# hirofumi0810/tensorflow_end2end_speech_recognition

Hardware: AMD Instinct MI355X
Metric: acoustic frames/sec (train), TIMIT-shaped BLSTM-CTC (higher is better)
Workload: dtype bf16; 1 GPU; TIMIT 61-phone 5x256 BLSTM-CTC, B=16/GPU, D=120, C=62, seq_len~U{100..778}, dropout 0.2, rmsprop, train step; global_batch=16, parallelism=dp1, padded_to=own Tmax per rank

## Files before the change

include/asr_hip.h:

```cpp
#ifndef ASR_HIP_H_
#define ASR_HIP_H_

#include <stddef.h>
#include <stdint.h>

#ifdef __cplusplus
extern "C" {
#endif

typedef struct asr_handle asr_handle;
typedef void* asr_stream;

typedef enum {
  ASR_OK = 0,
  ASR_ERR_INVALID_ARG = -1,
  ASR_ERR_UNSUPPORTED = -2,
  ASR_ERR_HIP = -3,
  ASR_ERR_WORKSPACE = -4
} asr_status;

typedef enum { ASR_F32 = 0, ASR_BF16 = 1 } asr_dtype;

typedef enum {
  ASR_OPT_SGD = 0, ASR_OPT_MOMENTUM = 1, ASR_OPT_NESTEROV = 2, ASR_OPT_ADAGRAD = 3,
  ASR_OPT_ADADELTA = 4, ASR_OPT_RMSPROP = 5, ASR_OPT_ADAM = 6
} asr_optimizer;

int asr_abi_version(void);
int asr_create(asr_handle** out, int device);
int asr_create_ex(asr_handle** out, int device, size_t scratch_bytes);
size_t asr_scratch_bytes(asr_handle* h);
int asr_destroy(asr_handle* h);
const char* asr_last_error_string(asr_handle* h);
int asr_set_xcd_skip(asr_handle* h, int n);
int asr_set_gemm_tn_workgroups(asr_handle* h, int n);
int asr_device_info(asr_handle* h, int* num_cu, char* name, int name_len);

int asr_bt_to_tb(asr_handle* h, int dtype, const float* in_btd, void* out_tbd,
                 int B, int T, int D, asr_stream s);
int asr_bt_to_tb_ld(asr_handle* h, int dtype, const float* in_btd, void* out_tbd,
                    int B, int T, int D, int ld_out, asr_stream s);
int asr_stack_frames(asr_handle* h, const float* x, const int32_t* seq_len, int B, int T, int F,
                     int num_stack, int num_skip, float* out, int32_t* out_len, asr_stream s);
int asr_splice(asr_handle* h, const float* x, const int32_t* seq_len, int B, int T, int D, int splice,
               int num_stack, float* out, asr_stream s);
int asr_transpose2d(asr_handle* h, int dtype, const void* in, int rows, int cols, int ld_in,
                    void* out, int ld_out, asr_stream s);
int asr_cast_from_f32(asr_handle* h, int dtype, const float* in, void* out, size_t n, asr_stream s);
int asr_cast_to_f32(asr_handle* h, int dtype, const void* in, float* out, size_t n, asr_stream s);
int asr_apply_mask(asr_handle* h, int dtype, const void* in, const float* mask, void* out,
                   size_t n, asr_stream s);
int asr_touch(asr_handle* h, const void* p, size_t bytes, asr_stream s);
int asr_dropout_mask(asr_handle* h, float* mask, size_t n, float keep_prob,
                     uint64_t seed, uint64_t offset, asr_stream s);
int asr_dropout_apply(asr_handle* h, int dtype, const void* in, void* out, size_t n, float keep_prob, uint64_t seed,
                      uint64_t offset, asr_stream s);
int asr_relu_bwd_drop(asr_handle* h, int dtype, const float* dout, const void* out, size_t n, float keep_prob,
                      uint64_t seed, uint64_t offset, void* dpre, asr_stream s);
int asr_colsum(asr_handle* h, int dtype, const void* a, int M, int N, int lda,
               float* out, asr_stream s);

int asr_gemm(asr_handle* h, int dtype, int out_dtype, int transA, int transB,
             int M, int N, int K, const void* A, int lda, const void* B, int ldb,
             void* C, int ldc, const float* bias, int accumulate, asr_stream s);

int asr_gemm_act(asr_handle* h, int dtype, int out_dtype, int transA, int transB,
                 int M, int N, int K, const void* A, int lda, const void* B, int ldb,
                 void* C, int ldc, const float* bias, int accumulate, int act, asr_stream s);
int asr_gemm_mul(asr_handle* h, int dtype, int transA, int transB, int M, int N, int K,
                 const void* A, int lda, const void* B, int ldb, float* C, int ldc,
                 const float* bias, int accumulate, int act, const float* mul, int ldmul, asr_stream s);
int asr_gemm_drop(asr_handle* h, int dtype, int transA, int transB, int M, int N, int K, const void* A, int lda,
                  const void* B, int ldb, float* C, int ldc, const float* bias, int accumulate, int act, float keep_prob,
                  uint64_t seed, uint64_t offset, asr_stream s);

int asr_im2col3x3(asr_handle* h, int dtype, const void* in, int N, int H, int W, int Cin, int ldp,
                  void* patches, asr_stream s);
int asr_col2im3x3(asr_handle* h, const float* dpatches, int N, int H, int W, int Cin, int ldp,
                  float* din, asr_stream s);
int asr_im2col(asr_handle* h, int dtype, const void* in_nhwc, int N, int H, int W, int Cin, int kh, int kw,
               int sh, int sw, int ldp, void* patches, asr_stream s);
int asr_col2im(asr_handle* h, const float* dpatches, int N, int H, int W, int Cin, int kh, int kw,
               int sh, int sw, int ldp, float* din_nhwc, asr_stream s);
int asr_conv3x3_prep_weights(asr_handle* h, const float* w_hwio, int Cin, int Cout, void* wt_fwd,
                             void* wt_bwd, asr_stream s);
int asr_conv3x3_fwd(asr_handle* h, const void* x, int N, int H, int W, int Cin, const void* wt_fwd,
                    const float* bias, int Cout, int relu, void* out, asr_stream s);
int asr_conv3x3_fwd_drop(asr_handle* h, const void* x, int N, int H, int W, int Cin, const void* wt_fwd,
                         const float* bias, int Cout, float keep_prob, uint64_t seed, uint64_t offset, void* out,
                         asr_stream s);
int asr_conv3x3_bwd_data(asr_handle* h, const void* dy, int N, int H, int W, int Cout,
                         const void* wt_bwd, int Cin, float* dx, asr_stream s);
int asr_conv3x3_bwd_data_relu(asr_handle* h, const void* dy, int N, int H, int W, int Cout, const void* wt_bwd, int Cin,
                              const void* act_below, float keep_prob, uint64_t seed, uint64_t offset, int use_drop,
                              void* dpre_below, asr_stream s);
int asr_conv3x3_bwd_weight(asr_handle* h, const void* x, const void* dy, int N, int H, int W,
                           int Cin, int Cout, float* dw, int accumulate, asr_stream s);
int asr_conv3x3_bwd_weight_bias(asr_handle* h, const void* x, const void* dy, int N, int H, int W,
                                int Cin, int Cout, float* dw, float* dbias, asr_stream s);
int asr_maxpool2x2_fwd(asr_handle* h, int dtype, const void* in, int N, int H, int W, int C,
                       void* out, uint8_t* argmax, asr_stream s);
int asr_maxpool2x2_fwd_drop(asr_handle* h, int dtype, const void* in, int N, int H, int W, int C, void* out,
                            uint8_t* argmax, float keep_prob, uint64_t seed, uint64_t offset, asr_stream s);
int asr_maxpool2x2_bwd(asr_handle* h, const float* dout, const uint8_t* argmax, int N, int H, int W,
                       int C, float* din, asr_stream s);
int asr_conv3x3_smallc_fwd(asr_handle* h, const void* x, int N, int H, int W, int Cin, const void* w2d,
                           const float* bias, int Cout, int relu, void* out, asr_stream s);
int asr_conv3x3_smallc_fwd_drop(asr_handle* h, const void* x, int N, int H, int W, int Cin, const void* w2d,
                                const float* bias, int Cout, float keep_prob, uint64_t seed, uint64_t offset, void* out,
                                asr_stream s);
int asr_conv3x3_smallc_bwd_weight(asr_handle* h, const void* x, const void* dpre, int N, int H, int W, int Cin,
                                  int Cout, float* dw, asr_stream s);
int asr_conv3x3_smallc_bwd_weight_bias(asr_handle* h, const void* x, const void* dpre, int N, int H, int W, int Cin,
                                       int Cout, float* dw, float* dbias, asr_stream s);
int asr_maxpool2x2_relu_bwd(asr_handle* h, int dtype, const float* dout, const uint8_t* argmax, const void* act, int N,
                            int H, int W, int C, void* dpre, float keep_prob, uint64_t seed, uint64_t offset,
                            int use_drop, asr_stream s);
int asr_relu_bwd(asr_handle* h, int dtype, const float* dout, const void* out, const float* mask,
                 size_t n, void* dpre, asr_stream s);
int asr_relu_bwd_scaled(asr_handle* h, int dtype, const float* dout, const void* out, size_t n, float keep, void* dpre,
                        asr_stream s);

int asr_conv3x5_prep_weights(asr_handle* h, const float* w_hwio, int Cin, int Cout, void* wt_fwd, void* wt_bwd,
                             asr_stream s);
int asr_conv3x5_fwd(asr_handle* h, const void* x, int N, int H, int W, int Cin, const void* wt_fwd, const float* bias,
                    int Cout, int relu, void* out, asr_stream s);
int asr_conv3x5_fwd_drop(asr_handle* h, const void* x, int N, int H, int W, int Cin, const void* wt_fwd,
                         const float* bias, int Cout, float keep_prob, uint64_t seed, uint64_t offset, void* out,
                         asr_stream s);
int asr_conv3x5_bwd_data(asr_handle* h, const void* dy, int N, int H, int W, int Cout, const void* wt_bwd, int Cin,
                         float* dx, asr_stream s);
int asr_conv3x5_bwd_data_relu(asr_handle* h, const void* dy, int N, int H, int W, int Cout, const void* wt_bwd, int Cin,
                              const void* act_below, float keep_prob, uint64_t seed, uint64_t offset, int use_drop,
                              void* dpre_below, asr_stream s);
int asr_conv3x5_bwd_weight_bias(asr_handle* h, const void* x, const void* dy, int N, int H, int W, int Cin, int Cout,
                                float* dw, float* dbias, asr_stream s);
int asr_maxpool3x1_fwd(asr_handle* h, int dtype, const void* in, int N, int H, int W, int C, void* out, uint8_t* argmax,
                       float keep_prob, uint64_t seed, uint64_t offset, int use_drop, asr_stream s);
int asr_maxpool3x1_bwd(asr_handle* h, int dtype, const void* dout, const uint8_t* argmax, int N, int H, int W, int C,
                       void* din, asr_stream s);

int asr_conv3x4_prep_weights(asr_handle* h, const float* w_hwio, int Cin, int Cout, void* wt_fwd, void* wt_bwd,
                             asr_stream s);
int asr_conv3x4_fwd(asr_handle* h, const void* x, int N, int H, int W, int Cin, const void* wt_fwd, const float* bias,
                    int Cout, int relu, int out_f32, void* out, asr_stream s);
int asr_conv3x4_bwd_data(asr_handle* h, const void* dy, int N, int H, int W, int Cout, const void* wt_bwd, int Cin,
                         float* dx, asr_stream s);
int asr_conv3x4_bwd_weight_bias(asr_handle* h, const void* x, const void* dy, int N, int H, int W, int Cin, int Cout,
                                float* dw, float* dbias, asr_stream s);
size_t asr_bn_workspace_bytes(long long M, int C);
int asr_bn_stats(asr_handle* h, const float* x, long long M, int C, float eps, float momentum, const float* avg_mean,
                 const float* avg_var, float* stats, void* ws, asr_stream s);
int asr_bn_apply(asr_handle* h, int out_dtype, const float* x, int N, int H, int W, int C, const float* mean,
                 const float* var, const float* gamma, const float* beta, float eps, int pool, void* out,
                 uint8_t* argmax, asr_stream s);
int asr_bn_bwd(asr_handle* h, int out_dtype, const float* dz, const uint8_t* argmax, int pool, const float* x, int N,
               int H, int W, int C, const float* stats, const float* gamma, int relu_gate, float* dgamma, float* dbeta,
               void* dx, void* ws, asr_stream s);
int asr_softmax_xent_soft(asr_handle* h, const float* logits, const float* targets, int rows, int C, float grad_scale,
                          float* row_loss, float* dlogits, asr_stream s);

int asr_lstm_prep_weights(asr_handle* h, int dtype, const float* kernel, const float* bias,
                          int Din, int H, void* wx_il, float* bias_il,
                          void* packed_fwd, void* packed_bwd, asr_stream s);
int asr_lstm_prep_layer(asr_handle* h, int dtype, int ndir, const float* const* vars, int Din, int ldk, int H,
                        void* wxT, void* wx_cat, float* bias_cat, void* packed_fwd, void* packed_bwd,
                        float* peep_out, asr_stream s);
int asr_lstm_grad_finish(asr_handle* h, int ndir, float* const* grads, int rows, int H, const float* dw_il,
                         const float* dpeep_dbias, int has_peep, asr_stream s);
int asr_gate_deinterleave(asr_handle* h, const float* in, int ld_in, float* out, int ld_out,
                          int rows, int H, asr_stream s);

int asr_lstm_fwd(asr_handle* h, int dtype, int T, int B, int H, int ndir,
                 const float* xproj, const void* wh_packed, const float* peep,
                 const int32_t* seq_len, float forget_bias, float cell_clip,
                 void* gates, void* hout, float* cs, float* c_final, float* h_final,
                 asr_stream s);

int asr_lstm_bwd(asr_handle* h, int dtype, int T, int B, int H, int ndir,
                 const float* dhout, const void* gates, const float* cs,
                 const void* wh_packed_bwd, const float* peep, const int32_t* seq_len,
                 const float* d_c_final, const float* d_h_final,
                 void* dgates, float* dpeep_dbias, float* dpeep_workspace, asr_stream s);
int asr_lstm_bwd_ex(asr_handle* h, int dtype, int T, int B, int H, int ndir,
                    const float* dhout, const void* gates, const float* cs,
                    const void* wh_packed_bwd, const float* peep, const int32_t* seq_len,
                    const float* d_c_final, const float* d_h_final, float clip_no_grad,
                    void* dgates, float* dpeep_dbias, float* dpeep_workspace, asr_stream s);

int asr_check_async_errors(asr_handle* h, unsigned* flags_out);
int asr_peek_async_errors(asr_handle* h, unsigned* host_flags, asr_stream s);
int asr_clear_async_errors(asr_handle* h, asr_stream s);
int asr_debug_set_lstm_flags(int flags);
int asr_debug_set_gru_persistent(int on);

int asr_debug_tear_probe(asr_handle* h, unsigned* buf, unsigned iters, int peer, int write_through,
                         unsigned long long* out, asr_stream s);

int asr_debug_placement(asr_handle* h, unsigned* out, int nblocks, int spin_cycles, asr_stream s);
int asr_debug_poison_lds(asr_handle* h, asr_stream s);

int asr_gru_fwd(asr_handle* h, int T, int B, int H, int ndir, const float* xg, const float* xc,
                const float* wgh, const float* wch, const int32_t* seq_len, int tmax, float* r, float* u,
                float* c, float* rh, float* hout, float* hstate2, asr_stream s);
int asr_gru_bwd(asr_handle* h, int T, int B, int H, int ndir, const float* dout, const float* d_h_final,
                const float* hout, const float* r, const float* u, const float* c, const float* wghT,
                const float* wchT, const int32_t* seq_len, int tmax, float* dgate, float* dcand,
                float* work2, asr_stream s);

size_t asr_ctc_workspace_bytes(int T, int B, int max_label_len);
int asr_ctc_loss(asr_handle* h, const float* logits, int T, int B, int C,
                 const int32_t* labels_flat, const int32_t* label_offsets,
                 const int32_t* seq_len, int max_label_len, float grad_scale,
                 float* loss, float* grad, int32_t* num_infeasible,
                 void* workspace, size_t workspace_bytes, asr_stream s);

int asr_ctc_greedy_decode(asr_handle* h, const float* logits, int T, int B, int C,
                          const int32_t* seq_len, int blank,
                          int32_t* out_labels, int32_t* out_len, asr_stream s);

size_t asr_ctc_beam_workspace_bytes(int T, int B, int C, int beam_width);
int asr_ctc_beam_decode(asr_handle* h, const float* logits, int T, int B, int C,
                        const int32_t* seq_len, int blank, int beam_width,
                        int32_t* out_labels, int32_t* out_len, double* out_score,
                        void* workspace, size_t workspace_bytes, asr_stream s);

int asr_softmax_rows(asr_handle* h, const float* in, float* out, int rows, int C, asr_stream s);
// ... 135 lines not shown
```

tensorflow_end2end_speech_recognition_amd/_lib.py:

```python
import ctypes as C
import os

_PKG = os.path.dirname(os.path.abspath(__file__))
LIB_PATH = os.path.join(_PKG, 'libasr_hip.so')

ASR_F32, ASR_BF16 = 0, 1
OPTIMIZER_IDS = {'sgd': 0, 'momentum': 1, 'nestrov': 2, 'adagrad': 3, 'adadelta': 4,
                 'rmsprop': 5, 'adam': 6}

_vp, _i, _f, _sz = C.c_void_p, C.c_int, C.c_float, C.c_size_t
_i64, _u64 = C.c_int64, C.c_uint64

SIGNATURES = {
    'asr_abi_version': (_i, []),
    'asr_create': (_i, [C.POINTER(_vp), _i]),
    'asr_create_ex': (_i, [C.POINTER(_vp), _i, _sz]),
    'asr_scratch_bytes': (_sz, [_vp]),
    'asr_destroy': (_i, [_vp]),
    'asr_set_xcd_skip': (_i, [_vp, _i]),
    'asr_set_gemm_tn_workgroups': (_i, [_vp, _i]),
    'asr_last_error_string': (C.c_char_p, [_vp]),
    'asr_device_info': (_i, [_vp, C.POINTER(_i), C.c_char_p, _i]),
    'asr_bt_to_tb': (_i, [_vp, _i, _vp, _vp, _i, _i, _i, _vp]),
    'asr_bt_to_tb_ld': (_i, [_vp, _i, _vp, _vp, _i, _i, _i, _i, _vp]),
    'asr_transpose2d': (_i, [_vp, _i, _vp, _i, _i, _i, _vp, _i, _vp]),
    'asr_cast_from_f32': (_i, [_vp, _i, _vp, _vp, _sz, _vp]),
    'asr_cast_to_f32': (_i, [_vp, _i, _vp, _vp, _sz, _vp]),
    'asr_apply_mask': (_i, [_vp, _i, _vp, _vp, _vp, _sz, _vp]),
    'asr_dropout_mask': (_i, [_vp, _vp, _sz, _f, _u64, _u64, _vp]),
    'asr_touch': (_i, [_vp, _vp, _sz, _vp]),
    'asr_dropout_apply': (_i, [_vp, _i, _vp, _vp, _sz, _f, _u64, _u64, _vp]),
    'asr_relu_bwd_drop': (_i, [_vp, _i, _vp, _vp, _sz, _f, _u64, _u64, _vp, _vp]),
    'asr_colsum': (_i, [_vp, _i, _vp, _i, _i, _i, _vp, _vp]),
    'asr_gemm': (_i, [_vp, _i, _i, _i, _i, _i, _i, _i, _vp, _i, _vp, _i, _vp, _i, _vp, _i, _vp]),
    'asr_gemm_act': (_i, [_vp, _i, _i, _i, _i, _i, _i, _i, _vp, _i, _vp, _i, _vp, _i, _vp, _i, _i, _vp]),
    'asr_gemm_drop': (_i, [_vp, _i, _i, _i, _i, _i, _i, _vp, _i, _vp, _i, _vp, _i, _vp, _i, _i, _f, _u64, _u64, _vp]),
    'asr_gemm_mul': (_i, [_vp, _i, _i, _i, _i, _i, _i, _vp, _i, _vp, _i, _vp, _i, _vp, _i, _i, _vp, _i, _vp]),
    'asr_conv3x3_prep_weights': (_i, [_vp, _vp, _i, _i, _vp, _vp, _vp]),
    'asr_conv3x3_fwd': (_i, [_vp, _vp, _i, _i, _i, _i, _vp, _vp, _i, _i, _vp, _vp]),
    'asr_conv3x3_fwd_drop': (_i, [_vp, _vp, _i, _i, _i, _i, _vp, _vp, _i, _f, _u64, _u64, _vp, _vp]),
    'asr_conv3x3_bwd_data': (_i, [_vp, _vp, _i, _i, _i, _i, _vp, _i, _vp, _vp]),
    'asr_conv3x3_smallc_fwd': (_i, [_vp, _vp, _i, _i, _i, _i, _vp, _vp, _i, _i, _vp, _vp]),
    'asr_conv3x3_smallc_fwd_drop': (_i, [_vp, _vp, _i, _i, _i, _i, _vp, _vp, _i, _f, _u64, _u64, _vp, _vp]),
    'asr_conv3x3_smallc_bwd_weight': (_i, [_vp, _vp, _vp, _i, _i, _i, _i, _i, _vp, _vp]),
    'asr_conv3x3_smallc_bwd_weight_bias': (_i, [_vp, _vp, _vp, _i, _i, _i, _i, _i, _vp, _vp, _vp]),
    'asr_conv3x3_bwd_data_relu': (_i, [_vp, _vp, _i, _i, _i, _i, _vp, _i, _vp, _f, _u64, _u64, _i, _vp, _vp]),
    'asr_conv3x3_bwd_weight': (_i, [_vp, _vp, _vp, _i, _i, _i, _i, _i, _vp, _i, _vp]),
    'asr_conv3x3_bwd_weight_bias': (_i, [_vp, _vp, _vp, _i, _i, _i, _i, _i, _vp, _vp, _vp]),
    'asr_im2col3x3': (_i, [_vp, _i, _vp, _i, _i, _i, _i, _i, _vp, _vp]),
    'asr_col2im3x3': (_i, [_vp, _vp, _i, _i, _i, _i, _i, _vp, _vp]),
    'asr_im2col': (_i, [_vp, _i, _vp, _i, _i, _i, _i, _i, _i, _i, _i, _i, _vp, _vp]),
    'asr_col2im': (_i, [_vp, _vp, _i, _i, _i, _i, _i, _i, _i, _i, _i, _vp, _vp]),
    'asr_maxpool2x2_fwd': (_i, [_vp, _i, _vp, _i, _i, _i, _i, _vp, _vp, _vp]),
    'asr_maxpool2x2_fwd_drop': (_i, [_vp, _i, _vp, _i, _i, _i, _i, _vp, _vp, _f, _u64, _u64, _vp]),
    'asr_relu_bwd_scaled': (_i, [_vp, _i, _vp, _vp, _sz, _f, _vp, _vp]),
    'asr_maxpool2x2_bwd': (_i, [_vp, _vp, _vp, _i, _i, _i, _i, _vp, _vp]),
    'asr_relu_bwd': (_i, [_vp, _i, _vp, _vp, _vp, _sz, _vp, _vp]),
    'asr_maxpool2x2_relu_bwd': (_i, [_vp, _i, _vp, _vp, _vp, _i, _i, _i, _i, _vp, _f, _u64, _u64, _i, _vp]),
    'asr_conv3x5_prep_weights': (_i, [_vp, _vp, _i, _i, _vp, _vp, _vp]),
    'asr_conv3x5_fwd': (_i, [_vp, _vp, _i, _i, _i, _i, _vp, _vp, _i, _i, _vp, _vp]),
    'asr_conv3x5_fwd_drop': (_i, [_vp, _vp, _i, _i, _i, _i, _vp, _vp, _i, _f, _u64, _u64, _vp, _vp]),
    'asr_conv3x5_bwd_data': (_i, [_vp, _vp, _i, _i, _i, _i, _vp, _i, _vp, _vp]),
    'asr_conv3x5_bwd_data_relu': (_i, [_vp, _vp, _i, _i, _i, _i, _vp, _i, _vp, _f, _u64, _u64, _i, _vp, _vp]),
    'asr_conv3x5_bwd_weight_bias': (_i, [_vp, _vp, _vp, _i, _i, _i, _i, _i, _vp, _vp, _vp]),
    'asr_maxpool3x1_fwd': (_i, [_vp, _i, _vp, _i, _i, _i, _i, _vp, _vp, _f, _u64, _u64, _i, _vp]),
    'asr_maxpool3x1_bwd': (_i, [_vp, _i, _vp, _vp, _i, _i, _i, _i, _vp, _vp]),
    'asr_conv3x4_prep_weights': (_i, [_vp, _vp, _i, _i, _vp, _vp, _vp]),
    'asr_conv3x4_fwd': (_i, [_vp, _vp, _i, _i, _i, _i, _vp, _vp, _i, _i, _i, _vp, _vp]),
    'asr_conv3x4_bwd_data': (_i, [_vp, _vp, _i, _i, _i, _i, _vp, _i, _vp, _vp]),
    'asr_conv3x4_bwd_weight_bias': (_i, [_vp, _vp, _vp, _i, _i, _i, _i, _i, _vp, _vp, _vp]),
    'asr_bn_workspace_bytes': (_sz, [_i64, _i]),
    'asr_bn_stats': (_i, [_vp, _vp, _i64, _i, _f, _f, _vp, _vp, _vp, _vp, _vp]),
    'asr_bn_apply': (_i, [_vp, _i, _vp, _i, _i, _i, _i, _vp, _vp, _vp, _vp, _f, _i, _vp, _vp, _vp]),
    'asr_bn_bwd': (_i, [_vp, _i, _vp, _vp, _i, _vp, _i, _i, _i, _i, _vp, _vp, _i, _vp, _vp, _vp, _vp, _vp]),
    'asr_softmax_xent_soft': (_i, [_vp, _vp, _vp, _i, _i, _f, _vp, _vp, _vp]),
    'asr_lstm_prep_weights': (_i, [_vp, _i, _vp, _vp, _i, _i, _vp, _vp, _vp, _vp, _vp]),
    'asr_lstm_prep_layer': (_i, [_vp, _i, _i, _vp, _i, _i, _i, _vp, _vp, _vp, _vp, _vp, _vp, _vp]),
    'asr_lstm_grad_finish': (_i, [_vp, _i, _vp, _i, _i, _vp, _vp, _i, _vp]),
    'asr_gate_deinterleave': (_i, [_vp, _vp, _i, _vp, _i, _i, _i, _vp]),
    'asr_lstm_fwd': (_i, [_vp, _i, _i, _i, _i, _i, _vp, _vp, _vp, _vp, _f, _f, _vp, _vp, _vp, _vp, _vp, _vp]),
    'asr_lstm_bwd': (_i, [_vp, _i, _i, _i, _i, _i, _vp, _vp, _vp, _vp, _vp, _vp, _vp, _vp, _vp, _vp,
                          _vp, _vp]),
    'asr_lstm_bwd_ex': (_i, [_vp, _i, _i, _i, _i, _i, _vp, _vp, _vp, _vp, _vp, _vp, _vp, _vp, _f, _vp, _vp,
                             _vp, _vp]),
    'asr_gru_fwd': (_i, [_vp, _i, _i, _i, _i, _vp, _vp, _vp, _vp, _vp, _i, _vp, _vp, _vp, _vp, _vp, _vp, _vp]),
    'asr_gru_bwd': (_i, [_vp, _i, _i, _i, _i, _vp, _vp, _vp, _vp, _vp, _vp, _vp, _vp, _vp, _i, _vp, _vp, _vp, _vp]),
    'asr_check_async_errors': (_i, [_vp, C.POINTER(C.c_uint)]),
    'asr_peek_async_errors': (_i, [_vp, _vp, _vp]),
    'asr_clear_async_errors': (_i, [_vp, _vp]),
    'asr_debug_set_lstm_flags': (_i, [_i]),
    'asr_debug_set_gru_persistent': (_i, [_i]),
    'asr_debug_placement': (_i, [_vp, _vp, _i, _i, _vp]),
    'asr_debug_poison_lds': (_i, [_vp, _vp]),
    'asr_debug_tear_probe': (_i, [_vp, _vp, C.c_uint, _i, _i, _vp, _vp]),
    'asr_ctc_workspace_bytes': (_sz, [_i, _i, _i]),
    'asr_ctc_loss': (_i, [_vp, _vp, _i, _i, _i, _vp, _vp, _vp, _i, _f, _vp, _vp, _vp, _vp, _sz, _vp]),
    'asr_ctc_greedy_decode': (_i, [_vp, _vp, _i, _i, _i, _vp, _i, _vp, _vp, _vp]),
    'asr_ctc_beam_workspace_bytes': (_sz, [_i, _i, _i, _i]),
    'asr_ctc_beam_decode': (_i, [_vp, _vp, _i, _i, _i, _vp, _i, _i, _vp, _vp, _vp, _vp, _sz, _vp]),
    'asr_softmax_rows': (_i, [_vp, _vp, _vp, _i, _i, _vp]),
    'asr_lstm_cell_fwd': (_i, [_vp] * 6 + [_i, _i, _f, _f] + [_vp] * 6),
    'asr_lstm_cell_fwd_ex': (_i, [_vp] * 6 + [_i, _i, _f, _f] + [_vp] * 5 + [_vp, _vp, _vp, _i, _vp, _i, _vp]),
    'asr_lstm_cell_gemm_ok': (_i, [_i, _i, _i, _i]),
    'asr_lstm_cell_gemm_prep': (_i, [_vp, _vp, _vp, _i, _i, _vp, _vp]),
    'asr_lstm_cell_gemm_fwd': (_i, [_vp, _vp, _i, _i, _vp, _i] + [_vp] * 4 + [_i, _i, _f, _f] + [_vp] * 5 +
                               [_vp, _vp, _vp, _i, _vp, _i, _vp]),
    'asr_lstm_cell_gemm_h_bytes': (_sz, [_i, _i]),
    'asr_lstm_cell_gemm_prep_h': (_i, [_vp, _vp, _vp, _i, _i, _vp, _vp]),
    'asr_lstm_cell_gemm_fwd_h': (_i, [_vp, _vp, _i, _i, _vp] + [_vp] * 4 + [_i, _i, _f, _f] + [_vp] * 5 +
                                 [_vp, _vp, _vp, _i, _vp, _i, _vp]),
    'asr_lstm_cell_gemm_bwd_h': (_i, [_vp, _vp, _i, _i, _i, _vp, _vp, _i, _vp]),
    'asr_lstm_cell_bwd': (_i, [_vp] * 9 + [_i, _i] + [_vp] * 5),
    'asr_lstm_cell_bwd_ex': (_i, [_vp] * 9 + [_i, _i, _f] + [_vp] * 5),
    'asr_stack_frames': (_i, [_vp, _vp, _vp, _i, _i, _i, _i, _i, _vp, _vp, _vp]),
    'asr_splice': (_i, [_vp, _vp, _vp, _i, _i, _i, _i, _i, _vp, _vp]),
    'asr_att_energy_fwd': (_i, [_vp, _vp, _vp, _vp, _i, _i, _i, _i, _vp, _vp]),
    'asr_att_energy_bwd': (_i, [_vp, _vp, _vp, _vp, _vp, _i, _i, _i, _i, _vp, _vp, _vp, _vp]),
    'asr_att_softmax_ctx_fwd': (_i, [_vp, _vp, _vp, _f, _vp, _i, _i, _i, _i, _vp, _vp, _vp, _vp]),
    'asr_att_softmax_ctx_fwd_ex': (_i, [_vp, _vp, _vp, _f, _vp, _i, _i, _i, _i, _vp, _vp, _vp, _vp, _i, _vp, _i, _vp]),
    'asr_att_softmax_ctx_bwd': (_i, [_vp, _vp, _vp, _vp, _f, _vp, _i, _i, _i, _i, _vp, _vp, _vp, _vp, _vp]),
    'asr_att_loc_energy_fwd': (_i, [_vp] * 7 + [_i, _i, _i, _i, _vp, _vp]),
    'asr_att_loc_energy_bwd': (_i, [_vp] * 8 + [_i, _i, _i, _i] + [_vp] * 6 + [_i, _vp]),
    'asr_att_decoder_fwd': (_i, [_vp, _vp, _vp]),
    'asr_att_decoder_bwd': (_i, [_vp, _vp, _vp]),
    'asr_att_decoder_infer': (_i, [_vp, _vp, _vp, _vp, _vp]),
    'asr_add_cols': (_i, [_vp, _vp, _i, _vp, _i, _vp, _i, _i, _i, _vp]),
    'asr_tanh_fwd': (_i, [_vp, _vp, _vp, _sz, _vp]),
    'asr_tanh_bwd': (_i, [_vp, _vp, _vp, _vp, _sz, _vp]),
    'asr_embedding_gather': (_i, [_vp, _vp, _vp, _i, _i, _vp, _vp]),
    'asr_embedding_scatter': (_i, [_vp, _vp, _vp, _i, _i, _i, _vp, _vp]),
    'asr_seq_xent': (_i, [_vp, _vp, _vp, _vp, _i, _i, _f, _f, _vp, _vp, _vp]),
    'asr_argmax_rows': (_i, [_vp, _vp, _i, _i, _vp, _vp]),
    'asr_clip_plan': (_i, [_vp, _vp, _i, _vp]),
    'asr_clip_by_norm_multi': (_i, [_vp, _vp, _vp, _vp, _i, _i64, _f, _vp, _vp]),
    'asr_weight_decay': (_i, [_vp, _vp, _vp, _vp, _vp, _i, _f, _vp, _vp]),
    'asr_optimizer_step': (_i, [_vp, _i, _vp, _vp, _vp, _vp, _sz, _f, _i64, _vp]),
    'asr_scale': (_i, [_vp, _vp, _sz, _f, _vp]),
    'asr_comm_set_library': (_i, [C.c_char_p]),
    'asr_comm_unique_id': (_i, [_vp]),
    'asr_comm_init': (_i, [C.POINTER(_vp), _vp, _i, _i, _vp]),
    'asr_comm_destroy': (_i, [_vp]),
    'asr_comm_info': (_i, [_vp, C.POINTER(_i), C.POINTER(_i)]),
    'asr_allreduce_mean': (_i, [_vp, _vp, _sz, _vp]),
}

_lib = None


ABI_VERSION = 5


def load():
    global _lib
    if _lib is not None:
        return _lib
    if not os.path.exists(LIB_PATH):
        raise RuntimeError(
            'libasr_hip.so not found at %s -- build it with '
            '`python -m tensorflow_end2end_speech_recognition_amd.build` '
            '(there is no CPU fallback for the HIP path)' % LIB_PATH)
    lib = C.CDLL(LIB_PATH, mode=C.RTLD_GLOBAL)
    ver = getattr(lib, 'asr_abi_version', None)
    got = int(ver()) if ver is not None else 0
    if got < ABI_VERSION:
        raise RuntimeError('%s reports asr_abi_version() = %d but this package binds version %d entry points: the '
                           'library is stale -- rebuild it with `python -m tensorflow_end2end_speech_recognition_amd.build`'
                           % (LIB_PATH, got, ABI_VERSION))
    for name, (res, args) in SIGNATURES.items():
        fn = getattr(lib, name, None)
        if fn is None:
            raise RuntimeError('%s (abi %d) does not export %s: rebuild it with '
                               '`python -m tensorflow_end2end_speech_recognition_amd.build`' % (LIB_PATH, got, name))
        fn.restype = res
        fn.argtypes = args
    _lib = lib
    return lib


class AsrError(RuntimeError):
    pass


class Handle(object):

    def __init__(self, device=0):
        self.lib = load()
        h = _vp()
        rc = self.lib.asr_create(C.byref(h), int(device))
        if rc != 0:
            raise AsrError('asr_create(device=%d) failed with %d: no usable MI355X/HIP device -- '
# ... 36 lines not shown
```

tensorflow_end2end_speech_recognition_amd/csrc/elementwise.hip:

```cpp
#include "common.h"
#include <math.h>

extern "C" int asr_abi_version(void) { return 5; }

extern "C" int asr_create(asr_handle** out, int device) { return asr_create_ex(out, device, (size_t)192 << 20); }
extern "C" size_t asr_scratch_bytes(asr_handle* h) { return h ? h->scratch_bytes : 0; }

extern "C" int asr_create_ex(asr_handle** out, int device, size_t scratch_bytes) {
  if (!out || scratch_bytes < ((size_t)96 << 20)) return ASR_ERR_INVALID_ARG;
  int n = 0;
  if (hipGetDeviceCount(&n) != hipSuccess || device < 0 || device >= n) return ASR_ERR_HIP;
  if (hipSetDevice(device) != hipSuccess) return ASR_ERR_HIP;
  hipDeviceProp_t p;
  if (hipGetDeviceProperties(&p, device) != hipSuccess) return ASR_ERR_HIP;
  asr_handle* h = new asr_handle();
  h->device = device;
  h->num_cu = p.multiProcessorCount;
  snprintf(h->name, sizeof(h->name), "%s (%s)", p.name, p.gcnArchName);
  h->err[0] = 0;
  h->scratch = nullptr;
  h->scratch_bytes = scratch_bytes;
  h->xch_dirty[0] = h->xch_dirty[1] = 0;
  h->xch_next = 0;
  h->xcd_skip = 0;
// ... 31 lines not shown
  return ASR_OK;
}

namespace {
__global__ void placement_kernel(unsigned* out, int spin) {
  if (threadIdx.x == 0) {
    out[2 * blockIdx.x] = __builtin_amdgcn_s_getreg((3 << 11) | 20) & 0xFu;
    out[2 * blockIdx.x + 1] = __builtin_amdgcn_s_getreg((31 << 11) | 4);
  }
  const unsigned long long t0 = __builtin_amdgcn_s_memtime();
  while ((long long)(__builtin_amdgcn_s_memtime() - t0) < spin) __builtin_amdgcn_s_sleep(8);
}
}
extern "C" int asr_debug_placement(asr_handle* h, unsigned* out, int nblocks, int spin_cycles, asr_stream s) {
  if (!h || !out || nblocks < 1) return ASR_ERR_INVALID_ARG;
  hipLaunchKernelGGL(placement_kernel, dim3(nblocks), dim3(64), 0, (hipStream_t)s, out, spin_cycles);
  ASR_CHECK_LAUNCH(h, "placement_kernel");
  return ASR_OK;
}

namespace {

inline int grid_for(size_t n, int per_thread = 1) {
  size_t blocks = (n + 256 * (size_t)per_thread - 1) / (256 * (size_t)per_thread);
  if (blocks < 1) blocks = 1;
  if (blocks > 2048) blocks = 2048;
  return (int)blocks;
}

template <typename T>
__global__ void bt_to_tb_kernel(const float* __restrict__ in, T* __restrict__ out, int B, int T_, int D, int ld) {
  const size_t total = (size_t)B * T_ * ld;
  for (size_t i = blockIdx.x * (size_t)blockDim.x + threadIdx.x; i < total;
       i += (size_t)gridDim.x * blockDim.x) {
    const int dd = i % ld;
    const size_t r = i / ld;
    const int b = r % B;
    const size_t t = r / B;
    out[i] = dd < D ? Elem<T>::from_f32(in[((size_t)b * T_ + t) * D + dd]) : Elem<T>::from_f32(0.f);
  }
}

template <typename T>
__global__ void cast_from_f32_kernel(const float* __restrict__ in, T* __restrict__ out, size_t n) {
  for (size_t i = blockIdx.x * (size_t)blockDim.x + threadIdx.x; i < n; i += (size_t)gridDim.x * blockDim.x)
    out[i] = Elem<T>::from_f32(in[i]);
}
template <typename T>
__global__ void cast_to_f32_kernel(const T* __restrict__ in, float* __restrict__ out, size_t n) {
  for (size_t i = blockIdx.x * (size_t)blockDim.x + threadIdx.x; i < n; i += (size_t)gridDim.x * blockDim.x)
    out[i] = Elem<T>::to_f32(in[i]);
}
template <typename T>
__global__ void apply_mask_kernel(const T* __restrict__ in, const float* __restrict__ mask,
                                  T* __restrict__ out, size_t n) {
  for (size_t i = blockIdx.x * (size_t)blockDim.x + threadIdx.x; i < n; i += (size_t)gridDim.x * blockDim.x)
    out[i] = Elem<T>::from_f32(Elem<T>::to_f32(in[i]) * mask[i]);
}

__device__ __forceinline__ void philox4x32(uint32_t c[4], uint32_t k0, uint32_t k1) {
#pragma unroll
  for (int r = 0; r < 10; ++r) {
    const uint64_t p0 = (uint64_t)0xD2511F53u * c[0];
    const uint64_t p1 = (uint64_t)0xCD9E8D57u * c[2];
    const uint32_t n0 = (uint32_t)(p1 >> 32) ^ c[1] ^ k0;
    const uint32_t n1 = (uint32_t)p1;
    const uint32_t n2 = (uint32_t)(p0 >> 32) ^ c[3] ^ k1;
    const uint32_t n3 = (uint32_t)p0;
    c[0] = n0; c[1] = n1; c[2] = n2; c[3] = n3;
    k0 += 0x9E3779B9u; k1 += 0xBB67AE85u;
  }
}
__global__ void dropout_mask_kernel(float* __restrict__ mask, size_t n, float keep, uint64_t seed,
                                    uint64_t offset) {
  const float inv = 1.f / keep;
  const size_t n4 = (n + 3) / 4;
  for (size_t i = blockIdx.x * (size_t)blockDim.x + threadIdx.x; i < n4; i += (size_t)gridDim.x * blockDim.x) {
    const uint64_t ctr = offset + i;
    uint32_t c[4] = {(uint32_t)ctr, (uint32_t)(ctr >> 32), 0u, 0u};
    philox4x32(c, (uint32_t)seed, (uint32_t)(seed >> 32));
#pragma unroll
    for (int j = 0; j < 4; ++j) {
      const size_t e = i * 4 + j;
      if (e < n) {
        const float u = (c[j] >> 8) * (1.0f / 16777216.0f);
        mask[e] = (u < keep) ? inv : 0.f;
      }
    }
  }
}

__device__ __forceinline__ void dropout_words(uint64_t ctr, uint64_t seed, float keep, float inv, float m[4]) {
  uint32_t c[4] = {(uint32_t)ctr, (uint32_t)(ctr >> 32), 0u, 0u};
  philox4x32(c, (uint32_t)seed, (uint32_t)(seed >> 32));
#pragma unroll
  for (int j = 0; j < 4; ++j) m[j] = ((c[j] >> 8) * (1.0f / 16777216.0f) < keep) ? inv : 0.f;
}
template <typename T> struct Vec4;
template <> struct Vec4<float> {
  typedef f32x4_t raw_t;
  static __device__ __forceinline__ void load(const float* p, float v[4]) {
    const f32x4_t r = *reinterpret_cast<const f32x4_t*>(p);
    v[0] = r[0]; v[1] = r[1]; v[2] = r[2]; v[3] = r[3];
  }
  static __device__ __forceinline__ void store(float* p, const float v[4]) {
    *reinterpret_cast<f32x4_t*>(p) = (f32x4_t){v[0], v[1], v[2], v[3]};
  }
};
template <> struct Vec4<bf16_t> {
  typedef __attribute__((ext_vector_type(4))) unsigned short us4_t;
  static __device__ __forceinline__ void load(const bf16_t* p, float v[4]) {
    const us4_t r = *reinterpret_cast<const us4_t*>(p);
#pragma unroll
    for (int j = 0; j < 4; ++j) v[j] = bf16_to_f32(r[j]);
  }
  static __device__ __forceinline__ void store(bf16_t* p, const float v[4]) {
    us4_t r;
#pragma unroll
    for (int j = 0; j < 4; ++j) r[j] = f32_to_bf16(v[j]);
    *reinterpret_cast<us4_t*>(p) = r;
  }
};
template <typename TI, typename TO>
__global__ void dropout_apply_kernel(const TI* __restrict__ in, const TO* __restrict__ relu_out, TO* __restrict__ out,
                                     size_t n, float keep, uint64_t seed, uint64_t offset, int vec_ok) {
  const float inv = 1.f / keep;
  const size_t n4 = (n + 3) / 4;
  for (size_t i = blockIdx.x * (size_t)blockDim.x + threadIdx.x; i < n4; i += (size_t)gridDim.x * blockDim.x) {
    float m[4];
    dropout_words(offset + i, seed, keep, inv, m);
    const size_t e0 = i * 4;
    if (vec_ok && e0 + 4 <= n) {
      float x[4], r[4];
      Vec4<TI>::load(in + e0, x);
      if (relu_out) Vec4<TO>::load(relu_out + e0, r);
#pragma unroll
      for (int j = 0; j < 4; ++j) {
        x[j] *= m[j];
        if (relu_out) x[j] = r[j] > 0.f ? x[j] : 0.f;
      }
      Vec4<TO>::store(out + e0, x);
      continue;
    }
#pragma unroll
    for (int j = 0; j < 4; ++j) {
      const size_t e = e0 + j;
      if (e < n) {
        float g = Elem<TI>::to_f32(in[e]) * m[j];
        if (relu_out) g = Elem<TO>::to_f32(relu_out[e]) > 0.f ? g : 0.f;
        out[e] = Elem<TO>::from_f32(g);
      }
    }
  }
}

__global__ void touch_kernel(const f32x4_t* __restrict__ p, size_t n16, unsigned* __restrict__ sink) {
  f32x4_t acc = {0.f, 0.f, 0.f, 0.f};
  for (size_t i = blockIdx.x * (size_t)blockDim.x + threadIdx.x; i < n16; i += (size_t)gridDim.x * blockDim.x) {
    const f32x4_t v = p[i];
    acc[0] += v[0]; acc[1] += v[1]; acc[2] += v[2]; acc[3] += v[3];
  }
  if (acc[0] + acc[1] + acc[2] + acc[3] == 1.2345e-33f) *sink = 1u;
}

constexpr int COLSUM_ROWS = 512;
template <typename T>
__global__ __launch_bounds__(256) void colsum_kernel(const T* __restrict__ a, int M, int N, int lda,
                                                     float* __restrict__ partial) {
  __shared__ float part[4][64];
  const int col = blockIdx.x * 64 + (threadIdx.x & 63);
  const int rgp = threadIdx.x >> 6;
  const int r0 = blockIdx.y * COLSUM_ROWS, r1 = min(M, r0 + COLSUM_ROWS);
  float s = 0.f;
  if (col < N) {
#pragma unroll 8
    for (int m = r0 + rgp; m < r1; m += 4) s += Elem<T>::to_f32(a[(size_t)m * lda + col]);
  }
  part[rgp][threadIdx.x & 63] = s;
  __syncthreads();
  if (rgp == 0 && col < N)
    partial[(size_t)blockIdx.y * N + col] =
        part[0][threadIdx.x] + part[1][threadIdx.x] + part[2][threadIdx.x] + part[3][threadIdx.x];
}
__global__ __launch_bounds__(256) void colsum_bf16_vec_kernel(const bf16_t* __restrict__ a, long long M, int N,
                                                              long long rows_per_block, float* __restrict__ partial) {
  extern __shared__ float cred[];
  const int NV = N / 8, RT = 256 / NV;
  const int cg = threadIdx.x % NV, rt = threadIdx.x / NV;
  const long long r0 = (long long)blockIdx.x * rows_per_block;
  const long long r1 = r0 + rows_per_block < M ? r0 + rows_per_block : M;
  float s[8] = {0.f, 0.f, 0.f, 0.f, 0.f, 0.f, 0.f, 0.f};
  if (rt < RT) {
    for (long long m = r0 + rt; m < r1; m += RT) {
      const bf16x8_t v = *reinterpret_cast<const bf16x8_t*>(a + (size_t)m * N + cg * 8);
#pragma unroll
      for (int i = 0; i < 8; ++i) s[i] += bf16_to_f32((bf16_t)v[i]);
    }
#pragma unroll
    for (int i = 0; i < 8; ++i) cred[rt * N + cg * 8 + i] = s[i];
  }
  __syncthreads();
  for (int col = threadIdx.x; col < N; col += 256) {
    float t = 0.f;
    for (int r = 0; r < RT; ++r) t += cred[r * N + col];
    partial[(size_t)blockIdx.x * N + col] = t;
  }
}
__global__ void colsum_final_kernel(const float* __restrict__ partial, int RB, int N, float* __restrict__ out) {
  const int col = blockIdx.x * blockDim.x + threadIdx.x;
  if (col >= N) return;
  float s = 0.f;
#pragma unroll 8
  for (int r = 0; r < RB; ++r) s += partial[(size_t)r * N + col];
  out[col] = s;
}

__global__ __launch_bounds__(256) void colsum_final_wide_kernel(const float* __restrict__ partial, int RB, int N,
                                                                float* __restrict__ out) {
  __shared__ float red[16][17];
  const int c = threadIdx.x & 15, grp = threadIdx.x >> 4;
  const int col = blockIdx.x * 16 + c;
  float s = 0.f;
  if (col < N)
    for (int r = grp; r < RB; r += 16) s += partial[(size_t)r * N + col];
  red[grp][c] = s;
  __syncthreads();
  if (grp == 0 && col < N) {
    float t = 0.f;
#pragma unroll
    for (int k = 0; k < 16; ++k) t += red[k][c];
    out[col] = t;
  }
}

constexpr int NORM_CHUNK = 4096;
__global__ __launch_bounds__(256) void sqsum_partial_kernel(const float* __restrict__ g,
                                                            const int64_t* __restrict__ offsets,
                                                            const int64_t* __restrict__ chunk_start,
                                                            int num_tensors, float* __restrict__ partial) {
  __shared__ float red[4];
  const int64_t cid = blockIdx.x;
  int lo = 0, hi = num_tensors - 1;
  while (lo < hi) {
    const int mid = (lo + hi + 1) >> 1;
    if (chunk_start[mid] <= cid) lo = mid; else hi = mid - 1;
  }
  const int64_t beg = offsets[lo] + (cid - chunk_start[lo]) * NORM_CHUNK;
  const int64_t end = min(beg + (int64_t)NORM_CHUNK, offsets[lo + 1]);
  float s = 0.f;
#pragma unroll 8
  for (int64_t i = beg + threadIdx.x; i < end; i += 256) { const float v = g[i]; s += v * v; }
  s = wave_reduce_sum(s);
  if ((threadIdx.x & 63) == 0) red[threadIdx.x >> 6] = s;
  __syncthreads();
  if (threadIdx.x == 0) partial[cid] = red[0] + red[1] + red[2] + red[3];
}
__global__ void clip_scale_kernel(float* __restrict__ g, const int64_t* __restrict__ offsets,
                                  const int64_t* __restrict__ chunk_start, int num_tensors,
                                  const float* __restrict__ partial, float clip) {
  const int64_t cid = blockIdx.x;
  int lo = 0, hi = num_tensors - 1;
  while (lo < hi) {
    const int mid = (lo + hi + 1) >> 1;
    if (chunk_start[mid] <= cid) lo = mid; else hi = mid - 1;
  }
  __shared__ float sp[1024];
  float ss = 0.f;
  const int64_t cend = chunk_start[lo + 1];
  for (int64_t c0 = chunk_start[lo]; c0 < cend; c0 += 1024) {
    const int n = (int)min((int64_t)1024, cend - c0);
    for (int i = threadIdx.x; i < n; i += blockDim.x) sp[i] = partial[c0 + i];
    __syncthreads();
    for (int i = 0; i < n; ++i) ss += sp[i];
    __syncthreads();
  }
  const float norm = sqrtf(ss);
  const float scale = clip / fmaxf(norm, clip);
  if (scale == 1.f) return;
  const int64_t beg = offsets[lo] + (cid - chunk_start[lo]) * NORM_CHUNK;
  const int64_t end = min(beg + (int64_t)NORM_CHUNK, offsets[lo + 1]);
  const int64_t a0 = min(end, (beg + 3) & ~(int64_t)3), a1 = a0 + ((end - a0) & ~(int64_t)3);
  for (int64_t i = beg + threadIdx.x; i < a0; i += blockDim.x) g[i] *= scale;
  for (int64_t i = a0 + 4 * (int64_t)threadIdx.x; i < a1; i += 4 * (int64_t)blockDim.x) {
    f32x4_t v = *reinterpret_cast<f32x4_t*>(g + i);
    v[0] *= scale; v[1] *= scale; v[2] *= scale; v[3] *= scale;
    *reinterpret_cast<f32x4_t*>(g + i) = v;
  }
  for (int64_t i = a1 + threadIdx.x; i < end; i += blockDim.x) g[i] *= scale;
}

__global__ void weight_decay_kernel(float* __restrict__ g, const float* __restrict__ p,
                                    const int64_t* __restrict__ offsets,
                                    const uint8_t* __restrict__ decay_mask, int num_tensors, float wd) {
  const int t = blockIdx.y;
  if (!decay_mask[t]) return;
  const int64_t beg = offsets[t], end = offsets[t + 1];
  for (int64_t i = beg + blockIdx.x * (int64_t)blockDim.x + threadIdx.x; i < end;
       i += (int64_t)gridDim.x * blockDim.x)
    g[i] += wd * p[i];
}
__global__ __launch_bounds__(256) void l2_loss_kernel(const float* __restrict__ p,
                                                      const int64_t* __restrict__ offsets,
                                                      const uint8_t* __restrict__ decay_mask,
                                                      int num_tensors, float wd, float* __restrict__ out) {
  __shared__ float red[4];
  float s = 0.f;
// ... 163 lines not shown
    float* o = out + f * row;
    const bool live = t < len;
    for (int c4 = threadIdx.x * 4; c4 < row; c4 += 1024) {
      const uint4 u = *reinterpret_cast<const uint4*>(tab + c4);
      const uint32_t uu[4] = {u.x, u.y, u.z, u.w};
      float v[4];
#pragma unroll
      for (int e = 0; e < 4; ++e) {
        v[e] = 0.f;
        if (live && uu[e] != 0xffffffffu) {
          const int is = (int)(uu[e] >> 24);
          int src = t + is - splice;
          if (t <= splice - 1 && is < splice - t) src = 0;
          else if (len - splice <= t && src > len - 1) src = len - 1;
          v[e] = xb[(size_t)src * D + (uu[e] & 0xffffffu)];
        }
      }
      *reinterpret_cast<float4*>(o + c4) = make_float4(v[0], v[1], v[2], v[3]);
    }
  }
}
}

extern "C" int asr_stack_frames(asr_handle* h, const float* x, const int32_t* seq_len, int B, int T, int F,
                                int num_stack, int num_skip, float* out, int32_t* out_len, asr_stream s) {
  if (!h) return ASR_ERR_INVALID_ARG;
  ASR_NEED(x && seq_len && out && B >= 0 && T >= 0 && F > 0 && num_stack >= 1 && num_skip >= 1,
           "asr_stack_frames: bad args");
  ASR_NEED(num_stack >= num_skip, "asr_stack_frames: num_skip must not exceed num_stack");
  const int Tn = (T + num_skip - 1) / num_skip;
  const size_t n = (size_t)B * Tn * F * num_stack;
  if (!n) return ASR_OK;
  hipLaunchKernelGGL(stack_frames_kernel, dim3(grid_for(n)), dim3(256), 0, (hipStream_t)s, x, seq_len, B, T, F,
                     num_stack, num_skip, Tn, out, out_len);
  ASR_CHECK_LAUNCH(h, "asr_stack_frames");
  return ASR_OK;
}

extern "C" int asr_splice(asr_handle* h, const float* x, const int32_t* seq_len, int B, int T, int D, int splice,
                          int num_stack, float* out, asr_stream s) {
  if (!h) return ASR_ERR_INVALID_ARG;
  ASR_NEED(x && seq_len && out && B >= 0 && T >= 0 && D > 0 && splice >= 1 && num_stack >= 1,
           "asr_splice: bad args");
  ASR_NEED(D % (3 * num_stack) == 0, "asr_splice: frame width %d is not channels*3*num_stack", D);
  const size_t n = (size_t)B * T * D * splice;
  if (!n) return ASR_OK;
  const size_t row = (size_t)D * splice;
  if (row % 4 == 0 && row * sizeof(uint32_t) <= 48 * 1024 && splice < 256 && D < (1 << 24) &&
      (reinterpret_cast<uintptr_t>(out) & 15) == 0) {
    const size_t nblk = ((size_t)B * T + SPLICE_FPB - 1) / SPLICE_FPB;
    hipLaunchKernelGGL(splice_rows_kernel, dim3((unsigned)nblk), dim3(256), row * sizeof(uint32_t), (hipStream_t)s, x,
                       seq_len, B, T, D, splice, num_stack, out);
  } else {
    hipLaunchKernelGGL(splice_kernel, dim3(grid_for(n)), dim3(256), 0, (hipStream_t)s, x, seq_len, B, T, D, splice,
                       num_stack, out);
  }
  ASR_CHECK_LAUNCH(h, "asr_splice");
  return ASR_OK;
}

extern "C" int asr_bt_to_tb_ld(asr_handle* h, int dtype, const float* in, void* out, int B, int T, int D, int ld_out,
                               asr_stream s) {
  if (!h) return ASR_ERR_INVALID_ARG;
  ASR_NEED(asr_dtype_ok(dtype) && in && out && B >= 0 && T >= 0 && D >= 0 && ld_out >= D, "asr_bt_to_tb: bad args");
  const size_t n = (size_t)B * T * ld_out;
  if (!n) return ASR_OK;
  if (dtype == ASR_F32) hipLaunchKernelGGL(bt_to_tb_kernel<float>, dim3(grid_for(n)), dim3(256), 0, (hipStream_t)s, in, (float*)out, B, T, D, ld_out);
  else hipLaunchKernelGGL(bt_to_tb_kernel<bf16_t>, dim3(grid_for(n)), dim3(256), 0, (hipStream_t)s, in, (bf16_t*)out, B, T, D, ld_out);
  ASR_CHECK_LAUNCH(h, "asr_bt_to_tb");
  return ASR_OK;
}
extern "C" int asr_bt_to_tb(asr_handle* h, int dtype, const float* in, void* out, int B, int T, int D, asr_stream s) {
  return asr_bt_to_tb_ld(h, dtype, in, out, B, T, D, D, s);
}
extern "C" int asr_cast_from_f32(asr_handle* h, int dtype, const float* in, void* out, size_t n, asr_stream s) {
  if (!h) return ASR_ERR_INVALID_ARG;
  ASR_NEED(asr_dtype_ok(dtype) && in && out, "asr_cast_from_f32: bad args");
  if (!n) return ASR_OK;
  if (dtype == ASR_F32) hipLaunchKernelGGL(cast_from_f32_kernel<float>, dim3(grid_for(n)), dim3(256), 0, (hipStream_t)s, in, (float*)out, n);
  else hipLaunchKernelGGL(cast_from_f32_kernel<bf16_t>, dim3(grid_for(n)), dim3(256), 0, (hipStream_t)s, in, (bf16_t*)out, n);
  ASR_CHECK_LAUNCH(h, "asr_cast_from_f32");
  return ASR_OK;
}
extern "C" int asr_cast_to_f32(asr_handle* h, int dtype, const void* in, float* out, size_t n, asr_stream s) {
  if (!h) return ASR_ERR_INVALID_ARG;
  ASR_NEED(asr_dtype_ok(dtype) && in && out, "asr_cast_to_f32: bad args");
  if (!n) return ASR_OK;
  if (dtype == ASR_F32) hipLaunchKernelGGL(cast_to_f32_kernel<float>, dim3(grid_for(n)), dim3(256), 0, (hipStream_t)s, (const float*)in, out, n);
  else hipLaunchKernelGGL(cast_to_f32_kernel<bf16_t>, dim3(grid_for(n)), dim3(256), 0, (hipStream_t)s, (const bf16_t*)in, out, n);
  ASR_CHECK_LAUNCH(h, "asr_cast_to_f32");
  return ASR_OK;
}
extern "C" int asr_apply_mask(asr_handle* h, int dtype, const void* in, const float* mask, void* out, size_t n, asr_stream s) {
  if (!h) return ASR_ERR_INVALID_ARG;
  ASR_NEED(asr_dtype_ok(dtype) && in && mask && out, "asr_apply_mask: bad args");
  if (!n) return ASR_OK;
  if (dtype == ASR_F32) hipLaunchKernelGGL(apply_mask_kernel<float>, dim3(grid_for(n)), dim3(256), 0, (hipStream_t)s, (const float*)in, mask, (float*)out, n);
  else hipLaunchKernelGGL(apply_mask_kernel<bf16_t>, dim3(grid_for(n)), dim3(256), 0, (hipStream_t)s, (const bf16_t*)in, mask, (bf16_t*)out, n);
  ASR_CHECK_LAUNCH(h, "asr_apply_mask");
  return ASR_OK;
}
extern "C" int asr_dropout_mask(asr_handle* h, float* mask, size_t n, float keep_prob, uint64_t seed, uint64_t offset, asr_stream s) {
  if (!h) return ASR_ERR_INVALID_ARG;
  ASR_NEED(mask && keep_prob > 0.f && keep_prob <= 1.f, "asr_dropout_mask: keep_prob must be in (0,1]");
  if (!n) return ASR_OK;
  hipLaunchKernelGGL(dropout_mask_kernel, dim3(grid_for((n + 3) / 4)), dim3(256), 0, (hipStream_t)s, mask, n, keep_prob, seed, offset);
  ASR_CHECK_LAUNCH(h, "asr_dropout_mask");
  return ASR_OK;
}
extern "C" int asr_dropout_apply(asr_handle* h, int dtype, const void* in, void* out, size_t n, float keep_prob,
                                 uint64_t seed, uint64_t offset, asr_stream s) {
  if (!h) return ASR_ERR_INVALID_ARG;
  ASR_NEED(asr_dtype_ok(dtype) && in && out && keep_prob > 0.f && keep_prob <= 1.f, "asr_dropout_apply: bad args");
  if (!n) return ASR_OK;
  const dim3 grid(grid_for((n + 3) / 4));
  const int vec_ok = (((uintptr_t)in | (uintptr_t)out) % 16) == 0;
  if (dtype == ASR_F32)
    hipLaunchKernelGGL((dropout_apply_kernel<float, float>), grid, dim3(256), 0, (hipStream_t)s, (const float*)in,
                       (const float*)nullptr, (float*)out, n, keep_prob, seed, offset, vec_ok);
  else
    hipLaunchKernelGGL((dropout_apply_kernel<bf16_t, bf16_t>), grid, dim3(256), 0, (hipStream_t)s, (const bf16_t*)in,
                       (const bf16_t*)nullptr, (bf16_t*)out, n, keep_prob, seed, offset, vec_ok);
  ASR_CHECK_LAUNCH(h, "asr_dropout_apply");
  return ASR_OK;
}
extern "C" int asr_relu_bwd_drop(asr_handle* h, int dtype, const float* dout, const void* out, size_t n, float keep_prob,
                                 uint64_t seed, uint64_t offset, void* dpre, asr_stream s) {
  if (!h) return ASR_ERR_INVALID_ARG;
  ASR_NEED(asr_dtype_ok(dtype) && dout && out && dpre && keep_prob > 0.f && keep_prob <= 1.f, "asr_relu_bwd_drop: bad args");
  if (!n) return ASR_OK;
  const dim3 grid(grid_for((n + 3) / 4));
  const int vec_ok = (((uintptr_t)dout | (uintptr_t)out | (uintptr_t)dpre) % 16) == 0;
  if (dtype == ASR_F32)
    hipLaunchKernelGGL((dropout_apply_kernel<float, float>), grid, dim3(256), 0, (hipStream_t)s, dout, (const float*)out,
                       (float*)dpre, n, keep_prob, seed, offset, vec_ok);
  else
    hipLaunchKernelGGL((dropout_apply_kernel<float, bf16_t>), grid, dim3(256), 0, (hipStream_t)s, dout,
                       (const bf16_t*)out, (bf16_t*)dpre, n, keep_prob, seed, offset, vec_ok);
  ASR_CHECK_LAUNCH(h, "asr_relu_bwd_drop");
  return ASR_OK;
}
extern "C" int asr_touch(asr_handle* h, const void* p, size_t bytes, asr_stream s) {
  if (!h) return ASR_ERR_INVALID_ARG;
  ASR_NEED(p && ((uintptr_t)p) % 16 == 0, "asr_touch: 16-byte aligned buffer");
  const size_t n16 = bytes / 16;
  if (!n16) return ASR_OK;
  int blocks = (int)((n16 + 255) / 256);
  if (blocks > 1024) blocks = 1024;
  hipLaunchKernelGGL(touch_kernel, dim3(blocks), dim3(256), 0, (hipStream_t)s, (const f32x4_t*)p, n16,
                     (unsigned*)h->scratch);
  ASR_CHECK_LAUNCH(h, "asr_touch");
  return ASR_OK;
}
extern "C" int asr_colsum(asr_handle* h, int dtype, const void* a, int M, int N, int lda, float* out, asr_stream s) {
  if (!h) return ASR_ERR_INVALID_ARG;
  ASR_NEED(asr_dtype_ok(dtype) && a && out && M >= 0 && N > 0 && lda >= N, "asr_colsum: bad args");
  if (dtype == ASR_BF16 && lda == N && N % 8 == 0 && 256 % (N / 8) == 0 && N <= 512 && M >= 4096 &&
      ((uintptr_t)a & 15) == 0) {
    long long rpb = ((long long)M + 2047) / 2048;
    if (rpb < 256) rpb = 256;
    const int nb = (int)(((long long)M + rpb - 1) / rpb);
    float* pv = (float*)h->scratch;
    hipLaunchKernelGGL(colsum_bf16_vec_kernel, dim3(nb), dim3(256), (size_t)(256 / (N / 8)) * N * sizeof(float),
                       (hipStream_t)s, (const bf16_t*)a, (long long)M, N, rpb, pv);
    if (nb > 64)
      hipLaunchKernelGGL(colsum_final_wide_kernel, dim3((N + 15) / 16), dim3(256), 0, (hipStream_t)s, pv, nb, N, out);
    else
      hipLaunchKernelGGL(colsum_final_kernel, dim3((N + 255) / 256), dim3(256), 0, (hipStream_t)s, pv, nb, N, out);
    ASR_CHECK_LAUNCH(h, "asr_colsum");
    return ASR_OK;
  }
  int RB = (M + COLSUM_ROWS - 1) / COLSUM_ROWS > 0 ? (M + COLSUM_ROWS - 1) / COLSUM_ROWS : 1;
  const size_t need = ((size_t)RB + (size_t)(RB + COLSUM_ROWS - 1) / COLSUM_ROWS + 1) * N * sizeof(float);
  if (need > h->scratch_bytes - ASR_XCH_BYTES) ASR_FAIL(h, ASR_ERR_WORKSPACE, "asr_colsum: scratch too small");
  float* partial = (float*)h->scratch;
  {
    const dim3 grid((N + 63) / 64, RB);
    if (dtype == ASR_F32) hipLaunchKernelGGL(colsum_kernel<float>, grid, dim3(256), 0, (hipStream_t)s, (const float*)a, M, N, lda, partial);
    else hipLaunchKernelGGL(colsum_kernel<bf16_t>, grid, dim3(256), 0, (hipStream_t)s, (const bf16_t*)a, M, N, lda, partial);
  }
  float* other = partial + (size_t)RB * N;
  while (RB > 64) {
    const int RB2 = (RB + COLSUM_ROWS - 1) / COLSUM_ROWS;
    hipLaunchKernelGGL(colsum_kernel<float>, dim3((N + 63) / 64, RB2), dim3(256), 0, (hipStream_t)s, partial, RB, N, N, other);
    float* t = partial; partial = other; other = t;
    RB = RB2;
  }
  hipLaunchKernelGGL(colsum_final_kernel, dim3((N + 255) / 256), dim3(256), 0, (hipStream_t)s, partial, RB, N, out);
  ASR_CHECK_LAUNCH(h, "asr_colsum");
  return ASR_OK;
}

extern "C" int asr_clip_plan(asr_handle* h, const int64_t* offsets_host, int num_tensors,
                             int64_t* chunk_start_host) {
  if (!h) return ASR_ERR_INVALID_ARG;
  ASR_NEED(offsets_host && chunk_start_host && num_tensors >= 0, "asr_clip_plan: bad args");
  int64_t c = 0;
  for (int t = 0; t < num_tensors; ++t) {
    chunk_start_host[t] = c;
    c += (offsets_host[t + 1] - offsets_host[t] + NORM_CHUNK - 1) / NORM_CHUNK;
  }
  chunk_start_host[num_tensors] = c;
  return ASR_OK;
}
extern "C" int asr_clip_by_norm_multi(asr_handle* h, float* grads, const int64_t* offsets,
                                      const int64_t* chunk_start, int num_tensors, int64_t total_chunks,
                                      float clip_norm, float* partial_ws, asr_stream s) {
  if (!h) return ASR_ERR_INVALID_ARG;
  ASR_NEED(grads && offsets && chunk_start && partial_ws && num_tensors >= 0 && clip_norm > 0.f,
           "asr_clip_by_norm_multi: bad args (clip_norm must be > 0)");
  if (num_tensors == 0 || total_chunks == 0) return ASR_OK;
  hipLaunchKernelGGL(sqsum_partial_kernel, dim3((unsigned)total_chunks), dim3(256), 0, (hipStream_t)s, grads,
                     offsets, chunk_start, num_tensors, partial_ws);
  ASR_CHECK_LAUNCH(h, "asr_clip_by_norm_multi(sqsum)");
  hipLaunchKernelGGL(clip_scale_kernel, dim3((unsigned)total_chunks), dim3(256), 0, (hipStream_t)s, grads,
                     offsets, chunk_start, num_tensors, partial_ws, clip_norm);
  ASR_CHECK_LAUNCH(h, "asr_clip_by_norm_multi(scale)");
  return ASR_OK;
}
extern "C" int asr_weight_decay(asr_handle* h, float* grads, const float* params, const int64_t* offsets,
                                const uint8_t* decay_mask, int num_tensors, float wd, float* l2_out,
                                asr_stream s) {
  if (!h) return ASR_ERR_INVALID_ARG;
  ASR_NEED(params && offsets && decay_mask && num_tensors >= 0 && wd >= 0.f, "asr_weight_decay: bad args");
  if (num_tensors == 0) return ASR_OK;
  if (grads) {
    hipLaunchKernelGGL(weight_decay_kernel, dim3(64, num_tensors), dim3(256), 0, (hipStream_t)s, grads, params,
                       offsets, decay_mask, num_tensors, wd);
    ASR_CHECK_LAUNCH(h, "asr_weight_decay");
  }
  if (l2_out) {
    hipLaunchKernelGGL(l2_loss_kernel, dim3(1), dim3(256), 0, (hipStream_t)s, params, offsets, decay_mask,
                       num_tensors, wd, l2_out);
    ASR_CHECK_LAUNCH(h, "asr_weight_decay(l2)");
  }
  return ASR_OK;
}
extern "C" int asr_optimizer_step(asr_handle* h, int optimizer, float* params, const float* grads,
                                  float* slot0, float* slot1, size_t n, float lr, int64_t step,
                                  asr_stream s) {
  if (!h) return ASR_ERR_INVALID_ARG;
  ASR_NEED(params && grads, "asr_optimizer_step: null params/grads");
  if (!n) return ASR_OK;
  const int needs0 = optimizer != ASR_OPT_SGD;
  const int needs1 = optimizer == ASR_OPT_ADADELTA || optimizer == ASR_OPT_RMSPROP || optimizer == ASR_OPT_ADAM;
  ASR_NEED(!needs0 || slot0, "asr_optimizer_step: optimizer %d needs slot0", optimizer);
  ASR_NEED(!needs1 || slot1, "asr_optimizer_step: optimizer %d needs slot1", optimizer);
  float adam_lr_t = lr;
  if (optimizer == ASR_OPT_ADAM) {
    ASR_NEED(step >= 1, "asr_optimizer_step: adam needs step >= 1");
    adam_lr_t = (float)(lr * sqrt(1.0 - pow(0.999, (double)step)) / (1.0 - pow(0.9, (double)step)));
  }
  const dim3 g(grid_for(n)), b(256);
  hipStream_t st = (hipStream_t)s;
  switch (optimizer) {
#define ASR_OPT_CASE(O) case O: hipLaunchKernelGGL(optimizer_kernel<O>, g, b, 0, st, params, grads, slot0, slot1, n, lr, adam_lr_t); break
    ASR_OPT_CASE(ASR_OPT_SGD);
    ASR_OPT_CASE(ASR_OPT_MOMENTUM);
    ASR_OPT_CASE(ASR_OPT_NESTEROV);
    ASR_OPT_CASE(ASR_OPT_ADAGRAD);
    ASR_OPT_CASE(ASR_OPT_ADADELTA);
    ASR_OPT_CASE(ASR_OPT_RMSPROP);
    ASR_OPT_CASE(ASR_OPT_ADAM);
#undef ASR_OPT_CASE
    default: ASR_FAIL(h, ASR_ERR_INVALID_ARG, "asr_optimizer_step: unknown optimizer %d", optimizer);
  }
  ASR_CHECK_LAUNCH(h, "asr_optimizer_step");
  return ASR_OK;
}
extern "C" int asr_scale(asr_handle* h, float* x, size_t n, float scale, asr_stream s) {
  if (!h) return ASR_ERR_INVALID_ARG;
  ASR_NEED(x, "asr_scale: null");
  if (!n) return ASR_OK;
  hipLaunchKernelGGL(scale_kernel, dim3(grid_for(n)), dim3(256), 0, (hipStream_t)s, x, n, scale);
  ASR_CHECK_LAUNCH(h, "asr_scale");
  return ASR_OK;
}

namespace {
__global__ __launch_bounds__(256) void poison_lds_kernel(unsigned pattern, unsigned words, unsigned* sink) {
  extern __shared__ unsigned lds_words[];
  for (unsigned i = threadIdx.x; i < words; i += 256) lds_words[i] = pattern;
  __syncthreads();
  if (sink && lds_words[(threadIdx.x * 97u) % words] != pattern) *sink = 1u;
  __builtin_amdgcn_s_sleep(64);
}
}
extern "C" int asr_debug_poison_lds(asr_handle* h, asr_stream s) {
  if (!h) return ASR_ERR_INVALID_ARG;
  const size_t bytes = (size_t)160 << 10;
  (void)hipFuncSetAttribute((const void*)poison_lds_kernel, hipFuncAttributeMaxDynamicSharedMemorySize, (int)bytes);
  hipLaunchKernelGGL(poison_lds_kernel, dim3((unsigned)(2 * h->num_cu)), dim3(256), bytes, (hipStream_t)s, 0xFFFFFFFFu,
                     (unsigned)(bytes / 4), (unsigned*)nullptr);
  ASR_CHECK_LAUNCH(h, "asr_debug_poison_lds");
  return ASR_OK;
}
```

tensorflow_end2end_speech_recognition_amd/csrc/gemm.hip:

```cpp
#include "common.h"
#include <stdlib.h>

namespace {

static inline bool first_on_device(unsigned long long& mask) {
  int d = 0;
  (void)hipGetDevice(&d);
  const unsigned long long bit = 1ull << (d & 63);
  if (mask & bit) return false;
  mask |= bit;
  return true;
}

template <typename T> struct GT;
template <> struct GT<float> {
  static constexpr int BK = 32;
  static constexpr int VEC = 4;
};
template <> struct GT<bf16_t> {
  static constexpr int BK = 64;
  static constexpr int VEC = 8;
};

template <typename T> struct Vec16 { T v[GT<T>::VEC]; } __attribute__((aligned(16)));
// ... 58 lines not shown
#pragma unroll
        for (int j = 0; j < VEC; ++j) s[(r + j) * lds_ld + k] = reg[i].v[j];
      }
    }
  }
};

template <typename T, typename TO, int BM, int BN, bool TA, bool TB>
__global__ __launch_bounds__(256) void gemm_kernel(int M, int N, int K, const T* __restrict__ A,
                                                   int lda, const T* __restrict__ B, int ldb,
                                                   TO* __restrict__ C, int ldc,
                                                   const float* __restrict__ bias, int accumulate,
                                                   int a_aligned, int b_aligned, int kchunk,
                                                   float* __restrict__ partial, int act, int c_vec) {
  constexpr int BK = GT<T>::BK, VEC = GT<T>::VEC;
  constexpr int LDS_LD = BK + VEC;
  constexpr int WM = BM / 2, WN = BN / 2, TM = WM / 16, TN = WN / 16;
  extern __shared__ __attribute__((aligned(16))) char smem[];
  T* As = reinterpret_cast<T*>(smem);
  T* Bs = As + BM * LDS_LD;

  const int lane = threadIdx.x & 63, wave = threadIdx.x >> 6;
  const int wm = wave >> 1, wn = wave & 1;
  const int m0 = blockIdx.y * BM, n0 = blockIdx.x * BN;

  TileLoader<T, BM, !TA> la;
  TileLoader<T, BN, TB> lb;

  f32x4_t acc[TM][TN];
#pragma unroll
  for (int i = 0; i < TM; ++i)
#pragma unroll
    for (int j = 0; j < TN; ++j) acc[i][j] = (f32x4_t){0.f, 0.f, 0.f, 0.f};

  const int kbeg = blockIdx.z * kchunk;
  const int kend = min(K, kbeg + kchunk);
  const int nkt = (kend - kbeg + BK - 1) / BK;
  constexpr int STAGE = (BM + BN) * LDS_LD;
  la.load(A, lda, m0, kbeg, M, kend, a_aligned);
  lb.load(B, ldb, n0, kbeg, N, kend, b_aligned);
  la.store(As, LDS_LD);
  lb.store(Bs, LDS_LD);
  __syncthreads();

  for (int kt = 0; kt < nkt; ++kt) {
    const T* Ac = As + (kt & 1) * STAGE;
    const T* Bc = Bs + (kt & 1) * STAGE;
    if (kt + 1 < nkt) {
      la.load(A, lda, m0, kbeg + (kt + 1) * BK, M, kend, a_aligned);
      lb.load(B, ldb, n0, kbeg + (kt + 1) * BK, N, kend, b_aligned);
    }
    const int fr = lane & 15, fq = lane >> 4;
    if constexpr (sizeof(T) == 2) {
#pragma unroll
      for (int ks = 0; ks < BK / 32; ++ks) {
        bf16x8_t a[TM], b[TN];
#pragma unroll
        for (int i = 0; i < TM; ++i)
          a[i] = *reinterpret_cast<const bf16x8_t*>(Ac + (wm * WM + i * 16 + fr) * LDS_LD + ks * 32 + fq * 8);
#pragma unroll
        for (int j = 0; j < TN; ++j)
          b[j] = *reinterpret_cast<const bf16x8_t*>(Bc + (wn * WN + j * 16 + fr) * LDS_LD + ks * 32 + fq * 8);
#pragma unroll
        for (int i = 0; i < TM; ++i)
#pragma unroll
          for (int j = 0; j < TN; ++j)
            acc[i][j] = __builtin_amdgcn_mfma_f32_16x16x32_bf16(b[j], a[i], acc[i][j], 0, 0, 0);
      }
    } else {
#pragma unroll
      for (int ks = 0; ks < BK / 4; ++ks) {
        float a[TM], b[TN];
#pragma unroll
        for (int i = 0; i < TM; ++i) a[i] = Ac[(wm * WM + i * 16 + fr) * LDS_LD + ks * 4 + fq];
#pragma unroll
        for (int j = 0; j < TN; ++j) b[j] = Bc[(wn * WN + j * 16 + fr) * LDS_LD + ks * 4 + fq];
#pragma unroll
        for (int i = 0; i < TM; ++i)
#pragma unroll
          for (int j = 0; j < TN; ++j)
            acc[i][j] = __builtin_amdgcn_mfma_f32_16x16x4f32(b[j], a[i], acc[i][j], 0, 0, 0);
      }
    }
    if (kt + 1 < nkt) {
      la.store(As + ((kt + 1) & 1) * STAGE, LDS_LD);
      lb.store(Bs + ((kt + 1) & 1) * STAGE, LDS_LD);
    }
    __syncthreads();
  }

#pragma unroll
  for (int i = 0; i < TM; ++i)
#pragma unroll
    for (int j = 0; j < TN; ++j) {
      const int m = m0 + wm * WM + i * 16 + (lane & 15);
      const int nb = n0 + wn * WN + j * 16 + (lane >> 4) * 4;
      if (m >= M || nb >= N) continue;
      const bool full = nb + 3 < N;
      if (partial) {
        float* pp = partial + ((size_t)blockIdx.z * M + m) * N + nb;
        if (full && (N & 3) == 0) *reinterpret_cast<f32x4_t*>(pp) = acc[i][j];
        else
          for (int r = 0; r < 4 && nb + r < N; ++r) pp[r] = acc[i][j][r];
        continue;
      }
      TO* cp = C + (size_t)m * ldc + nb;
      float v[4];
#pragma unroll
      for (int r = 0; r < 4; ++r) v[r] = acc[i][j][r] + ((bias && nb + r < N) ? bias[nb + r] : 0.f);
      if (full && c_vec) {
        if constexpr (sizeof(TO) == 4) {
          if (accumulate) {
            const f32x4_t o = *reinterpret_cast<const f32x4_t*>(cp);
#pragma unroll
            for (int r = 0; r < 4; ++r) v[r] += o[r];
          }
          if (act == 1) {
#pragma unroll
            for (int r = 0; r < 4; ++r) v[r] = fmaxf(v[r], 0.f);
          }
          *reinterpret_cast<f32x4_t*>(cp) = (f32x4_t){v[0], v[1], v[2], v[3]};
        } else {
          typedef __attribute__((ext_vector_type(4))) unsigned short us4_t;
          if (accumulate) {
            const us4_t o = *reinterpret_cast<const us4_t*>(cp);
#pragma unroll
            for (int r = 0; r < 4; ++r) v[r] += bf16_to_f32(o[r]);
          }
          if (act == 1) {
#pragma unroll
            for (int r = 0; r < 4; ++r) v[r] = fmaxf(v[r], 0.f);
          }
          *reinterpret_cast<us4_t*>(cp) = (us4_t){f32_to_bf16(v[0]), f32_to_bf16(v[1]), f32_to_bf16(v[2]), f32_to_bf16(v[3])};
        }
      } else {
        for (int r = 0; r < 4 && nb + r < N; ++r) {
          float w = v[r];
          if (accumulate) w += load_out<TO>(cp + r);
          if (act == 1) w = fmaxf(w, 0.f);
          store_out<TO>(cp + r, w);
        }
      }
    }
}

__device__ __forceinline__ unsigned nt_swz(int row) { return (((row + 4) >> 3) & 1) ? 8u : 0u; }

struct GemmDrop {
  float keep;
  uint64_t seed, offset;
  int use;
};

template <typename TO>
__global__ __launch_bounds__(256) void gemm_nt_bf16_kernel(int M, int N, int K, const bf16_t* __restrict__ A,
                                                           int lda, const bf16_t* __restrict__ Bt, int ldb,
                                                           TO* __restrict__ C, int ldc,
                                                           const float* __restrict__ bias, int accumulate,
                                                           int act, const float* __restrict__ mul, int ldm,
                                                           GemmDrop drop) {
  constexpr int BM = 128, BN = 128, BK = 64, LD = BK + 8;
  constexpr int STAGE = (BM + BN) * LD;
  extern __shared__ __attribute__((aligned(16))) char smem[];
  bf16_t* S = reinterpret_cast<bf16_t*>(smem);

  const int tid = threadIdx.x, lane = tid & 63, wave = tid >> 6;
  const int wm = wave >> 1, wn = wave & 1;
  const int ntn = N / BN, ntm = (M + BM - 1) / BM, total = ntn * ntm;
  int t = blockIdx.x;
  if ((total & 7) == 0) t = (t & 7) * (total >> 3) + (t >> 3);
  const int m0 = (t / ntn) * BM, n0 = (t % ntn) * BN;

  const bf16_t* pa[4];
  const bf16_t* pb[4];
  unsigned so[4];
#pragma unroll
  for (int i = 0; i < 4; ++i) {
    const int v = tid + i * 256, r = v >> 3, kv = (v & 7) * 8;
    pa[i] = A + (size_t)min(m0 + r, M - 1) * lda + kv;
    pb[i] = Bt + (size_t)(n0 + r) * ldb + kv;
    so[i] = (unsigned)(r * LD) + ((unsigned)kv ^ nt_swz(r));
  }
  bf16x8_t ra[4], rb[4];
  auto gload = [&]() {
#pragma unroll
    for (int i = 0; i < 4; ++i) {
      ra[i] = *reinterpret_cast<const bf16x8_t*>(pa[i]);
      rb[i] = *reinterpret_cast<const bf16x8_t*>(pb[i]);
      pa[i] += BK;
      pb[i] += BK;
    }
  };
  auto sstore = [&](bf16_t* st) {
#pragma unroll
    for (int i = 0; i < 4; ++i) {
      *reinterpret_cast<bf16x8_t*>(st + so[i]) = ra[i];
      *reinterpret_cast<bf16x8_t*>(st + BM * LD + so[i]) = rb[i];
    }
  };

  f32x4_t acc[4][4];
#pragma unroll
  for (int i = 0; i < 4; ++i)
#pragma unroll
    for (int j = 0; j < 4; ++j) acc[i][j] = (f32x4_t){0.f, 0.f, 0.f, 0.f};

  const int nkt = K / BK;
  gload();
  sstore(S);
  __syncthreads();
  const int fr = lane & 15, fq = lane >> 4;
  const unsigned aoff = (unsigned)((wm * 64 + fr) * LD) + ((unsigned)(fq * 8) ^ nt_swz(fr));
  const unsigned boff = (unsigned)(BM * LD + (wn * 64 + fr) * LD) + ((unsigned)(fq * 8) ^ nt_swz(fr));
  for (int kt = 0; kt < nkt; ++kt) {
    const bf16_t* cur = S + (kt & 1) * STAGE;
    if (kt + 1 < nkt) gload();
#pragma unroll
    for (int ks = 0; ks < 2; ++ks) {
      bf16x8_t a[4], b[4];
#pragma unroll
      for (int i = 0; i < 4; ++i) a[i] = *reinterpret_cast<const bf16x8_t*>(cur + aoff + i * 16 * LD + ks * 32);
#pragma unroll
      for (int j = 0; j < 4; ++j) b[j] = *reinterpret_cast<const bf16x8_t*>(cur + boff + j * 16 * LD + ks * 32);
#pragma unroll
      for (int i = 0; i < 4; ++i)
#pragma unroll
        for (int j = 0; j < 4; ++j)
          acc[i][j] = __builtin_amdgcn_mfma_f32_16x16x32_bf16(b[j], a[i], acc[i][j], 0, 0, 0);
    }
    if (kt + 1 < nkt) sstore(S + ((kt + 1) & 1) * STAGE);
    __syncthreads();
  }
#pragma unroll
  for (int i = 0; i < 4; ++i) {
    const int m = m0 + wm * 64 + i * 16 + fr;
    if (m >= M) continue;
#pragma unroll
    for (int j = 0; j < 4; ++j) {
      const int nb = n0 + wn * 64 + j * 16 + fq * 4;
      TO* cp = C + (size_t)m * ldc + nb;
      float v[4];
#pragma unroll
      for (int r = 0; r < 4; ++r) v[r] = acc[i][j][r];
      if (bias) {
        const f32x4_t bv = *reinterpret_cast<const f32x4_t*>(bias + nb);
#pragma unroll
        for (int r = 0; r < 4; ++r) v[r] += bv[r];
      }
      if constexpr (sizeof(TO) == 4) {
        if (accumulate) {
          const f32x4_t o = *reinterpret_cast<const f32x4_t*>(cp);
#pragma unroll
          for (int r = 0; r < 4; ++r) v[r] += o[r];
        }
        if (act == 1) {
#pragma unroll
          for (int r = 0; r < 4; ++r) v[r] = fmaxf(v[r], 0.f);
        }
        if (mul) {
          const f32x4_t mv = *reinterpret_cast<const f32x4_t*>(mul + (size_t)m * ldm + nb);
#pragma unroll
          for (int r = 0; r < 4; ++r) v[r] *= mv[r];
        }
        if (drop.use) {
          float mk[4];
          asr_dropout_words(drop.offset + ((size_t)m * N + nb) / 4, drop.seed, drop.keep, 1.f / drop.keep, mk);
#pragma unroll
          for (int r = 0; r < 4; ++r) v[r] *= mk[r];
        }
        *reinterpret_cast<f32x4_t*>(cp) = (f32x4_t){v[0], v[1], v[2], v[3]};
      } else {
        typedef __attribute__((ext_vector_type(4))) unsigned short us4_t;
        if (accumulate) {
          const us4_t o = *reinterpret_cast<const us4_t*>(cp);
#pragma unroll
          for (int r = 0; r < 4; ++r) v[r] += bf16_to_f32(o[r]);
        }
        if (act == 1) {
#pragma unroll
          for (int r = 0; r < 4; ++r) v[r] = fmaxf(v[r], 0.f);
        }
        *reinterpret_cast<us4_t*>(cp) = (us4_t){f32_to_bf16(v[0]), f32_to_bf16(v[1]), f32_to_bf16(v[2]), f32_to_bf16(v[3])};
      }
    }
  }
}

template <typename TO, int BM, int BN, int WM, int WN>
__global__ __launch_bounds__(WM * WN * 64, 1) void gemm_nt_bf16_big_kernel(int M, int N, int K, const bf16_t* __restrict__ A,
                                                                           int lda, const bf16_t* __restrict__ Bt, int ldb,
                                                                           TO* __restrict__ C, int ldc,
                                                                           const float* __restrict__ bias, int accumulate,
                                                                           int act, const float* __restrict__ mul, int ldm,
                                                                           GemmDrop drop) {
  constexpr int BK = 64, LD = BK + 8, NT = WM * WN * 64;
  constexpr int STAGE = (BM + BN) * LD;
  constexpr int TM = BM / WM, TN = BN / WN, TI = TM / 16, TJ = TN / 16;
  constexpr int VA = BM * 8 / NT, VB = BN * 8 / NT, RSTEP = NT / 8;
  extern __shared__ __attribute__((aligned(16))) char smem[];
  bf16_t* S = reinterpret_cast<bf16_t*>(smem);

  const int tid = threadIdx.x, lane = tid & 63, wave = tid >> 6;
  const int wm = wave / WN, wn = wave % WN;
  const int ntn = N / BN, ntm = (M + BM - 1) / BM, total = ntn * ntm;
  int t = blockIdx.x;
  if ((total & 7) == 0) t = (t & 7) * (total >> 3) + (t >> 3);
  const int m0 = (t / ntn) * BM, n0 = (t % ntn) * BN;

  const int r0 = tid >> 3, kv = (tid & 7) * 8;
  unsigned oa[VA], ob[VB];
#pragma unroll
  for (int i = 0; i < VA; ++i) oa[i] = (unsigned)(((size_t)min(m0 + r0 + RSTEP * i, M - 1) * lda + kv) * sizeof(bf16_t));
#pragma unroll
  for (int i = 0; i < VB; ++i) ob[i] = (unsigned)(((size_t)(n0 + r0 + RSTEP * i) * ldb + kv) * sizeof(bf16_t));
  const unsigned so0 = (unsigned)(r0 * LD) + ((unsigned)kv ^ nt_swz(r0));
  const __amdgpu_buffer_rsrc_t rsA = __builtin_amdgcn_make_buffer_rsrc(
      const_cast<bf16_t*>(A), 0, (int)min((size_t)0xFFFFFFFFu, ((size_t)(M - 1) * lda + K) * sizeof(bf16_t)), 0x00020000);
  const __amdgpu_buffer_rsrc_t rsB = __builtin_amdgcn_make_buffer_rsrc(
      const_cast<bf16_t*>(Bt), 0, (int)min((size_t)0xFFFFFFFFu, ((size_t)(N - 1) * ldb + K) * sizeof(bf16_t)), 0x00020000);
  typedef __attribute__((ext_vector_type(4))) unsigned u32x4_t;
  u32x4_t ra[VA], rb[VB];
  unsigned koff = 0;
  auto gload = [&]() {
#pragma unroll
    for (int i = 0; i < VA; ++i) ra[i] = __builtin_amdgcn_raw_buffer_load_b128(rsA, oa[i], koff, 0);
#pragma unroll
    for (int i = 0; i < VB; ++i) rb[i] = __builtin_amdgcn_raw_buffer_load_b128(rsB, ob[i], koff, 0);
    koff += BK * sizeof(bf16_t);
  };
  auto sstore = [&](bf16_t* st) {
#pragma unroll
    for (int i = 0; i < VA; ++i) *reinterpret_cast<u32x4_t*>(st + so0 + i * RSTEP * LD) = ra[i];
#pragma unroll
    for (int i = 0; i < VB; ++i) *reinterpret_cast<u32x4_t*>(st + BM * LD + so0 + i * RSTEP * LD) = rb[i];
  };

  f32x4_t acc[TI][TJ];
#pragma unroll
  for (int i = 0; i < TI; ++i)
#pragma unroll
    for (int j = 0; j < TJ; ++j) acc[i][j] = (f32x4_t){0.f, 0.f, 0.f, 0.f};

  const int nkt = K / BK;
  gload();
  sstore(S);
  __syncthreads();
  const int fr = lane & 15, fq = lane >> 4;
  const unsigned aoff = (unsigned)((wm * TM + fr) * LD) + ((unsigned)(fq * 8) ^ nt_swz(fr));
  const unsigned boff = (unsigned)(BM * LD + (wn * TN + fr) * LD) + ((unsigned)(fq * 8) ^ nt_swz(fr));
  for (int kt = 0; kt < nkt; ++kt) {
    const bf16_t* cur = S + (kt & 1) * STAGE;
    if (kt + 1 < nkt) gload();
#pragma unroll
    for (int ks = 0; ks < 2; ++ks) {
      bf16x8_t a[TI];
#pragma unroll
      for (int i = 0; i < TI; ++i) a[i] = *reinterpret_cast<const bf16x8_t*>(cur + aoff + i * 16 * LD + ks * 32);
#pragma unroll
      for (int jh = 0; jh < TJ; jh += 4) {
        bf16x8_t b[4];
#pragma unroll
        for (int j = 0; j < 4; ++j) b[j] = *reinterpret_cast<const bf16x8_t*>(cur + boff + (jh + j) * 16 * LD + ks * 32);
#pragma unroll
        for (int i = 0; i < TI; ++i)
#pragma unroll
          for (int j = 0; j < 4; ++j)
            acc[i][jh + j] = __builtin_amdgcn_mfma_f32_16x16x32_bf16(b[j], a[i], acc[i][jh + j], 0, 0, 0);
      }
    }
    if (kt + 1 < nkt) sstore(S + ((kt + 1) & 1) * STAGE);
    __syncthreads();
  }
#pragma unroll
  for (int i = 0; i < TI; ++i) {
    const int m = m0 + wm * TM + i * 16 + fr;
    if (m >= M) continue;
#pragma unroll
    for (int j = 0; j < TJ; ++j) {
      const int nb = n0 + wn * TN + j * 16 + fq * 4;
      TO* cp = C + (size_t)m * ldc + nb;
      float v[4];
#pragma unroll
      for (int r = 0; r < 4; ++r) v[r] = acc[i][j][r];
      if (bias) {
        const f32x4_t bv = *reinterpret_cast<const f32x4_t*>(bias + nb);
#pragma unroll
        for (int r = 0; r < 4; ++r) v[r] += bv[r];
      }
      if constexpr (sizeof(TO) == 4) {
        if (accumulate) {
          const f32x4_t o = *reinterpret_cast<const f32x4_t*>(cp);
#pragma unroll
          for (int r = 0; r < 4; ++r) v[r] += o[r];
        }
        if (act == 1) {
#pragma unroll
          for (int r = 0; r < 4; ++r) v[r] = fmaxf(v[r], 0.f);
        }
        if (mul) {
          const f32x4_t mv = *reinterpret_cast<const f32x4_t*>(mul + (size_t)m * ldm + nb);
#pragma unroll
          for (int r = 0; r < 4; ++r) v[r] *= mv[r];
        }
        if (drop.use) {
          float mk[4];
          asr_dropout_words(drop.offset + ((size_t)m * N + nb) / 4, drop.seed, drop.keep, 1.f / drop.keep, mk);
#pragma unroll
          for (int r = 0; r < 4; ++r) v[r] *= mk[r];
        }
        *reinterpret_cast<f32x4_t*>(cp) = (f32x4_t){v[0], v[1], v[2], v[3]};
      } else {
        typedef __attribute__((ext_vector_type(4))) unsigned short us4_t;
        if (accumulate) {
          const us4_t o = *reinterpret_cast<const us4_t*>(cp);
#pragma unroll
          for (int r = 0; r < 4; ++r) v[r] += bf16_to_f32(o[r]);
        }
        if (act == 1) {
#pragma unroll
          for (int r = 0; r < 4; ++r) v[r] = fmaxf(v[r], 0.f);
        }
        *reinterpret_cast<us4_t*>(cp) = (us4_t){f32_to_bf16(v[0]), f32_to_bf16(v[1]), f32_to_bf16(v[2]), f32_to_bf16(v[3])};
      }
    }
  }
}

template <typename TO, int BM, int BN, int WM, int WN>
static void launch_gemm_nt_big(int M, int N, int K, const void* A, int lda, const void* B, int ldb, void* C, int ldc,
                               const float* bias, int accumulate, hipStream_t st, int act, const float* mul, int ldm,
                               GemmDrop drop) {
  const size_t lds = (size_t)2 * (BM + BN) * (64 + 8) * sizeof(bf16_t);
  static unsigned long long attr_done = 0;
  auto k = gemm_nt_bf16_big_kernel<TO, BM, BN, WM, WN>;
  if (first_on_device(attr_done)) {
    (void)hipFuncSetAttribute((const void*)k, hipFuncAttributeMaxDynamicSharedMemorySize, (int)lds);
  }
  const long tiles = (long)(N / BN) * ((M + BM - 1) / BM);
  hipLaunchKernelGGL(k, dim3((unsigned)tiles), dim3(WM * WN * 64), lds, st, M, N, K, (const bf16_t*)A, lda,
                     (const bf16_t*)B, ldb, (TO*)C, ldc, bias, accumulate, act, mul, ldm, drop);
}

template <typename TO>
bool try_gemm_nt_bf16(int transA, int transB, int M, int N, int K, const void* A, int lda, const void* B,
                      int ldb, void* C, int ldc, const float* bias, int accumulate, hipStream_t st, int act,
                      const float* mul, int ldm, GemmDrop drop = GemmDrop{1.f, 0, 0, 0}) {
  if (transA || !transB || K % 64 != 0 || N % 128 != 0 || M < 1024) return false;
  if (drop.use && sizeof(TO) != 4) return false;
  if (mul && (sizeof(TO) != 4 || ldm % 4 != 0 || ((uintptr_t)mul) % 16 != 0)) return false;
  if (lda % 8 != 0 || ldb % 8 != 0 || ((uintptr_t)A) % 16 != 0 || ((uintptr_t)B) % 16 != 0) return false;
  if (ldc % 4 != 0 || ((uintptr_t)C) % (4 * sizeof(TO)) != 0 || (bias && ((uintptr_t)bias) % 16 != 0)) return false;
  static const int big = [] { const char* e = getenv("ASR_GEMM_NT_BIG"); return e ? atoi(e) : 1; }();
  const bool fits32 = ((size_t)(M - 1) * lda + K) * sizeof(bf16_t) < 0xFFFFFFFFull && ((size_t)(N - 1) * ldb + K) * sizeof(bf16_t) < 0xFFFFFFFFull;
  const long tiles256 = (long)(N / 256) * ((M + 255) / 256);
  if (big && fits32 && N % 256 == 0 && (big == 2 ? M >= 2048 : tiles256 >= 512)) {
    launch_gemm_nt_big<TO, 256, 256, 2, 4>(M, N, K, A, lda, B, ldb, C, ldc, bias, accumulate, st, act, mul, ldm, drop);
    return true;
  }
  const size_t lds = (size_t)2 * (128 + 128) * (64 + 8) * sizeof(bf16_t);
  static unsigned long long attr_done = 0;
  if (first_on_device(attr_done)) {
    (void)hipFuncSetAttribute((const void*)gemm_nt_bf16_kernel<TO>, hipFuncAttributeMaxDynamicSharedMemorySize, (int)lds);
  }
  const int total = (N / 128) * ((M + 127) / 128);
  hipLaunchKernelGGL(gemm_nt_bf16_kernel<TO>, dim3(total), dim3(256), lds, st, M, N, K, (const bf16_t*)A, lda,
                     (const bf16_t*)B, ldb, (TO*)C, ldc, bias, accumulate, act, mul, ldm, drop);
  return true;
}

__device__ __forceinline__ int xcd_work_index(int skip) {
  const int b = blockIdx.x, x = b & 7;
  if (x < skip) return -1;
  return (b >> 3) * (8 - skip) + (x - skip);
}
static inline unsigned xcd_grid(long work, int skip) {
  const long per = 8 - skip;
  return (unsigned)((work + per - 1) / per * 8);
}

constexpr int SK_WAVES = 8;
struct SkinnyCell {
  const float *c_prev, *h_prev, *peep, *live, *out_mask;
  float *gates, *c_raw, *c_out, *h_out, *h_raw, *cell_out, *h_out2, *cell_out2;
  int U, ld_h2, ld_c2;
  float fb, clip;
};
__device__ __forceinline__ float sk_sigf(float x) { return 1.0f / (1.0f + expf(-x)); }
template <bool TRANSB, int NT, bool CELL = false, bool BH = false>
__global__ __launch_bounds__(64 * SK_WAVES) void gemm_skinny_f32_kernel(int M, int N, int K, const float* __restrict__ A,
                                                                        int lda, const float* __restrict__ Bm, int ldb,
                                                                        float* __restrict__ C, int ldc,
                                                                        const float* __restrict__ bias, int accumulate,
                                                                        int act, SkinnyCell cell) {
  constexpr int TN = 16 * NT;
  __shared__ float red[SK_WAVES][16][TN + 1];
  const int lane = threadIdx.x & 63, wave = threadIdx.x >> 6;
  const int col = lane & 15, rg = lane >> 4;
  const int n0 = blockIdx.x * TN, m0 = blockIdx.y * 16;
  float cl_cp = 0.f, cl_hp = 0.f, cl_lv = 0.f, cl_wci = 0.f, cl_wcf = 0.f, cl_wco = 0.f, cl_om = 1.f;
  const int cl_m = m0 + (int)threadIdx.x / (TN / 4), cl_u = n0 / 4 + (int)threadIdx.x % (TN / 4);
  const bool cl_on = CELL && (int)threadIdx.x < 16 * (TN / 4) && cl_m < M;
  if (CELL && cl_on) {
    const size_t ci = (size_t)cl_m * cell.U + cl_u;
    cl_cp = cell.c_prev[ci];
    cl_hp = cell.h_prev[ci];
    cl_lv = cell.live[cl_m];
    if (cell.peep) { cl_wci = cell.peep[cl_u]; cl_wcf = cell.peep[cell.U + cl_u]; cl_wco = cell.peep[2 * cell.U + cl_u]; }
    if (cell.out_mask) cl_om = cell.out_mask[ci];
  }
  typedef __attribute__((ext_vector_type(4))) unsigned skw4_t;
  static_assert(!BH || (TRANSB ? NT == 1 : NT == 2), "bf16 weights: NT = 2 fragment image / NT = 1 transposed rows");
  struct Frag {
    f32x4_t a[4], b[BH ? 1 : NT][BH ? 1 : 4];
    skw4_t w[BH ? (TRANSB ? 2 : 4) : 1];
    float keep;
  };
  f32x4_t acc[NT];
#pragma unroll
  for (int j = 0; j < NT; ++j) acc[j] = (f32x4_t){0.f, 0.f, 0.f, 0.f};
  const float* ap = A + (size_t)min(m0 + col, M - 1) * lda + ((BH && TRANSB) ? rg * 16 : rg * 4);
  const int units = K / 64;
  const bf16_t* Bh = reinterpret_cast<const bf16_t*>(Bm);
  auto load = [&](int round, Frag& f) {
    const int unit = wave + round * SK_WAVES;
    const bool valid = unit < units;
    const int kb = (valid ? unit : units - 1) * 64;
    f.keep = valid ? 1.f : 0.f;
    if constexpr (BH) {
      if constexpr (TRANSB) {
#pragma unroll
        for (int j = 0; j < 4; ++j) f.a[j] = *reinterpret_cast<const f32x4_t*>(ap + kb + j * 4);
        const bf16_t* bp = Bh + (size_t)(n0 + col) * ldb + kb + rg * 16;
        f.w[0] = *reinterpret_cast<const skw4_t*>(bp);
        f.w[1] = *reinterpret_cast<const skw4_t*>(bp + 8);
      } else {
#pragma unroll
        for (int j = 0; j < 4; ++j) f.a[j] = *reinterpret_cast<const f32x4_t*>(ap + kb + j * 16);
        const skw4_t* bp = reinterpret_cast<const skw4_t*>(Bh + (((size_t)blockIdx.x * units + (kb >> 6)) * 64 + lane) * 32);
#pragma unroll
        for (int j = 0; j < 4; ++j) f.w[j] = bp[j];
      }
      return;
    }
#pragma unroll
    for (int j = 0; j < 4; ++j) {
      f.a[j] = *reinterpret_cast<const f32x4_t*>(ap + kb + j * 16);
#pragma unroll
      for (int n = 0; n < NT; ++n) {
        if (TRANSB) {
          f.b[n][j] = *reinterpret_cast<const f32x4_t*>(Bm + (size_t)(n0 + n * 16 + col) * ldb + kb + j * 16 + rg * 4);
        } else {
          const float* bp = Bm + (size_t)(kb + j * 16 + rg * 4) * ldb + n0 + n * 16 + col;
#pragma unroll
          for (int e = 0; e < 4; ++e) f.b[n][j][e] = bp[(size_t)e * ldb];
        }
      }
    }
  };
  auto mma = [&](const Frag& f) {
    if constexpr (BH) {
#pragma unroll
      for (int j = 0; j < 4; ++j)
#pragma unroll
        for (int e = 0; e < 4; ++e) {
          if constexpr (TRANSB) {
            const int t = 4 * j + e;
            const unsigned wd = f.w[t >> 3][(t & 7) >> 1];
            const float bv = __uint_as_float((t & 1) ? (wd & 0xffff0000u) : (wd << 16));
            acc[0] = __builtin_amdgcn_mfma_f32_16x16x4f32(f.a[j][e] * f.keep, bv, acc[0], 0, 0, 0);
          } else {
            const unsigned wd = f.w[j][e];
            acc[0] = __builtin_amdgcn_mfma_f32_16x16x4f32(f.a[j][e] * f.keep, __uint_as_float(wd << 16), acc[0], 0, 0, 0);
            acc[NT - 1] = __builtin_amdgcn_mfma_f32_16x16x4f32(f.a[j][e] * f.keep, __uint_as_float(wd & 0xffff0000u), acc[NT - 1], 0, 0, 0);
          }
        }
      return;
    }
#pragma unroll
    for (int j = 0; j < 4; ++j)
#pragma unroll
      for (int e = 0; e < 4; ++e)
#pragma unroll
        for (int n = 0; n < NT; ++n)
          acc[n] = __builtin_amdgcn_mfma_f32_16x16x4f32(f.a[j][e] * f.keep, f.b[n][j][e], acc[n], 0, 0, 0);
  };
  Frag f0, f1;
  load(0, f0);
  if (units <= SK_WAVES) {
    mma(f0);
  } else {
    const int rounds = ((units + SK_WAVES - 1) / SK_WAVES + 1) & ~1;
    for (int r = 0; r < rounds; r += 2) {
      load(r + 1, f1);
      __builtin_amdgcn_sched_barrier(0);
      mma(f0);
      __builtin_amdgcn_sched_barrier(0);
      load(r + 2, f0);
      __builtin_amdgcn_sched_barrier(0);
      mma(f1);
      __builtin_amdgcn_sched_barrier(0);
    }
  }
#pragma unroll
  for (int n = 0; n < NT; ++n)
#pragma unroll
    for (int r = 0; r < 4; ++r) red[wave][rg * 4 + r][n * 16 + col] = acc[n][r];
  __syncthreads();
  if constexpr (CELL) {
    if (!cl_on) return;
    const int m = (int)threadIdx.x / (TN / 4), ul = (int)threadIdx.x % (TN / 4), U = cell.U;
    float p[4];
#pragma unroll
    for (int g = 0; g < 4; ++g) {
      float v = 0.f;
#pragma unroll
      for (int w = 0; w < SK_WAVES; ++w) v += red[w][m][ul * 4 + g];
      if (bias) v += bias[n0 + ul * 4 + g];
      p[g] = v;
    }
// ... 908 lines not shown
    return launch_layout<T, TO, 128, 128>(transA, transB, grid, lds, st, M, N, K, (const T*)A, lda,
                                          (const T*)B, ldb, (TO*)C, ldc, bias, accumulate, aa, ba, K, nullptr, act);
  }
  const long tiles64 = (long)((M + 63) / 64) * ((N + 63) / 64);
  int S = 1;
  if (tiles64 < 256 && K >= 16 * BK) {
    S = (int)((512 + tiles64 - 1) / tiles64);
    const int maxS = K / (4 * BK);
    if (S > maxS) S = maxS;
    if (S > 64) S = 64;
    while (S > 1 && (size_t)S * M * N * sizeof(float) > h->scratch_bytes - ASR_XCH_BYTES) --S;
  }
  size_t lds = (size_t)2 * (64 + 64) * (BK + VEC) * sizeof(T);
  if (S <= 1) {
    dim3 grid((N + 63) / 64, (M + 63) / 64);
    return launch_layout<T, TO, 64, 64>(transA, transB, grid, lds, st, M, N, K, (const T*)A, lda,
                                        (const T*)B, ldb, (TO*)C, ldc, bias, accumulate, aa, ba, K, nullptr, act);
  }
  int kchunk = (K + S - 1) / S;
  kchunk = (kchunk + BK - 1) / BK * BK;
  S = (K + kchunk - 1) / kchunk;
  dim3 grid((N + 63) / 64, (M + 63) / 64, S);
  float* partial = (float*)h->scratch;
  launch_layout<T, TO, 64, 64>(transA, transB, grid, lds, st, M, N, K, (const T*)A, lda, (const T*)B, ldb,
                               (TO*)C, ldc, nullptr, 0, aa, ba, kchunk, partial, 0);
  const size_t total = (size_t)M * N;
  int blocks = (int)((total + 255) / 256);
  if (blocks > 2048) blocks = 2048;
  hipLaunchKernelGGL(splitk_reduce_kernel<TO>, dim3(blocks), dim3(256), 0, st, partial, S, M, N, (TO*)C, ldc,
                     bias, accumulate, act, 0);
  return 0;
}

__global__ void interleave_gates_kernel(const float* __restrict__ W, const float* __restrict__ bias, int K, int U,
                                        float* __restrict__ out) {
  const size_t n = (size_t)(K + (bias ? 1 : 0)) * U;
  for (size_t i = blockIdx.x * (size_t)blockDim.x + threadIdx.x; i < n; i += (size_t)gridDim.x * blockDim.x) {
    const size_t k = i / U;
    const int u = (int)(i % U);
    const float* src = k < (size_t)K ? W + k * 4 * U : bias;
    *reinterpret_cast<f32x4_t*>(out + k * 4 * U + (size_t)u * 4) = (f32x4_t){src[u], src[U + u], src[2 * U + u], src[3 * U + u]};
  }
}

__global__ void cell_images_h_kernel(const float* __restrict__ W, const float* __restrict__ bias, int K, int U,
                                     bf16_t* __restrict__ frag, float* __restrict__ bias_il, bf16_t* __restrict__ plain) {
  const size_t n = (size_t)K * 4 * U;
  const int units = K / 64;
  for (size_t i = blockIdx.x * (size_t)blockDim.x + threadIdx.x; i < n; i += (size_t)gridDim.x * blockDim.x) {
    plain[i] = f32_to_bf16(W[i]);
    const int idx = (int)(i & 31), lane = (int)((i >> 5) & 63);
    const size_t bu = i >> 11;
    const int unit = (int)(bu % units), nb = (int)(bu / units);
    const int nn = idx & 1, je = idx >> 1, j = je >> 2, e = je & 3, rg = lane >> 4, col = lane & 15;
    const int k = unit * 64 + 16 * j + 4 * rg + e, c = nb * 32 + 16 * nn + col;
    frag[i] = f32_to_bf16(W[(size_t)k * 4 * U + (size_t)(c & 3) * U + (c >> 2)]);
    if (i < (size_t)4 * U) bias_il[i] = bias ? bias[(i & 3) * U + (i >> 2)] : 0.f;
  }
}

}

extern "C" int asr_gemm_act(asr_handle* h, int dtype, int out_dtype, int transA, int transB, int M,
                            int N, int K, const void* A, int lda, const void* B, int ldb, void* C,
                            int ldc, const float* bias, int accumulate, int act, asr_stream s);
extern "C" int asr_gemm(asr_handle* h, int dtype, int out_dtype, int transA, int transB, int M,
                        int N, int K, const void* A, int lda, const void* B, int ldb, void* C,
                        int ldc, const float* bias, int accumulate, asr_stream s) {
  return asr_gemm_act(h, dtype, out_dtype, transA, transB, M, N, K, A, lda, B, ldb, C, ldc, bias, accumulate, 0, s);
}
extern "C" int asr_gemm_act(asr_handle* h, int dtype, int out_dtype, int transA, int transB, int M,
                            int N, int K, const void* A, int lda, const void* B, int ldb, void* C,
                            int ldc, const float* bias, int accumulate, int act, asr_stream s) {
  if (!h) return ASR_ERR_INVALID_ARG;
  if (!asr_dtype_ok(dtype) || !asr_dtype_ok(out_dtype))
    ASR_FAIL(h, ASR_ERR_INVALID_ARG, "asr_gemm: bad dtype %d/%d", dtype, out_dtype);
  if (act != 0 && act != 1) ASR_FAIL(h, ASR_ERR_INVALID_ARG, "asr_gemm_act: act must be 0 (none) or 1 (relu)");
  if (M < 0 || N < 0 || K < 0 || !A || !B || !C)
    ASR_FAIL(h, ASR_ERR_INVALID_ARG, "asr_gemm: bad shape/pointer M=%d N=%d K=%d", M, N, K);
  if (lda < (transA ? M : K) || ldb < (transB ? K : N) || ldc < N)
    ASR_FAIL(h, ASR_ERR_INVALID_ARG, "asr_gemm: leading dimension too small (lda=%d ldb=%d ldc=%d)",
             lda, ldb, ldc);
  if (M == 0 || N == 0) return ASR_OK;
  hipStream_t st = (hipStream_t)s;
  if (dtype == ASR_F32 && out_dtype == ASR_F32)
    launch_gemm<float, float>(h, transA, transB, M, N, K, A, lda, B, ldb, C, ldc, bias, accumulate, st, act);
  else if (dtype == ASR_F32 && out_dtype == ASR_BF16)
    launch_gemm<float, bf16_t>(h, transA, transB, M, N, K, A, lda, B, ldb, C, ldc, bias, accumulate, st, act);
  else if (dtype == ASR_BF16 && out_dtype == ASR_F32)
    launch_gemm<bf16_t, float>(h, transA, transB, M, N, K, A, lda, B, ldb, C, ldc, bias, accumulate, st, act);
  else
    launch_gemm<bf16_t, bf16_t>(h, transA, transB, M, N, K, A, lda, B, ldb, C, ldc, bias, accumulate, st, act);
  ASR_CHECK_LAUNCH(h, "asr_gemm");
  return ASR_OK;
}

namespace {
__global__ void mul_rows_kernel(float* __restrict__ C, int ldc, const float* __restrict__ mul, int ldm, int M, int N) {
  const size_t total = (size_t)M * N;
  for (size_t i = blockIdx.x * (size_t)blockDim.x + threadIdx.x; i < total; i += (size_t)gridDim.x * blockDim.x) {
    const size_t m = i / N, n = i % N;
    C[m * ldc + n] *= mul[m * ldm + n];
  }
}
}

extern "C" int asr_gemm_mul(asr_handle* h, int dtype, int transA, int transB, int M, int N, int K, const void* A,
                            int lda, const void* B, int ldb, float* C, int ldc, const float* bias, int accumulate,
                            int act, const float* mul, int ldmul, asr_stream s) {
  if (!h) return ASR_ERR_INVALID_ARG;
  if (!mul) return asr_gemm_act(h, dtype, ASR_F32, transA, transB, M, N, K, A, lda, B, ldb, C, ldc, bias, accumulate, act, s);
  if (!asr_dtype_ok(dtype) || (act != 0 && act != 1) || M < 0 || N < 0 || K < 0 || !A || !B || !C ||
      lda < (transA ? M : K) || ldb < (transB ? K : N) || ldc < N || ldmul < N)
    ASR_FAIL(h, ASR_ERR_INVALID_ARG, "asr_gemm_mul: bad args M=%d N=%d K=%d lda=%d ldb=%d ldc=%d ldmul=%d", M, N, K, lda,
             ldb, ldc, ldmul);
  if (M == 0 || N == 0) return ASR_OK;
  hipStream_t st = (hipStream_t)s;
  bool fused = false;
  if (dtype == ASR_F32)
    launch_gemm<float, float>(h, transA, transB, M, N, K, A, lda, B, ldb, C, ldc, bias, accumulate, st, act, mul, ldmul, &fused);
  else
    launch_gemm<bf16_t, float>(h, transA, transB, M, N, K, A, lda, B, ldb, C, ldc, bias, accumulate, st, act, mul, ldmul, &fused);
  ASR_CHECK_LAUNCH(h, "asr_gemm_mul");
  if (!fused) {
    const size_t total = (size_t)M * N;
    int blocks = (int)((total + 255) / 256);
    if (blocks > 2048) blocks = 2048;
    hipLaunchKernelGGL(mul_rows_kernel, dim3(blocks), dim3(256), 0, st, C, ldc, mul, ldmul, M, N);
    ASR_CHECK_LAUNCH(h, "asr_gemm_mul(multiply)");
  }
  return ASR_OK;
}

extern "C" int asr_dropout_apply(asr_handle* h, int dtype, const void* in, void* out, size_t n, float keep_prob,
                                 uint64_t seed, uint64_t offset, asr_stream s);
extern "C" int asr_gemm_drop(asr_handle* h, int dtype, int transA, int transB, int M, int N, int K, const void* A,
                             int lda, const void* B, int ldb, float* C, int ldc, const float* bias, int accumulate,
                             int act, float keep_prob, uint64_t seed, uint64_t offset, asr_stream s) {
  if (!h) return ASR_ERR_INVALID_ARG;
  if (!asr_dtype_ok(dtype) || (act != 0 && act != 1) || M < 0 || N < 0 || K < 0 || !A || !B || !C ||
      lda < (transA ? M : K) || ldb < (transB ? K : N) || ldc != N || N % 4 != 0 || !(keep_prob > 0.f && keep_prob <= 1.f))
    ASR_FAIL(h, ASR_ERR_INVALID_ARG, "asr_gemm_drop: bad args M=%d N=%d K=%d ldc=%d (ldc == N, N %% 4 == 0)", M, N, K, ldc);
  if (M == 0 || N == 0) return ASR_OK;
  hipStream_t st = (hipStream_t)s;
  bool fused = false;
  const GemmDrop drop = {keep_prob, seed, offset, 1};
  if (dtype == ASR_F32)
    launch_gemm<float, float>(h, transA, transB, M, N, K, A, lda, B, ldb, C, ldc, bias, accumulate, st, act, nullptr, 0, &fused, drop);
  else
    launch_gemm<bf16_t, float>(h, transA, transB, M, N, K, A, lda, B, ldb, C, ldc, bias, accumulate, st, act, nullptr, 0, &fused, drop);
  ASR_CHECK_LAUNCH(h, "asr_gemm_drop");
  if (!fused) return asr_dropout_apply(h, ASR_F32, C, C, (size_t)M * N, keep_prob, seed, offset, s);
  return ASR_OK;
}

extern "C" int asr_conv3x3_prep_weights(asr_handle* h, const float* w_hwio, int Cin, int Cout, void* wt_fwd,
                                        void* wt_bwd, asr_stream s) {
  if (!h) return ASR_ERR_INVALID_ARG;
  if (!w_hwio || !wt_fwd || !wt_bwd || Cin < 1 || Cout < 1)
    ASR_FAIL(h, ASR_ERR_INVALID_ARG, "asr_conv3x3_prep_weights: bad args");
  const size_t total = (size_t)9 * Cin * Cout;
  int blocks = (int)((total + 255) / 256);
  if (blocks > 1024) blocks = 1024;
  hipLaunchKernelGGL(conv3x3_prep_kernel, dim3(blocks), dim3(256), 0, (hipStream_t)s, w_hwio, Cin, Cout,
                     (bf16_t*)wt_fwd, (bf16_t*)wt_bwd);
  ASR_CHECK_LAUNCH(h, "asr_conv3x3_prep_weights");
  return ASR_OK;
}

static unsigned long long* g_convdbg_host = nullptr;
extern "C" int asr_debug_conv_cycles(unsigned long long* out, int n) {
  if (!g_convdbg_host || n > 64 * 4 * 8) return -1;
  return hipMemcpy(out, g_convdbg_host, n * sizeof(unsigned long long), hipMemcpyDeviceToHost) == hipSuccess ? 0 : -3;
}
template <typename TO>
static int conv3x3_launch(asr_handle* h, const void* x, int Nimg, int H, int W, int Cin, const void* wt,
                          const float* bias, int Cout, int act, void* out, hipStream_t st,
                          ConvGate gate = ConvGate{nullptr, 1.f, 0, 0, 0}) {
  const long long mp = (long long)Nimg * H * W;
  if (mp <= 0 || mp >= (1ll << 31)) ASR_FAIL(h, ASR_ERR_UNSUPPORTED, "asr_conv3x3: %lld pixels", mp);
  const int Mpix = (int)mp;
  {
    static const bool img_on = [] { const char* e = getenv("ASR_CONV_IMG"); return !(e && e[0] == '0'); }();
    const size_t img_bytes = (size_t)(H + 2) * (W + 2) * (Cin * 2 + 16);
    const int nvec = H * W * Cin / 8;
    const bool shape = (Cin == 64 || Cin == 128) && (Cout == 64 || Cout == 128);
    if (img_on && shape && nvec <= 16 * 256 && img_bytes <= (size_t)156 * 1024 && Nimg >= 64) {
      const int nbuf = 2 * img_bytes <= (size_t)158 * 1024 ? 2 : 1;
      const size_t lds = nbuf * img_bytes + 128 * sizeof(float);
      const int mv = (nvec + 255) / 256;
      const unsigned grid = (unsigned)(Nimg < h->num_cu ? Nimg : h->num_cu);
      static unsigned long long* dbg_host = nullptr;
      static const bool dbg_on = [] { const char* e = getenv("ASR_CONV_DBG"); return e && e[0] == '1'; }();
      if (dbg_on && !dbg_host) {
        (void)hipMalloc(&dbg_host, 64 * 4 * 8 * sizeof(unsigned long long));
        (void)hipMemcpyToSymbol(HIP_SYMBOL(g_convdbg), &dbg_host, sizeof(dbg_host));
        g_convdbg_host = dbg_host;
      }
      const int actc = act == 2 ? (gate.use_drop == 1 ? 4 : 2) : act;
      static const bool stream_on = [] { const char* e = getenv("ASR_CONV_STREAM"); return !(e && e[0] == '0'); }();
      const bool strm = stream_on && nbuf == 2;
#define ASR_CONV_IMG_A(CI, CO, MV, AC)                                                                               \
  do {                                                                                                               \
     \
    constexpr bool SOK = CI == 64 && CO == 64 && (AC == 1 || AC == 3);                                               \
    auto k = conv3x3_img_kernel<TO, CI, CO, MV, AC, false>;                                                          \
    if constexpr (SOK) { if (strm) k = conv3x3_img_kernel<TO, CI, CO, MV, AC, false, 4, true>; }                     \
    if constexpr (AC == 1) { if (dbg_on) k = conv3x3_img_kernel<TO, CI, CO, MV, AC, true>; }                         \
    (void)hipFuncSetAttribute((const void*)k, hipFuncAttributeMaxDynamicSharedMemorySize, (int)lds);                 \
    hipLaunchKernelGGL(k, dim3(grid), dim3(256), lds, st, Nimg, H, W, (const bf16_t*)x, (const bf16_t*)wt, (TO*)out, \
                       bias, gate, nbuf);                                                                            \
  } while (0)
#define ASR_CONV_IMG8_A(CI, CO, MV, AC)                                                                              \
  do {                                                                                                               \
    auto k = conv3x3_img_kernel<TO, CI, CO, MV, AC, false, 8>;                                                       \
    (void)hipFuncSetAttribute((const void*)k, hipFuncAttributeMaxDynamicSharedMemorySize, (int)lds);                 \
    hipLaunchKernelGGL(k, dim3(grid), dim3(512), lds, st, Nimg, H, W, (const bf16_t*)x, (const bf16_t*)wt, (TO*)out, \
                       bias, gate, nbuf);                                                                            \
  } while (0)
#define ASR_CONV_IMG(CI, CO, MV)                                                                                     \
  do {                                                                                                               \
    if constexpr (sizeof(TO) == 4) { ASR_CONV_IMG_A(CI, CO, MV, 0); }                                                \
    else {                                                                                                           \
      if (actc == 1) ASR_CONV_IMG_A(CI, CO, MV, 1);                                                                  \
      else if (actc == 2) ASR_CONV_IMG_A(CI, CO, MV, 2);                                                             \
      else if (actc == 3) ASR_CONV_IMG_A(CI, CO, MV, 3);                                                             \
      else if (actc == 4) ASR_CONV_IMG_A(CI, CO, MV, 4);                                                             \
      else ASR_CONV_IMG_A(CI, CO, MV, 0);                                                                            \
    }                                                                                                                \
  } while (0)
      static const bool w8_on = [] { const char* e = getenv("ASR_CONV_IMG_W8"); return !(e && e[0] == '0'); }();
      bool done8 = false;
      if constexpr (sizeof(TO) == 2) {
        if (Cin == 64 && w8_on && mv <= 4 && actc == 3) {
          if (Cout == 64) ASR_CONV_IMG8_A(64, 64, 2, 3); else ASR_CONV_IMG8_A(64, 128, 2, 3);
          done8 = true;
        }
      }
      if (done8) {}
      else if (Cin == 64 && Cout == 64) { if (mv <= 14) ASR_CONV_IMG(64, 64, 14); else ASR_CONV_IMG(64, 64, 16); }
      else if (Cin == 64 && Cout == 128) { if (mv <= 4) ASR_CONV_IMG(64, 128, 4); else ASR_CONV_IMG(64, 128, 16); }
      else if (Cin == 128 && Cout == 128) { if (mv <= 8) ASR_CONV_IMG(128, 128, 8); else ASR_CONV_IMG(128, 128, 16); }
      else { if (mv <= 8) ASR_CONV_IMG(128, 64, 8); else ASR_CONV_IMG(128, 64, 16); }
#undef ASR_CONV_IMG
#undef ASR_CONV_IMG_A
#undef ASR_CONV_IMG8_A
      ASR_CHECK_LAUNCH(h, "asr_conv3x3(image-resident)");
      return ASR_OK;
    }
  }
  const int tm = (Mpix + 127) / 128;
  if (Cout % 128 == 0) {
    const size_t lds = (size_t)2 * (128 + 128) * 72 * sizeof(bf16_t);
    auto k = conv3x3_nt_bf16_kernel<TO, 128>;
    (void)hipFuncSetAttribute((const void*)k, hipFuncAttributeMaxDynamicSharedMemorySize, (int)lds);
    hipLaunchKernelGGL(k, dim3((unsigned)tm * (Cout / 128)), dim3(256), lds, st, Mpix, H, W, Cin, Cout,
                       (const bf16_t*)x, (const bf16_t*)wt, (TO*)out, bias, act, gate);
  } else {
    const size_t lds = (size_t)2 * (128 + 64) * 72 * sizeof(bf16_t);
    auto k = conv3x3_nt_bf16_kernel<TO, 64>;
    hipLaunchKernelGGL(k, dim3((unsigned)tm * (Cout / 64)), dim3(256), lds, st, Mpix, H, W, Cin, Cout,
                       (const bf16_t*)x, (const bf16_t*)wt, (TO*)out, bias, act, gate);
  }
  ASR_CHECK_LAUNCH(h, "asr_conv3x3");
  return ASR_OK;
}

extern "C" int asr_conv3x3_fwd(asr_handle* h, const void* x, int Nimg, int H, int W, int Cin, const void* wt_fwd,
                               const float* bias, int Cout, int relu, void* out, asr_stream s) {
  if (!h) return ASR_ERR_INVALID_ARG;
  if (!x || !wt_fwd || !out || Nimg < 1 || H < 1 || W < 1)
    ASR_FAIL(h, ASR_ERR_INVALID_ARG, "asr_conv3x3_fwd: bad args");
  if (Cin % 64 != 0 || Cout % 64 != 0)
    ASR_FAIL(h, ASR_ERR_UNSUPPORTED, "asr_conv3x3_fwd: Cin=%d, Cout=%d must be multiples of 64", Cin, Cout);
  return conv3x3_launch<bf16_t>(h, x, Nimg, H, W, Cin, wt_fwd, bias, Cout, relu ? 1 : 0, out, (hipStream_t)s);
}

extern "C" int asr_conv3x3_fwd_drop(asr_handle* h, const void* x, int Nimg, int H, int W, int Cin, const void* wt_fwd,
                                    const float* bias, int Cout, float keep_prob, uint64_t seed, uint64_t offset,
                                    void* out, asr_stream s) {
  if (!h) return ASR_ERR_INVALID_ARG;
  if (!x || !wt_fwd || !out || Nimg < 1 || H < 1 || W < 1 || !(keep_prob > 0.f && keep_prob <= 1.f))
    ASR_FAIL(h, ASR_ERR_INVALID_ARG, "asr_conv3x3_fwd_drop: bad args");
  if (Cin % 64 != 0 || Cout % 64 != 0)
    ASR_FAIL(h, ASR_ERR_UNSUPPORTED, "asr_conv3x3_fwd_drop: Cin=%d, Cout=%d must be multiples of 64", Cin, Cout);
  const ConvGate gate = {nullptr, keep_prob, seed, offset, 1};
  return conv3x3_launch<bf16_t>(h, x, Nimg, H, W, Cin, wt_fwd, bias, Cout, 3, out, (hipStream_t)s, gate);
}

extern "C" int asr_conv3x3_bwd_data(asr_handle* h, const void* dy, int Nimg, int H, int W, int Cout,
                                    const void* wt_bwd, int Cin, float* dx, asr_stream s) {
  if (!h) return ASR_ERR_INVALID_ARG;
  if (!dy || !wt_bwd || !dx || Nimg < 1 || H < 1 || W < 1)
    ASR_FAIL(h, ASR_ERR_INVALID_ARG, "asr_conv3x3_bwd_data: bad args");
  if (Cin % 64 != 0 || Cout % 64 != 0)
    ASR_FAIL(h, ASR_ERR_UNSUPPORTED, "asr_conv3x3_bwd_data: Cin=%d, Cout=%d must be multiples of 64", Cin, Cout);
  return conv3x3_launch<float>(h, dy, Nimg, H, W, Cout, wt_bwd, nullptr, Cin, 0, dx, (hipStream_t)s);
}

extern "C" int asr_conv3x3_bwd_data_relu(asr_handle* h, const void* dy, int Nimg, int H, int W, int Cout,
                                         const void* wt_bwd, int Cin, const void* act_below, float keep_prob,
                                         uint64_t seed, uint64_t offset, int use_drop, void* dpre_below, asr_stream s) {
  if (!h) return ASR_ERR_INVALID_ARG;
  if (!dy || !wt_bwd || !act_below || !dpre_below || Nimg < 1 || H < 1 || W < 1 ||
      (use_drop && !(keep_prob > 0.f && keep_prob <= 1.f)) || use_drop < 0 || use_drop > 2)
    ASR_FAIL(h, ASR_ERR_INVALID_ARG, "asr_conv3x3_bwd_data_relu: bad args");
// ... 385 lines not shown
```

tensorflow_end2end_speech_recognition_amd/models/encoders/core/blstm.py:

```python
import collections
import os as _os

import numpy as np
import torch

from .... import ops
from ...._lib import ASR_F32
from ....utils.parameter import ParamStore
from . import rnn_util
from .rnn_util import LSTMLayer, LSTMPLayer, declare_lstm_vars, declare_lstmp_vars

WARM_BPTT = _os.environ.get('ASR_WARM_BPTT', '1') != '0'
ENC_HALVES = _os.environ.get('ASR_ENC_HALVES', '0') == '1'
PIPE_LANE = 6

LSTMStateTuple = collections.namedtuple('LSTMStateTuple', ('c', 'h'))

LSTM_IMPLS = ('BasicLSTMCell', 'LSTMCell', 'LSTMBlockCell', 'LSTMBlockFusedCell', 'CudnnLSTM')


class _RecurrentEncoderBase(object):
    ndir = 2
    scope_fmt = 'blstm_hidden%d'

    def __init__(self, num_units, num_proj, num_layers, lstm_impl, use_peephole, parameter_init,
                 clip_activation, time_major=True, name='lstm_encoder', dtype=ASR_F32, seed=0):
        assert num_proj != 0
        if lstm_impl not in LSTM_IMPLS:
            raise IndexError('lstm_impl is "BasicLSTMCell" or "LSTMCell" or "LSTMBlockCell" or '
                             '"LSTMBlockFusedCell" or "CudnnLSTM".')
        self.num_units = num_units
        self.num_proj = num_proj if lstm_impl == 'LSTMCell' else None
        if self.num_proj is not None and type(self).__name__ not in ('BLSTMEncoder', 'LSTMEncoder', 'VGGBLSTMEncoder',
                                                                     'VGGLSTMEncoder', 'MultitaskBLSTMEncoder',
                                                                     'MultitaskLSTMEncoder', 'CLDNNEncoder'):
            raise ValueError('LSTMCell projection layers (num_proj) are implemented for the blstm / lstm / vgg_* / '
                             'multitask_* / cldnn_wang encoders, not for %s' % type(self).__name__)
        self.num_layers = num_layers
        self.lstm_impl = lstm_impl
        self.use_peephole = bool(use_peephole) and lstm_impl != 'BasicLSTMCell'
        self.parameter_init = parameter_init
        self.clip_activation = None if lstm_impl == 'BasicLSTMCell' else clip_activation
        self.time_major = time_major
        self.name = name
        self.dtype = ops.dtype_id(dtype)
        self.layer_dtype = self.dtype
        if self.num_proj is not None:
            self.dtype = ASR_F32
        self.seed = seed
        self.layers = None
        self.store = None
        self.scope_prefix = ''
        self.num_layers_sub = None
        self.grad_ready_hook = None
        self.side_extra = None
        self.side_extra_event = None
        self.want_f32_outputs = True
        self.halves = ENC_HALVES
        self.layers_b = None
        self._split = 0

    def build(self, store, input_dim, rng, scope_prefix=''):
        self.store = store
        self.scope_prefix = scope_prefix
        self.layers = []
        din = input_dim
        H = self.num_units
        if self.num_proj is not None:
            P = int(self.num_proj)
            for i in range(1, self.num_layers + 1):
                bases = self._declare_projected(store, i, din, P, rng)
                self.layers.append(LSTMPLayer(store, bases, din, H, P, self.use_peephole, 1.0, self.clip_activation,
                                              dtype=self.layer_dtype))
                din = self.ndir * P
            self.output_dim = self.ndir * P
            return self.output_dim
        for i in range(1, self.num_layers + 1):
            bases = self._declare(store, i, din, rng)
            self.layers.append(LSTMLayer(store, bases, din, H, self.use_peephole, 1.0,
                                         self.clip_activation))
            din = self.ndir * H
        self.output_dim = self.ndir * H
        return self.output_dim

    def _declare_projected(self, store, i, din, P, rng):
        scope = self.scope_prefix + (self.scope_fmt % i)
        return declare_lstmp_vars(store, scope, din, self.num_units, P, self.ndir, self.use_peephole,
                                  self.parameter_init, rng)

    def _declare(self, store, i, din, rng):
        scope = self.scope_prefix + (self.scope_fmt % i)
        return declare_lstm_vars(store, scope, din, self.num_units, self.ndir, self.use_peephole,
                                 self.parameter_init, rng)

    def _ensure_built(self, inputs):
        if self.layers is None:
            store = ParamStore(inputs.device)
            self.build(store, inputs.shape[-1], np.random.RandomState(self.seed))
            store.finalize()

    def __call__(self, inputs, inputs_seq_len, keep_prob, is_training, drop_masks=None, rng_state=None):
        self._ensure_built(inputs)
        if self.num_proj is not None:
            return self._call_projected(inputs, inputs_seq_len, keep_prob, is_training, drop_masks, rng_state)
        B, T, _ = inputs.shape
        self.pad_b = (-B) % 16
        if self.pad_b:
            inputs = torch.cat([inputs, inputs.new_zeros(self.pad_b, T, inputs.shape[2])], 0)
            inputs_seq_len = torch.cat([inputs_seq_len, inputs_seq_len.new_zeros(self.pad_b)], 0)
        self.batch = B
        seq_len = inputs_seq_len.to(torch.int32).contiguous()
        Tt, Bp = T, inputs.shape[0]
        D = inputs.shape[2]
        ldk0 = (D + 63) // 64 * 64 if self.dtype != ASR_F32 else D

        if rng_state is None and drop_masks is None and is_training and keep_prob is not None and keep_prob < 1.0:
            self._dropout_calls = getattr(self, '_dropout_calls', 0) + 1
            rng_state = (self.seed, self._dropout_calls << 40)

        def rs_of(li):
            return (rng_state[0], rng_state[1] + li * (1 << 32)) if rng_state is not None else None

        preps, ready_w, ready_m = [], [], []
        with ops.side_lane(inputs.device):
            for li, layer in enumerate(self.layers):
                preps.append(layer.prepare(inputs.device, self.dtype, Tt, Bp, 1.0, False, None, None,
                                           ldk=ldk0 if li == 0 else None))
                ready_w.append(ops.stream_event())
            self.side_extra_event = None
            if self.side_extra is not None:
                self.side_extra()
                self.side_extra_event = ops.stream_event()
            for li, layer in enumerate(self.layers):
                dm = drop_masks[li] if drop_masks is not None else None
                preps[li]['mask'] = layer.make_mask(inputs.device, Tt, Bp, keep_prob, is_training, rs_of(li), dm)
                ready_m.append(ops.stream_event())
        self._split = self._split_rows(Bp) if drop_masks is None else 0
        if self._split:
            x, finals = self._forward_halves(inputs, seq_len, preps, ready_w, ready_m, keep_prob, is_training, ldk0)
            return self._finish_call(x, finals, seq_len, B)
        x = ops.bt_to_tb(inputs.contiguous(), self.dtype, ld=ldk0)
        final = None
        finals = []
        for li, layer in enumerate(self.layers):
            if not rnn_util.FORK_ONCE or li == 0:
                ops.wait_event(ready_w[li])
            elif li == 1:
                ops.wait_event(ready_w[-1])
            x, final = layer.forward(x, seq_len, self.dtype, keep_prob, is_training, prep=preps[li],
                                     mask_event=ready_m[li])
            finals.append(final)
            if self.num_layers_sub is not None and li + 1 == self.num_layers_sub:
                self._out_sub_op, self._final_sub_ch = x, final
        return self._finish_call(x, finals, seq_len, B)

    def _finish_call(self, x, finals, seq_len, B):
        self.seq_len_padded = seq_len
        self._out_op = x
        out = ops.cast_to_f32(x) if (x.dtype != torch.float32 and self.want_f32_outputs) else x
        self._out_tm = out
        cf, hf = finals[-1]
        self._final_ch = (cf, hf)
        self._finals = finals
        final_state = self._state_tuple(finals, len(finals))
        out_user = out[:, :B]
        if not self.time_major:
            out_user = out_user.transpose(0, 1)
        return out_user, final_state

    def _split_rows(self, Bp):
        tiles = Bp // 16
        if not self.halves or tiles < 2 or self.num_proj is not None or self.num_layers_sub is not None:
            return 0
        return ((tiles + 1) // 2) * 16

    def _twins(self):
        if self.layers_b is None:
            self.layers_b = [LSTMLayer(l.store, l.bases, l.din, l.H, l.use_peephole, l.forget_bias, l.cell_clip)
                             for l in self.layers]
        return self.layers_b

    @staticmethod
    def _second_mask(mask):
        return (mask[0], mask[1], mask[2] + (1 << 30)) if isinstance(mask, tuple) else mask

    def _forward_halves(self, inputs, seq_len, preps, ready_w, ready_m, keep_prob, is_training, ldk0):
        dev = inputs.device
        B0, Bp = self._split, inputs.shape[0]
        parts = ((0, B0, self.layers), (B0, Bp, self._twins()))
        start = ops.stream_event()
        xs, fins = [None, None], [[], []]
        sl = [seq_len[lo:hi].contiguous() for lo, hi, _ in parts]
        for li in range(len(self.layers)):
            for h, (lo, hi, layers) in enumerate(parts):
                ctx = ops.side_lane(dev, keep=(inputs, seq_len, sl[1]), lane=PIPE_LANE, after=start) if h else _NoLane()
                with ctx:
                    if li == 0:
                        xs[h] = ops.bt_to_tb(inputs[lo:hi].contiguous(), self.dtype, ld=ldk0)
                        ops.wait_event(ready_w[-1] if h else ready_w[0])
                    elif not h:
                        if not rnn_util.FORK_ONCE:
                            ops.wait_event(ready_w[li])
                        elif li == 1:
                            ops.wait_event(ready_w[-1])
                    prep = preps[li] if not h else dict(preps[li], mask=self._second_mask(preps[li]['mask']))
                    xs[h], fin = layers[li].forward(xs[h], sl[h], self.dtype, keep_prob, is_training, prep=prep,
                                                    mask_event=ready_m[li])
                    fins[h].append(fin)
                    if h and li + 1 == len(self.layers):
                        done = ops.stream_event()
        ops.wait_event(done)
        ops.keep_on_lane(dev, PIPE_LANE, (xs[1],) + tuple(t for f in fins[1] for t in f))
        x = torch.cat([xs[0], xs[1]], 1)
        finals = []
        for li, (a, b) in enumerate(zip(fins[0], fins[1])):
            need = self.ndir == 1 or li + 1 == len(self.layers)
            finals.append((torch.cat([a[0], b[0]], 1), torch.cat([a[1], b[1]], 1)) if need else (None, None))
        return x, finals

    def _call_projected(self, inputs, inputs_seq_len, keep_prob, is_training, drop_masks, rng_state):
        B, T, _ = inputs.shape
        self.pad_b, self.batch = 0, B
        seq_len = inputs_seq_len.to(torch.int32).contiguous()
        x = ops.bt_to_tb(inputs.contiguous(), ASR_F32)
        if rng_state is None and drop_masks is None and is_training and keep_prob is not None and keep_prob < 1.0:
            self._dropout_calls = getattr(self, '_dropout_calls', 0) + 1
            rng_state = (self.seed, self._dropout_calls << 40)
        finals = []
        for li, layer in enumerate(self.layers):
            mask = None
            if is_training and drop_masks is not None:
                mask = drop_masks[li]
            elif is_training and rng_state is not None and keep_prob < 1.0:
                mask = ops.dropout_mask((T, B, self.ndir * layer.P), keep_prob, rng_state[0],
                                        rng_state[1] + li * (1 << 32), x.device)
            x, fin = layer.forward(x, seq_len, mask)
            finals.append(fin)
            if self.num_layers_sub is not None and li + 1 == self.num_layers_sub:
                self._out_sub_op, self._final_sub_ch = x, fin
        self.seq_len_padded = seq_len
        self._out_op = self._out_tm = x
        self._finals = finals
        self._final_ch = None
        out_user = x if self.time_major else x.transpose(0, 1)
        return out_user, self._state_tuple_projected(finals, len(finals))

    def _state_tuple_projected(self, finals, upto):
        if self.ndir == 2:
            return tuple(LSTMStateTuple(c, m) for c, m in finals[upto - 1])
        return tuple(LSTMStateTuple(*f[0]) for f in finals[:upto])

    def _state_tuple(self, finals, upto):
        B = self.batch
        if self.ndir == 2:
            cf, hf = finals[upto - 1]
            return tuple(LSTMStateTuple(cf[d, :B], hf[d, :B]) for d in range(2))
        return tuple(LSTMStateTuple(cf[0, :B], hf[0, :B]) for cf, hf in finals[:upto])

    def backward(self, d_outputs, d_final=None, need_input_grad=False, d_outputs_sub=None):
        if self.num_proj is not None:
            dx = d_outputs
            for li in reversed(range(len(self.layers))):
                if d_outputs_sub is not None and li == self.num_layers_sub - 1:
                    dx = torch.add(dx, d_outputs_sub)
                dx = self.layers[li].backward(dx.contiguous(), None, need_dx=(li > 0 or need_input_grad))
                if self.grad_ready_hook is not None:
                    self.grad_ready_hook(li, self.layers[li])
            ops.join_side(d_outputs.device)
            return dx
        if self._split:
            return self._backward_halves(d_outputs, d_final, need_input_grad)
        dx = d_outputs
        masked = False
        for li in reversed(range(len(self.layers))):
            if d_outputs_sub is not None and li == self.num_layers_sub - 1:
                dx = torch.add(dx, d_outputs_sub)
            dcf = dhf = None
            if d_final is not None and li == len(self.layers) - 1:
                dcf, dhf = d_final
            below = self.layers[li - 1].ctx['mask'] if li > 0 else None
            if d_outputs_sub is not None and li - 1 == self.num_layers_sub - 1:
                below = None
            cb = self.layers[li - 1].ctx if (li > 0 and WARM_BPTT) else None
            if cb is not None and (cb['gates'].numel() * cb['gates'].element_size() +
                                   cb['cs'].numel() * cb['cs'].element_size()) > (128 << 20):
                cb = None
            dx = self.layers[li].backward(dx.contiguous(), dcf, dhf, need_dx=(li > 0 or need_input_grad),
                                          dout_masked=masked, dx_mask=below, background=(li > 0),
                                          warm=(cb['gates'], cb['cs']) if cb is not None else None)
            ops.wait_event(getattr(self.layers[li], 'warm_event', None))
            masked = below is not None
            if self.grad_ready_hook is not None:
                self.grad_ready_hook(li, self.layers[li])
        ops.join_side(d_outputs.device)
        return dx


    def _backward_halves(self, d_outputs, d_final, need_input_grad):
        dev = d_outputs.device
        B0 = self._split
        dxs = [d_outputs[:, :B0].contiguous(), d_outputs[:, B0:].contiguous()]
        dfin = [(None, None), (None, None)]
        if d_final is not None:
            dcf, dhf = d_final
            dfin = [(dcf[:, :B0].contiguous(), dhf[:, :B0].contiguous()), (dcf[:, B0:].contiguous(), dhf[:, B0:].contiguous())]
        start = ops.stream_event()
        stacks = (self.layers, self.layers_b)
        masked = [False, False]
        top = len(self.layers) - 1
        for li in reversed(range(len(self.layers))):
            acc = None
            for h, layers in enumerate(stacks):
                ctx = ops.side_lane(dev, keep=(dxs[1],) + dfin[1], lane=PIPE_LANE, after=start) if h else _NoLane()
                with ctx:
                    below = layers[li - 1].ctx['mask'] if li > 0 else None
                    cb = layers[li - 1].ctx if (li > 0 and WARM_BPTT) else None
                    if cb is not None and (cb['gates'].numel() * cb['gates'].element_size() +
                                           cb['cs'].numel() * cb['cs'].element_size()) > (64 << 20):
                        cb = None
                    dcf, dhf = dfin[h] if li == top else (None, None)
                    dxs[h] = layers[li].backward(dxs[h].contiguous(), dcf, dhf, need_dx=(li > 0 or need_input_grad),
                                                 dout_masked=masked[h], dx_mask=below, background=(li > 0),
                                                 warm=(cb['gates'], cb['cs']) if cb is not None else None,
                                                 acc=acc, finish=bool(h))
                    ops.wait_event(getattr(layers[li], 'warm_event', None))
                    masked[h] = below is not None
                    if not h:
                        acc = layers[li].acc
                        layers[li].acc = None
                    elif li == 0:
                        done = ops.stream_event()
            if self.grad_ready_hook is not None:
                self.grad_ready_hook(li, self.layers_b[li])
        ops.wait_event(done)
        ops.join_side(dev)
        if not need_input_grad:
            return None
        return torch.cat([dxs[0], dxs[1]], 1)


class _NoLane(object):

    def __enter__(self):
        return self

    def __exit__(self, *exc):
        return False


class BLSTMEncoder(_RecurrentEncoderBase):
    ndir = 2
    scope_fmt = 'blstm_hidden%d'
```

tensorflow_end2end_speech_recognition_amd/models/encoders/core/rnn_util.py:

```python
import os as _os

import numpy as np
import torch

from .... import ops
from ...._lib import ASR_BF16, ASR_F32

DIRS = ('fw', 'bw')
DW_LANES = 2
FORK_ONCE = _os.environ.get('ASR_FORK_ONCE', '1') != '0'
BG_WGS = int(_os.environ.get('ASR_BG_WGS', '128'))
DW_AFTER_DX_FLOPS = {'0': float('inf'), '1': 0.0}.get(_os.environ.get('ASR_DW_AFTER_DX', ''), 2e11)


def declare_lstm_vars(store, scope, din, H, ndir, use_peephole, parameter_init, rng, cell_scope=None):
    names = []
    for d in range(ndir):
        base = '%s/%s/lstm_cell' % (scope, DIRS[d]) if cell_scope is None else cell_scope
        u = lambda *s: rng.uniform(-parameter_init, parameter_init, size=s)
        store.declare(base + '/kernel', (din + H, 4 * H), u(din + H, 4 * H))
        store.declare(base + '/bias', (4 * H,), np.zeros(4 * H))
        if use_peephole:
            store.declare(base + '/w_i_diag', (H,), u(H))
            store.declare(base + '/w_f_diag', (H,), u(H))
            store.declare(base + '/w_o_diag', (H,), u(H))
        names.append(base)
    return names


class LSTMLayer(object):
    def __init__(self, store, bases, din, H, use_peephole, forget_bias=1.0, cell_clip=None):
        self.store = store
        self.bases = bases
        self.ndir = len(bases)
        self.din, self.H = din, H
        self.use_peephole = use_peephole
        self.forget_bias = forget_bias
        self.cell_clip = cell_clip
        self.ctx = None
        self.grad_event = None

    def _vars(self, view):
        rows = []
        for b in self.bases:
            row = [view(b + '/kernel'), view(b + '/bias')]
            row += [view(b + '/w_i_diag'), view(b + '/w_f_diag'), view(b + '/w_o_diag')] if self.use_peephole \
                else [None, None, None]
            rows.append(tuple(row))
        return rows

    def prepare(self, device, dtype, T, B, keep_prob=1.0, is_training=True, rng_state=None, drop_mask=None,
                ldk=None):
        w = ops.lstm_prep_layer(self._vars(self.store.__getitem__), self.din, self.H, dtype, ldk=ldk)
        w['mask'] = self.make_mask(device, T, B, keep_prob, is_training, rng_state, drop_mask)
        return w

    def make_mask(self, device, T, B, keep_prob=1.0, is_training=True, rng_state=None, drop_mask=None):
        if not (is_training and (drop_mask is not None or keep_prob < 1.0)):
            return None
        if drop_mask is not None:
            return drop_mask
        seed, offset = rng_state
        return (float(keep_prob), int(seed), int(offset))

    @staticmethod
    def _masked(t, mask):
        return ops.dropout_apply(t, *mask) if isinstance(mask, tuple) else ops.apply_mask(t, mask)

    def forward(self, x, seq_len, dtype, keep_prob=1.0, is_training=True, rng_state=None,
                drop_mask=None, save=True, prep=None, mask_event=None):
        T, B, ldk = x.shape
        H, ndir = self.H, self.ndir
        if prep is None:
            prep = self.prepare(x.device, dtype, T, B, keep_prob, is_training, rng_state, drop_mask, ldk=ldk)
        xproj = torch.empty((T, B, ndir * 4 * H), dtype=torch.float32, device=x.device)
        ops.gemm(x.view(T * B, ldk), prep['wxT'], transB=True, bias=prep['bias'],
                 out=xproj.view(T * B, ndir * 4 * H))
        gates, hout, cs, cf, hf = ops.lstm_fwd(xproj, prep['whf'], prep['peep'], seq_len, H, ndir, dtype,
                                               self.forget_bias, self.cell_clip or 0.0)
        out = hout
        mask = prep['mask']
        if mask is not None:
            if not isinstance(mask, tuple):
                ops.wait_event(mask_event)
            out = self._masked(hout, mask)
        if save:
            self.ctx = dict(x=x, gates=gates, cs=cs, hout=hout, whb=prep['whb'], peep=prep['peep'],
                            seq_len=seq_len, dtype=dtype, mask=mask, wx_cat=prep['wx_cat'])
        return out, (cf, hf)

    def backward(self, dout, d_c_final=None, d_h_final=None, need_dx=True, dout_masked=False, dx_mask=None,
                 background=False, warm=None, acc=None, finish=True):
        c = self.ctx
        st = self.store
        dtype = c['dtype']
        x, hout = c['x'], c['hout']
        T, B, ldk = x.shape
        din, H, ndir = self.din, self.H, self.ndir
        if c['mask'] is not None and not dout_masked:
            dout = self._masked(dout, c['mask'])
        dgates, dpeep = ops.lstm_bwd(dout, c['gates'], c['cs'], c['whb'], c['peep'], c['seq_len'], H,
                                     ndir, dtype, d_c_final, d_h_final, want_dpeep=True)
        self.warm_event = None
        fork = ops.stream_event() if FORK_ONCE else None
        if warm:
            with ops.side_lane(dout.device, keep=tuple(warm), lane=2, after=fork):
                for t in warm:
                    ops.touch(t)
                if not FORK_ONCE:
                    self.warm_event = ops.stream_event()
        x2d = x.view(T * B, ldk)[:, :din]
        h2d = hout.view(T * B, ndir * H)
        dg2d = dgates.view(T * B, ndir * 4 * H)
        dx = torch.empty((T, B, din), dtype=torch.float32, device=x.device) if need_dx else None
        if need_dx:
            if isinstance(dx_mask, tuple):
                ops.gemm(dg2d, c['wx_cat'], transB=True, out=dx.view(T * B, din), drop=dx_mask)
            else:
                ops.gemm(dg2d, c['wx_cat'], transB=True, out=dx.view(T * B, din),
                         mul=dx_mask.view(T * B, din) if dx_mask is not None else None)
            if FORK_ONCE and background and 2.0 * T * B * din * ndir * 4 * H >= DW_AFTER_DX_FLOPS:
                fork = ops.stream_event()
        add = acc is not None
        dw_il = acc['dw_il'] if add else \
            torch.empty((ndir, din + H, 4 * H), dtype=torch.float32, device=x.device)
        ops.set_side_gemm_workgroups(x.device, BG_WGS if background else 0)
        done = []
        for d in range(ndir):
            with ops.side_lane(x.device, keep=(x, hout, dgates, dpeep, dw_il), lane=1 + (d % DW_LANES), after=fork):
                dg = dg2d[:, d * 4 * H:(d + 1) * 4 * H]
                ops.gemm(x2d, dg, transA=True, out=dw_il[d, :din], accumulate=add)
                if T > 1:
                    if d == 0:
                        ops.gemm(h2d[:(T - 1) * B, d * H:(d + 1) * H], dg[B:], transA=True, out=dw_il[d, din:],
                                 accumulate=add)
                    else:
                        ops.gemm(h2d[B:, d * H:(d + 1) * H], dg[:(T - 1) * B], transA=True, out=dw_il[d, din:],
                                 accumulate=add)
                elif not add:
                    dw_il[d, din:].zero_()
                if d % DW_LANES > 0:
                    done.append(ops.stream_event())
        if not finish:
            self.acc = dict(dw_il=dw_il, dpeep=dpeep)
            self.ctx = None
            return dx
        with ops.side_lane(x.device, keep=(dpeep,), lane=1, after=fork):
            for ev in done:
                ops.wait_event(ev)
            if add:
                dpeep = acc['dpeep'] + dpeep
                ops.keep_on_lane(x.device, 1, (dpeep,))
            ops.lstm_grad_finish(self._vars(st.g), dw_il, dpeep, H)
            self.grad_event = ops.stream_event()
        self.ctx = None
        return dx

    def var_names(self):
        names = []
        for b in self.bases:
            names += [b + '/kernel', b + '/bias']
            if self.use_peephole:
                names += [b + '/w_i_diag', b + '/w_f_diag', b + '/w_o_diag']
        return names


def declare_lstmp_vars(store, scope, din, H, P, ndir, use_peephole, parameter_init, rng, cell_scope=None):
    names = []
    for d in range(ndir):
        base = '%s/%s/lstm_cell' % (scope, DIRS[d]) if cell_scope is None else cell_scope
        u = lambda *s: rng.uniform(-parameter_init, parameter_init, size=s)
        store.declare(base + '/kernel', (din + P, 4 * H), u(din + P, 4 * H))
        store.declare(base + '/bias', (4 * H,), np.zeros(4 * H))
        if use_peephole:
            store.declare(base + '/w_f_diag', (H,), u(H))
            store.declare(base + '/w_i_diag', (H,), u(H))
            store.declare(base + '/w_o_diag', (H,), u(H))
        store.declare(base + '/projection/kernel', (H, P), u(H, P))
        names.append(base)
    return names


class LSTMPLayer(object):
    def __init__(self, store, bases, din, H, P, use_peephole, forget_bias=1.0, cell_clip=None, dtype=ASR_F32):
        self.store, self.bases = store, bases
        self.ndir = len(bases)
        self.din, self.H, self.P = din, H, P
        self.dtype = dtype
        self.use_peephole = use_peephole
        self.forget_bias, self.cell_clip = forget_bias, cell_clip
        self.ctx = None
        self.grad_event = None

    def var_names(self):
        names = []
        for b in self.bases:
            names += [b + '/kernel', b + '/bias']
            if self.use_peephole:
                names += [b + '/w_f_diag', b + '/w_i_diag', b + '/w_o_diag']
            names.append(b + '/projection/kernel')
        return names

    def _peep(self, b):
        st = self.store
        if not self.use_peephole:
            return None
        return torch.stack([st[b + '/w_i_diag'], st[b + '/w_f_diag'], st[b + '/w_o_diag']]).contiguous()

    @staticmethod
    def _frames(seq_len, T, reverse):
        B = seq_len.shape[0]
        s = torch.arange(T, device=seq_len.device).unsqueeze(1)
        L = seq_len.to(torch.int64).unsqueeze(0)
        live = s < L
        src = torch.where(live, L - 1 - s, s) if reverse else s.expand(T, B)
        return src.contiguous(), live.to(torch.float32).contiguous()

    def _vars(self, view):
        rows = []
        for b in self.bases:
            row = [view(b + '/kernel'), view(b + '/bias')]
            row += [view(b + '/w_i_diag'), view(b + '/w_f_diag'), view(b + '/w_o_diag')] if self.use_peephole \
                else [None, None, None]
            rows.append(tuple(row))
        return rows

    def fused(self):
        return _os.environ.get('ASR_LSTMP_FUSED', '1') != '0' and ops.lstm_units_supported(self.H)

    def operand_dtype(self):
        if self.dtype == ASR_BF16 and self.din % 8 == 0 and self.P % 8 == 0 and \
                _os.environ.get('ASR_LSTMP_BF16', '1') != '0':
            return ASR_BF16
        return ASR_F32

    def _forward_fused(self, x, seq_len, mask, save):
        st = self.store
        T, B, din = x.shape
        H, P, ndir = self.H, self.P, self.ndir
        dev = x.device
        Bp = (B + 15) // 16 * 16
        if Bp != B:
            x = torch.cat([x, x.new_zeros((T, Bp - B, din))], 1)
            seq_len = torch.cat([seq_len, seq_len.new_zeros((Bp - B,))])
        dt = self.operand_dtype()
        lo = dt != ASR_F32
        x = ops.cast_from_f32(x.contiguous(), dt) if lo else x.contiguous()
        rows = []
        for b, v in zip(self.bases, self._vars(st.__getitem__)):
            kf = torch.empty((din + P + H, 4 * H), dtype=torch.float32, device=dev)
            kf[:din + P].copy_(v[0])
            ops.gemm(st[b + '/projection/kernel'], v[0][din:], out=kf[din + P:])
            rows.append((kf,) + v[1:])
        prep = ops.lstm_prep_layer(rows, din + P, H, dt)
        xproj = torch.empty((T, Bp, ndir * 4 * H), dtype=torch.float32, device=dev)
        ops.gemm(x.view(T * Bp, din), prep['wxT'][:, :din], transB=True, bias=prep['bias'],
                 out=xproj.view(T * Bp, ndir * 4 * H))
        gates, hout, cs, cf, hf = ops.lstm_fwd(xproj, prep['whf'], prep['peep'], seq_len, H, ndir, dt,
                                               self.forget_bias, self.cell_clip or 0.0)
        m = torch.empty((T, Bp, ndir * P), dtype=hout.dtype, device=dev)
        finals, wps = [], []
        for d, b in enumerate(self.bases):
            wp = st[b + '/projection/kernel']
            wps.append(ops.cast_from_f32(wp, dt) if lo else wp)
            ops.gemm(hout.view(T * Bp, ndir * H)[:, d * H:(d + 1) * H], wps[d], out=m.view(T * Bp, ndir * P)[:, d * P:(d + 1) * P])
            finals.append((cf[d, :B], ops.gemm(hf[d], wp)[:B]))
        mo = ops.cast_to_f32(m) if lo else m
        out = mo[:, :B].contiguous() if Bp != B else mo
        res = out if mask is None else ops.apply_mask(out, mask)
        if save:
            self.ctx = dict(fused=True, x=x, m=m, hout=hout, hf=hf, gates=gates, cs=cs, whb=prep['whb'], peep=prep['peep'],
                            wx_cat=prep['wx_cat'], seq_len=seq_len, mask=mask, batch=B, dt=dt, wps=wps)
        return res, finals
# ... 177 lines not shown
```

tensorflow_end2end_speech_recognition_amd/ops.py:

```python
import ctypes as C
import os
import time as _time

import numpy as np
import torch

from . import _lib
from ._lib import ASR_BF16, ASR_F32

TORCH_DTYPE = {ASR_F32: torch.float32, ASR_BF16: torch.bfloat16}


def dtype_id(dtype):
    if dtype in (ASR_F32, 'f32', 'fp32', 'float32', torch.float32):
        return ASR_F32
    if dtype in (ASR_BF16, 'bf16', 'bfloat16', torch.bfloat16):
        return ASR_BF16
    raise ValueError('dtype must be f32 or bf16, got %r' % (dtype,))


_lane = 0
_side = {}


# ... 168 lines not shown

def host_ints(x):
    if not torch.is_tensor(x):
        return np.asarray(x)
    if not x.is_cuda:
        return x.detach().numpy()
    import weakref
    hit = _host_copies.get(id(x))
    if hit is not None and hit[0]() is x and hit[1] == x._version:
        return hit[2]
    if len(_host_copies) > 64:
        for k in [k for k, v in _host_copies.items() if v[0]() is None]:
            del _host_copies[k]
        if len(_host_copies) > 64:
            _host_copies.clear()
    host = x.detach().cpu().numpy()
    _host_copies[id(x)] = (weakref.ref(x), x._version, host)
    return host


def invalidate_host_ints(x=None):
    if x is None:
        _host_copies.clear()
    else:
        _host_copies.pop(id(x), None)


def _p(t):
    if t is None:
        return None
    if not t.is_contiguous():
        raise ValueError('tensor must be contiguous')
    return C.c_void_p(t.data_ptr())


def _chk(t, dtype, name):
    if t.dtype != dtype:
        raise ValueError('%s must be %s, got %s' % (name, dtype, t.dtype))


def bt_to_tb(x_btd, dtype=ASR_F32, ld=None):
    h = _h(x_btd)
    _chk(x_btd, torch.float32, 'inputs')
    B, T, D = x_btd.shape
    ld = D if ld is None else int(ld)
    out = torch.empty((T, B, ld), dtype=TORCH_DTYPE[dtype], device=x_btd.device)
    h.check(h.lib.asr_bt_to_tb_ld(h.h, dtype, _p(x_btd), _p(out), B, T, D, ld, _s()), 'asr_bt_to_tb')
    return out


def stack_frames(x_btf, seq_len, num_stack, num_skip):
    h = _h(x_btf)
    _chk(x_btf, torch.float32, 'inputs')
    _chk(seq_len, torch.int32, 'seq_len')
    if num_stack < num_skip:
        raise ValueError('num_skip must be less than num_stack.')
    B, T, F = x_btf.shape
    Tn = (T + num_skip - 1) // num_skip
    out = torch.empty((B, Tn, F * num_stack), dtype=torch.float32, device=x_btf.device)
    out_len = torch.empty((B,), dtype=torch.int32, device=x_btf.device)
    h.check(h.lib.asr_stack_frames(h.h, _p(x_btf), _p(seq_len), B, T, F, int(num_stack), int(num_skip), _p(out),
                                   _p(out_len), _s()), 'asr_stack_frames')
    return out, out_len


def splice(x_btd, seq_len, splice, num_stack=1):
    h = _h(x_btd)
    _chk(x_btd, torch.float32, 'inputs')
    _chk(seq_len, torch.int32, 'seq_len')
    B, T, D = x_btd.shape
    if D % (3 * num_stack) != 0:
        raise ValueError('frame width must be channels*3*num_stack')
    out = torch.empty((B, T, D * splice), dtype=torch.float32, device=x_btd.device)
    h.check(h.lib.asr_splice(h.h, _p(x_btd), _p(seq_len), B, T, D, int(splice), int(num_stack), _p(out), _s()),
            'asr_splice')
    return out


def transpose2d(x, out=None):
    h = _h(x)
    dt = dtype_id(x.dtype)
    if x.dim() != 2 or x.stride(1) != 1:
        raise ValueError('transpose2d: 2-D tensor with unit inner stride expected')
    R, Cc = x.shape
    if out is None:
        out = torch.empty((Cc, R), dtype=x.dtype, device=x.device)
    h.check(h.lib.asr_transpose2d(h.h, dt, C.c_void_p(x.data_ptr()), R, Cc, x.stride(0),
                                  C.c_void_p(out.data_ptr()), out.stride(0), _s()), 'asr_transpose2d')
    return out


def cast_from_f32(x, dtype, out=None):
    h = _h(x)
    _chk(x, torch.float32, 'x')
    if out is None:
        out = torch.empty(x.shape, dtype=TORCH_DTYPE[dtype], device=x.device)
    h.check(h.lib.asr_cast_from_f32(h.h, dtype, _p(x), _p(out), x.numel(), _s()), 'asr_cast_from_f32')
    return out


def cast_to_f32(x, out=None):
    h = _h(x)
    dt = dtype_id(x.dtype)
    if out is None:
        out = torch.empty(x.shape, dtype=torch.float32, device=x.device)
    h.check(h.lib.asr_cast_to_f32(h.h, dt, _p(x), _p(out), x.numel(), _s()), 'asr_cast_to_f32')
    return out


def apply_mask(x, mask, out=None):
    h = _h(x)
    dt = dtype_id(x.dtype)
    _chk(mask, torch.float32, 'mask')
    if out is None:
        out = torch.empty_like(x)
    h.check(h.lib.asr_apply_mask(h.h, dt, _p(x), _p(mask), _p(out), x.numel(), _s()), 'asr_apply_mask')
    return out


def dropout_mask(shape, keep_prob, seed, offset, device):
    mask = torch.empty(shape, dtype=torch.float32, device=device)
    h = _h(mask)
    h.check(h.lib.asr_dropout_mask(h.h, _p(mask), mask.numel(), float(keep_prob), int(seed),
                                   int(offset), _s()), 'asr_dropout_mask')
    return mask


def touch(t):
    h = _h(t)
    h.check(h.lib.asr_touch(h.h, _p(t), t.numel() * t.element_size(), _s()), 'asr_touch')


def dropout_apply(x, keep_prob, seed, offset):
    h = _h(x)
    out = torch.empty_like(x)
    h.check(h.lib.asr_dropout_apply(h.h, dtype_id(x.dtype), _p(x), _p(out), x.numel(), float(keep_prob), int(seed),
                                    int(offset), _s()), 'asr_dropout_apply')
    return out


def colsum(a, out=None):
    h = _h(a)
    dt = dtype_id(a.dtype)
    M, N = a.shape
    if a.stride(1) != 1:
        raise ValueError('colsum: inner stride must be 1')
    if out is None:
        out = torch.empty((N,), dtype=torch.float32, device=a.device)
    h.check(h.lib.asr_colsum(h.h, dt, C.c_void_p(a.data_ptr()), M, N, a.stride(0), _p(out), _s()),
            'asr_colsum')
    return out


def gemm(A, B, transA=False, transB=False, bias=None, out=None, out_dtype=None, accumulate=False, relu=False,
         mul=None, drop=None):
    h = _h(A)
    dt = dtype_id(A.dtype)
    if B.dtype != A.dtype:
        raise ValueError('gemm: A and B dtypes differ')
    for t, n in ((A, 'A'), (B, 'B')):
        if t.dim() != 2 or t.stride(1) != 1:
            raise ValueError('gemm: %s must be 2-D with unit inner stride' % n)
    M, K = (A.shape[1], A.shape[0]) if transA else (A.shape[0], A.shape[1])
    Kb, N = (B.shape[1], B.shape[0]) if transB else (B.shape[0], B.shape[1])
    if K != Kb:
        raise ValueError('gemm: inner dimensions differ (%d vs %d)' % (K, Kb))
    odt = dt if out_dtype is None else dtype_id(out_dtype)
    if out is None:
        out = torch.empty((M, N), dtype=TORCH_DTYPE[odt], device=A.device)
    else:
        odt = dtype_id(out.dtype)
        if out.shape != (M, N) or out.stride(1) != 1:
            raise ValueError('gemm: bad out shape %s' % (tuple(out.shape),))
    if bias is not None:
        _chk(bias, torch.float32, 'bias')
    if drop is not None:
        if odt != ASR_F32 or not out.is_contiguous() or N % 4:
            raise ValueError('gemm: drop needs a contiguous fp32 output with N % 4 == 0')
        h.check(h.lib.asr_gemm_drop(h.h, dt, int(transA), int(transB), M, N, K,
                                    C.c_void_p(A.data_ptr()), A.stride(0), C.c_void_p(B.data_ptr()), B.stride(0),
                                    C.c_void_p(out.data_ptr()), out.stride(0), _p(bias), int(accumulate),
                                    1 if relu else 0, float(drop[0]), int(drop[1]), int(drop[2]), _s()), 'asr_gemm_drop')
        return out
    if mul is not None:
        _chk(mul, torch.float32, 'mul')
        if odt != ASR_F32 or mul.dim() != 2 or mul.shape != (M, N) or mul.stride(1) != 1:
            raise ValueError('gemm: mul needs an fp32 output and an fp32 [M,N] multiplier')
        h.check(h.lib.asr_gemm_mul(h.h, dt, int(transA), int(transB), M, N, K,
                                   C.c_void_p(A.data_ptr()), A.stride(0), C.c_void_p(B.data_ptr()), B.stride(0),
                                   C.c_void_p(out.data_ptr()), out.stride(0), _p(bias), int(accumulate),
                                   1 if relu else 0, C.c_void_p(mul.data_ptr()), mul.stride(0), _s()), 'asr_gemm_mul')
        return out
    h.check(h.lib.asr_gemm_act(h.h, dt, odt, int(transA), int(transB), M, N, K,
                               C.c_void_p(A.data_ptr()), A.stride(0), C.c_void_p(B.data_ptr()), B.stride(0),
                               C.c_void_p(out.data_ptr()), out.stride(0), _p(bias), int(accumulate),
                               1 if relu else 0, _s()), 'asr_gemm')
    return out


def conv3x3_prep_weights(w_hwio):
    h = _h(w_hwio)
    _chk(w_hwio, torch.float32, 'w')
    _, _, Cin, Cout = w_hwio.shape
    wf = torch.empty((Cout, 9 * Cin), dtype=torch.bfloat16, device=w_hwio.device)
    wb = torch.empty((Cin, 9 * Cout), dtype=torch.bfloat16, device=w_hwio.device)
    h.check(h.lib.asr_conv3x3_prep_weights(h.h, _p(w_hwio.contiguous()), Cin, Cout, _p(wf), _p(wb), _s()),
            'asr_conv3x3_prep_weights')
    return wf, wb


def _out_like(out, shape, dtype, device, what):
    if out is None:
        return torch.empty(shape, dtype=dtype, device=device)
    if tuple(out.shape) != tuple(shape) or out.dtype != dtype or not out.is_contiguous():
        raise ValueError('%s: out must be a contiguous %s tensor of shape %s' % (what, dtype, tuple(shape)))
    return out


def conv3x3_fwd(x_nhwc, wt_fwd, bias, relu=True, out=None):
    h = _h(x_nhwc)
    _chk(x_nhwc, torch.bfloat16, 'x')
    N, H, W, Cin = x_nhwc.shape
    Cout = wt_fwd.shape[0]
    out = _out_like(out, (N, H, W, Cout), torch.bfloat16, x_nhwc.device, 'conv3x3_fwd')
    h.check(h.lib.asr_conv3x3_fwd(h.h, _p(x_nhwc), N, H, W, Cin, _p(wt_fwd), _p(bias), Cout, 1 if relu else 0,
                                  _p(out), _s()), 'asr_conv3x3_fwd')
    return out


def conv3x3_fwd_drop(x_nhwc, wt_fwd, bias, drop, out=None):
    h = _h(x_nhwc)
    _chk(x_nhwc, torch.bfloat16, 'x')
    N, H, W, Cin = x_nhwc.shape
    Cout = wt_fwd.shape[0]
    out = _out_like(out, (N, H, W, Cout), torch.bfloat16, x_nhwc.device, 'conv3x3_fwd_drop')
    h.check(h.lib.asr_conv3x3_fwd_drop(h.h, _p(x_nhwc), N, H, W, Cin, _p(wt_fwd), _p(bias), Cout, float(drop[0]),
                                       int(drop[1]), int(drop[2]), _p(out), _s()), 'asr_conv3x3_fwd_drop')
    return out


def conv3x3_bwd_data(dy_nhwc, wt_bwd):
    h = _h(dy_nhwc)
    _chk(dy_nhwc, torch.bfloat16, 'dy')
    N, H, W, Cout = dy_nhwc.shape
    Cin = wt_bwd.shape[0]
    dx = torch.empty((N, H, W, Cin), dtype=torch.float32, device=dy_nhwc.device)
    h.check(h.lib.asr_conv3x3_bwd_data(h.h, _p(dy_nhwc), N, H, W, Cout, _p(wt_bwd), Cin, _p(dx), _s()),
            'asr_conv3x3_bwd_data')
    return dx


def conv3x3_smallc_fwd(x_nhwc, w2d, bias, relu=True):
    h = _h(x_nhwc)
    _chk(x_nhwc, torch.bfloat16, 'x')
    _chk(w2d, torch.bfloat16, 'w2d')
    N, H, W, Cin = x_nhwc.shape
    out = torch.empty((N, H, W, w2d.shape[1]), dtype=torch.bfloat16, device=x_nhwc.device)
    h.check(h.lib.asr_conv3x3_smallc_fwd(h.h, _p(x_nhwc), N, H, W, Cin, _p(w2d), _p(bias), w2d.shape[1], int(relu),
                                         _p(out), _s()), 'asr_conv3x3_smallc_fwd')
    return out


def conv3x3_smallc_fwd_drop(x_nhwc, w2d, bias, drop, out=None):
    h = _h(x_nhwc)
    _chk(x_nhwc, torch.bfloat16, 'x')
    _chk(w2d, torch.bfloat16, 'w2d')
    N, H, W, Cin = x_nhwc.shape
    out = _out_like(out, (N, H, W, w2d.shape[1]), torch.bfloat16, x_nhwc.device, 'conv3x3_smallc_fwd_drop')
    h.check(h.lib.asr_conv3x3_smallc_fwd_drop(h.h, _p(x_nhwc), N, H, W, Cin, _p(w2d), _p(bias), w2d.shape[1],
                                              float(drop[0]), int(drop[1]), int(drop[2]), _p(out), _s()),
            'asr_conv3x3_smallc_fwd_drop')
    return out


def conv3x3_smallc_bwd_weight(x_nhwc, dpre_nhwc, dw):
    h = _h(x_nhwc)
    _chk(x_nhwc, torch.bfloat16, 'x')
    _chk(dpre_nhwc, torch.bfloat16, 'dpre')
    N, H, W, Cin = x_nhwc.shape
    h.check(h.lib.asr_conv3x3_smallc_bwd_weight(h.h, _p(x_nhwc), _p(dpre_nhwc), N, H, W, Cin, dpre_nhwc.shape[-1],
                                                _p(dw), _s()), 'asr_conv3x3_smallc_bwd_weight')
    return dw


def conv3x3_smallc_bwd_weight_bias(x_nhwc, dpre_nhwc, dw, dbias):
    h = _h(x_nhwc)
    _chk(x_nhwc, torch.bfloat16, 'x')
    _chk(dpre_nhwc, torch.bfloat16, 'dpre')
    _chk(dbias, torch.float32, 'dbias')
    N, H, W, Cin = x_nhwc.shape
    if dbias.numel() != dpre_nhwc.shape[-1]:
        raise ValueError('conv3x3_smallc_bwd_weight_bias: dbias has %d elements' % dbias.numel())
    h.check(h.lib.asr_conv3x3_smallc_bwd_weight_bias(h.h, _p(x_nhwc), _p(dpre_nhwc), N, H, W, Cin, dpre_nhwc.shape[-1],
                                                     _p(dw), _p(dbias), _s()), 'asr_conv3x3_smallc_bwd_weight_bias')
    return dw, dbias


def conv3x3_bwd_data_relu(dy_nhwc, wt_bwd, act_below, drop=None, dropped=False):
    h = _h(dy_nhwc)
    _chk(dy_nhwc, torch.bfloat16, 'dy')
    _chk(act_below, torch.bfloat16, 'act_below')
    N, H, W, Cout = dy_nhwc.shape
    Cin = wt_bwd.shape[0]
    dpre = torch.empty((N, H, W, Cin), dtype=torch.bfloat16, device=dy_nhwc.device)
    k, sd, off = drop if drop is not None else (1.0, 0, 0)
    mode = 0 if drop is None else (2 if dropped else 1)
    h.check(h.lib.asr_conv3x3_bwd_data_relu(h.h, _p(dy_nhwc), N, H, W, Cout, _p(wt_bwd), Cin, _p(act_below), float(k),
                                            int(sd), int(off), mode, _p(dpre), _s()),
            'asr_conv3x3_bwd_data_relu')
    return dpre


def conv3x3_bwd_weight(x_nhwc, dy_nhwc, dw, accumulate=False):
    h = _h(x_nhwc)
    _chk(x_nhwc, torch.bfloat16, 'x')
    _chk(dy_nhwc, torch.bfloat16, 'dy')
    N, H, W, Cin = x_nhwc.shape
    Cout = dy_nhwc.shape[3]
    h.check(h.lib.asr_conv3x3_bwd_weight(h.h, _p(x_nhwc), _p(dy_nhwc), N, H, W, Cin, Cout, _p(dw),
                                         int(accumulate), _s()), 'asr_conv3x3_bwd_weight')
    return dw


def conv3x3_bwd_weight_bias(x_nhwc, dy_nhwc, dw, dbias):
    h = _h(x_nhwc)
    _chk(x_nhwc, torch.bfloat16, 'x')
    _chk(dy_nhwc, torch.bfloat16, 'dy')
    _chk(dbias, torch.float32, 'dbias')
# ... 1147 lines not shown
```

Before: 721,000 frames/s.

## Skip padded timesteps in BLSTM input and dx GEMMs via device row lists

Adds a kernel that builds, on the GPU, a compacted list of valid (t,b) rows from seq_len, plus a row-gathering variant of the bf16 NT GEMM kernels that reads only listed rows and exits surplus workgroups early. The BLSTM forward input projection and the backward dx GEMMs use this path by default, so rows past each utterance's length are no longer computed. Because lengths are drawn from 100 to 778 and padded to the batch maximum, a large share of rows is padding. Padded output rows are left unwritten, so correctness depends on downstream kernels masking by seq_len. The grid is still sized for the full M, and each row load adds an indirection.

New measurement: 727,600 frames/s, median of 6. No clear change (+0.9%).

```diff
diff --git a/include/asr_hip.h b/include/asr_hip.h
--- a/include/asr_hip.h
+++ b/include/asr_hip.h
@@ -73,6 +73,12 @@
 int asr_gemm_drop(asr_handle* h, int dtype, int transA, int transB, int M, int N, int K, const void* A, int lda,
                   const void* B, int ldb, float* C, int ldc, const float* bias, int accumulate, int act, float keep_prob,
                   uint64_t seed, uint64_t offset, asr_stream s);
+
+int asr_valid_rows(asr_handle* h, const int32_t* seq_len, int T, int B, int32_t* rows, int32_t* count, asr_stream s);
+int asr_gemm_rows(asr_handle* h, int dtype, int out_dtype, int transA, int transB, int M, int N, int K,
+                  const void* A, int lda, const void* B, int ldb, void* C, int ldc, const float* bias, int accumulate,
+                  int act, const float* mul, int ldmul, int use_drop, float keep_prob, uint64_t seed, uint64_t offset,
+                  const int32_t* rows, const int32_t* nrows, asr_stream s);
 
 int asr_im2col3x3(asr_handle* h, int dtype, const void* in, int N, int H, int W, int Cin, int ldp,
                   void* patches, asr_stream s);
diff --git a/tensorflow_end2end_speech_recognition_amd/_lib.py b/tensorflow_end2end_speech_recognition_amd/_lib.py
--- a/tensorflow_end2end_speech_recognition_amd/_lib.py
+++ b/tensorflow_end2end_speech_recognition_amd/_lib.py
@@ -36,6 +36,9 @@
     'asr_gemm_act': (_i, [_vp, _i, _i, _i, _i, _i, _i, _i, _vp, _i, _vp, _i, _vp, _i, _vp, _i, _i, _vp]),
     'asr_gemm_drop': (_i, [_vp, _i, _i, _i, _i, _i, _i, _vp, _i, _vp, _i, _vp, _i, _vp, _i, _i, _f, _u64, _u64, _vp]),
     'asr_gemm_mul': (_i, [_vp, _i, _i, _i, _i, _i, _i, _vp, _i, _vp, _i, _vp, _i, _vp, _i, _i, _vp, _i, _vp]),
+    'asr_valid_rows': (_i, [_vp, _vp, _i, _i, _vp, _vp, _vp]),
+    'asr_gemm_rows': (_i, [_vp, _i, _i, _i, _i, _i, _i, _i, _vp, _i, _vp, _i, _vp, _i, _vp, _i, _i, _vp, _i, _i, _f, _u64,
+                           _u64, _vp, _vp, _vp]),
     'asr_conv3x3_prep_weights': (_i, [_vp, _vp, _i, _i, _vp, _vp, _vp]),
     'asr_conv3x3_fwd': (_i, [_vp, _vp, _i, _i, _i, _i, _vp, _vp, _i, _i, _vp, _vp]),
     'asr_conv3x3_fwd_drop': (_i, [_vp, _vp, _i, _i, _i, _i, _vp, _vp, _i, _f, _u64, _u64, _vp, _vp]),
diff --git a/tensorflow_end2end_speech_recognition_amd/csrc/elementwise.hip b/tensorflow_end2end_speech_recognition_amd/csrc/elementwise.hip
--- a/tensorflow_end2end_speech_recognition_amd/csrc/elementwise.hip
+++ b/tensorflow_end2end_speech_recognition_amd/csrc/elementwise.hip
@@ -207,6 +207,20 @@
       }
     }
   }
+}
+
+__global__ void valid_rows_kernel(const int32_t* __restrict__ seq_len, int T, int B, int* __restrict__ rows,
+                                  int* __restrict__ count) {
+  const int t = blockIdx.x * blockDim.x + threadIdx.x;
+  if (t > T) return;
+  int base = 0;
+  for (int b = 0; b < B; ++b) base += min(max(seq_len[b], 0), t);
+  if (t == T) {
+    *count = base;
+    return;
+  }
+  for (int b = 0; b < B; ++b)
+    if (t < seq_len[b]) rows[base++] = t * B + b;
 }
 
 __global__ void touch_kernel(const f32x4_t* __restrict__ p, size_t n16, unsigned* __restrict__ sink) {
@@ -676,6 +690,14 @@
   ASR_CHECK_LAUNCH(h, "asr_touch");
   return ASR_OK;
 }
+extern "C" int asr_valid_rows(asr_handle* h, const int32_t* seq_len, int T, int B, int32_t* rows, int32_t* count,
+                              asr_stream s) {
+  if (!h) return ASR_ERR_INVALID_ARG;
+  ASR_NEED(seq_len && rows && count && T >= 0 && B > 0 && (long long)T * B < (1ll << 31), "asr_valid_rows: bad args");
+  hipLaunchKernelGGL(valid_rows_kernel, dim3((unsigned)(T / 256 + 1)), dim3(256), 0, (hipStream_t)s, seq_len, T, B, rows, count);
+  ASR_CHECK_LAUNCH(h, "asr_valid_rows");
+  return ASR_OK;
+}
 extern "C" int asr_colsum(asr_handle* h, int dtype, const void* a, int M, int N, int lda, float* out, asr_stream s) {
   if (!h) return ASR_ERR_INVALID_ARG;
   ASR_NEED(asr_dtype_ok(dtype) && a && out && M >= 0 && N > 0 && lda >= N, "asr_colsum: bad args");
diff --git a/tensorflow_end2end_speech_recognition_amd/csrc/gemm.hip b/tensorflow_end2end_speech_recognition_amd/csrc/gemm.hip
--- a/tensorflow_end2end_speech_recognition_amd/csrc/gemm.hip
+++ b/tensorflow_end2end_speech_recognition_amd/csrc/gemm.hip
@@ -234,13 +234,20 @@
   int use;
 };
 
-template <typename TO>
+template <bool RL>
+__device__ __forceinline__ int nt_row(const int* __restrict__ rows, int m, int M) {
+  if constexpr (RL) return (int)min((unsigned)rows[m], (unsigned)(M - 1));
+  else return m;
+}
+
+template <typename TO, bool RL = false>
 __global__ __launch_bounds__(256) void gemm_nt_bf16_kernel(int M, int N, int K, const bf16_t* __restrict__ A,
                                                            int lda, const bf16_t* __restrict__ Bt, int ldb,
                                                            TO* __restrict__ C, int ldc,
                                                            const float* __restrict__ bias, int accumulate,
                                                            int act, const float* __restrict__ mul, int ldm,
-                                                           GemmDrop drop) {
+                                                           GemmDrop drop, const int* __restrict__ rows,
+                                                           const int* __restrict__ nrows) {
   constexpr int BM = 128, BN = 128, BK = 64, LD = BK + 8;
   constexpr int STAGE = (BM + BN) * LD;
   extern __shared__ __attribute__((aligned(16))) char smem[];
@@ -248,7 +255,12 @@
 
   const int tid = threadIdx.x, lane = tid & 63, wave = tid >> 6;
   const int wm = wave >> 1, wn = wave & 1;
-  const int ntn = N / BN, ntm = (M + BM - 1) / BM, total = ntn * ntm;
+  int Mv = M;
+  if constexpr (RL) Mv = min(max(*nrows, 0), M);
+  const int ntn = N / BN, ntm = (Mv + BM - 1) / BM, total = ntn * ntm;
+  if constexpr (RL) {
+    if ((int)blockIdx.x >= total) return;
+  }
   int t = blockIdx.x;
   if ((total & 7) == 0) t = (t & 7) * (total >> 3) + (t >> 3);
   const int m0 = (t / ntn) * BM, n0 = (t % ntn) * BN;
@@ -259,7 +271,7 @@
 #pragma unroll
   for (int i = 0; i < 4; ++i) {
     const int v = tid + i * 256, r = v >> 3, kv = (v & 7) * 8;
-    pa[i] = A + (size_t)min(m0 + r, M - 1) * lda + kv;
+    pa[i] = A + (size_t)nt_row<RL>(rows, min(m0 + r, Mv - 1), M) * lda + kv;
     pb[i] = Bt + (size_t)(n0 + r) * ldb + kv;
     so[i] = (unsigned)(r * LD) + ((unsigned)kv ^ nt_swz(r));
   }
@@ -315,8 +327,9 @@
   }
 #pragma unroll
   for (int i = 0; i < 4; ++i) {
-    const int m = m0 + wm * 64 + i * 16 + fr;
-    if (m >= M) continue;
+    const int mt = m0 + wm * 64 + i * 16 + fr;
+    if (mt >= Mv) continue;
+    const int m = nt_row<RL>(rows, mt, M);
 #pragma unroll
     for (int j = 0; j < 4; ++j) {
       const int nb = n0 + wn * 64 + j * 16 + fq * 4;
@@ -368,13 +381,14 @@
   }
 }
 
-template <typename TO, int BM, int BN, int WM, int WN>
+template <typename TO, int BM, int BN, int WM, int WN, bool RL = false>
 __global__ __launch_bounds__(WM * WN * 64, 1) void gemm_nt_bf16_big_kernel(int M, int N, int K, const bf16_t* __restrict__ A,
                                                                            int lda, const bf16_t* __restrict__ Bt, int ldb,
                                                                            TO* __restrict__ C, int ldc,
                                                                            const float* __restrict__ bias, int accumulate,
                                                                            int act, const float* __restrict__ mul, int ldm,
-                                                                           GemmDrop drop) {
+                                                                           GemmDrop drop, const int* __restrict__ rows,
+                                                                           const int* __restrict__ nrows) {
   constexpr int BK = 64, LD = BK + 8, NT = WM * WN * 64;
   constexpr int STAGE = (BM + BN) * LD;
   constexpr int TM = BM / WM, TN = BN / WN, TI = TM / 16, TJ = TN / 16;
@@ -384,7 +398,12 @@
 
   const int tid = threadIdx.x, lane = tid & 63, wave = tid >> 6;
   const int wm = wave / WN, wn = wave % WN;
-  const int ntn = N / BN, ntm = (M + BM - 1) / BM, total = ntn * ntm;
+  int Mv = M;
+  if constexpr (RL) Mv = min(max(*nrows, 0), M);
+  const int ntn = N / BN, ntm = (Mv + BM - 1) / BM, total = ntn * ntm;
+  if constexpr (RL) {
+    if ((int)blockIdx.x >= total) return;
+  }
   int t = blockIdx.x;
   if ((total & 7) == 0) t = (t & 7) * (total >> 3) + (t >> 3);
   const int m0 = (t / ntn) * BM, n0 = (t % ntn) * BN;
@@ -392,7 +411,7 @@
   const int r0 = tid >> 3, kv = (tid & 7) * 8;
   unsigned oa[VA], ob[VB];
 #pragma unroll
-  for (int i = 0; i < VA; ++i) oa[i] = (unsigned)(((size_t)min(m0 + r0 + RSTEP * i, M - 1) * lda + kv) * sizeof(bf16_t));
+  for (int i = 0; i < VA; ++i) oa[i] = (unsigned)(((size_t)nt_row<RL>(rows, min(m0 + r0 + RSTEP * i, Mv - 1), M) * lda + kv) * sizeof(bf16_t));
 #pragma unroll
   for (int i = 0; i < VB; ++i) ob[i] = (unsigned)(((size_t)(n0 + r0 + RSTEP * i) * ldb + kv) * sizeof(bf16_t));
   const unsigned so0 = (unsigned)(r0 * LD) + ((unsigned)kv ^ nt_swz(r0));
@@ -455,8 +474,9 @@
   }
 #pragma unroll
   for (int i = 0; i < TI; ++i) {
-    const int m = m0 + wm * TM + i * 16 + fr;
-    if (m >= M) continue;
+    const int mt = m0 + wm * TM + i * 16 + fr;
+    if (mt >= Mv) continue;
+    const int m = nt_row<RL>(rows, mt, M);
 #pragma unroll
     for (int j = 0; j < TJ; ++j) {
       const int nb = n0 + wn * TN + j * 16 + fq * 4;
@@ -508,25 +528,26 @@
   }
 }
 
-template <typename TO, int BM, int BN, int WM, int WN>
+template <typename TO, int BM, int BN, int WM, int WN, bool RL = false>
 static void launch_gemm_nt_big(int M, int N, int K, const void* A, int lda, const void* B, int ldb, void* C, int ldc,
                                const float* bias, int accumulate, hipStream_t st, int act, const float* mul, int ldm,
-                               GemmDrop drop) {
+                               GemmDrop drop, const int* rows = nullptr, const int* nrows = nullptr) {
   const size_t lds = (size_t)2 * (BM + BN) * (64 + 8) * sizeof(bf16_t);
   static unsigned long long attr_done = 0;
-  auto k = gemm_nt_bf16_big_kernel<TO, BM, BN, WM, WN>;
+  auto k = gemm_nt_bf16_big_kernel<TO, BM, BN, WM, WN, RL>;
   if (first_on_device(attr_done)) {
     (void)hipFuncSetAttribute((const void*)k, hipFuncAttributeMaxDynamicSharedMemorySize, (int)lds);
   }
   const long tiles = (long)(N / BN) * ((M + BM - 1) / BM);
   hipLaunchKernelGGL(k, dim3((unsigned)tiles), dim3(WM * WN * 64), lds, st, M, N, K, (const bf16_t*)A, lda,
-                     (const bf16_t*)B, ldb, (TO*)C, ldc, bias, accumulate, act, mul, ldm, drop);
+                     (const bf16_t*)B, ldb, (TO*)C, ldc, bias, accumulate, act, mul, ldm, drop, rows, nrows);
 }
 
 template <typename TO>
 bool try_gemm_nt_bf16(int transA, int transB, int M, int N, int K, const void* A, int lda, const void* B,
                       int ldb, void* C, int ldc, const float* bias, int accumulate, hipStream_t st, int act,
-                      const float* mul, int ldm, GemmDrop drop = GemmDrop{1.f, 0, 0, 0}) {
+                      const float* mul, int ldm, GemmDrop drop = GemmDrop{1.f, 0, 0, 0}, const int* rows = nullptr,
+                      const int* nrows = nullptr) {
   if (transA || !transB || K % 64 != 0 || N % 128 != 0 || M < 1024) return false;
   if (drop.use && sizeof(TO) != 4) return false;
   if (mul && (sizeof(TO) != 4 || ldm % 4 != 0 || ((uintptr_t)mul) % 16 != 0)) return false;
@@ -536,17 +557,27 @@
   const bool fits32 = ((size_t)(M - 1) * lda + K) * sizeof(bf16_t) < 0xFFFFFFFFull && ((size_t)(N - 1) * ldb + K) * sizeof(bf16_t) < 0xFFFFFFFFull;
   const long tiles256 = (long)(N / 256) * ((M + 255) / 256);
   if (big && fits32 && N % 256 == 0 && (big == 2 ? M >= 2048 : tiles256 >= 512)) {
-    launch_gemm_nt_big<TO, 256, 256, 2, 4>(M, N, K, A, lda, B, ldb, C, ldc, bias, accumulate, st, act, mul, ldm, drop);
+    if (rows)
+      launch_gemm_nt_big<TO, 256, 256, 2, 4, true>(M, N, K, A, lda, B, ldb, C, ldc, bias, accumulate, st, act, mul, ldm, drop,
+                                                   rows, nrows);
+    else
+      launch_gemm_nt_big<TO, 256, 256, 2, 4>(M, N, K, A, lda, B, ldb, C, ldc, bias, accumulate, st, act, mul, ldm, drop);
     return true;
   }
   const size_t lds = (size_t)2 * (128 + 128) * (64 + 8) * sizeof(bf16_t);
   static unsigned long long attr_done = 0;
   if (first_on_device(attr_done)) {
     (void)hipFuncSetAttribute((const void*)gemm_nt_bf16_kernel<TO>, hipFuncAttributeMaxDynamicSharedMemorySize, (int)lds);
+    (void)hipFuncSetAttribute((const void*)gemm_nt_bf16_kernel<TO, true>, hipFuncAttributeMaxDynamicSharedMemorySize, (int)lds);
   }
   const int total = (N / 128) * ((M + 127) / 128);
-  hipLaunchKernelGGL(gemm_nt_bf16_kernel<TO>, dim3(total), dim3(256), lds, st, M, N, K, (const bf16_t*)A, lda,
-                     (const bf16_t*)B, ldb, (TO*)C, ldc, bias, accumulate, act, mul, ldm, drop);
+  if (rows)
+    hipLaunchKernelGGL((gemm_nt_bf16_kernel<TO, true>), dim3(total), dim3(256), lds, st, M, N, K, (const bf16_t*)A, lda,
+                       (const bf16_t*)B, ldb, (TO*)C, ldc, bias, accumulate, act, mul, ldm, drop, rows, nrows);
+  else
+    hipLaunchKernelGGL(gemm_nt_bf16_kernel<TO>, dim3(total), dim3(256), lds, st, M, N, K, (const bf16_t*)A, lda,
+                       (const bf16_t*)B, ldb, (TO*)C, ldc, bias, accumulate, act, mul, ldm, drop, (const int*)nullptr,
+                       (const int*)nullptr);
   return true;
 }
 
@@ -1761,6 +1792,36 @@
   ASR_CHECK_LAUNCH(h, "asr_gemm_drop");
   if (!fused) return asr_dropout_apply(h, ASR_F32, C, C, (size_t)M * N, keep_prob, seed, offset, s);
   return ASR_OK;
+}
+
+extern "C" int asr_gemm_rows(asr_handle* h, int dtype, int out_dtype, int transA, int transB, int M, int N, int K,
+                             const void* A, int lda, const void* B, int ldb, void* C, int ldc, const float* bias,
+                             int accumulate, int act, const float* mul, int ldmul, int use_drop, float keep_prob,
+                             uint64_t seed, uint64_t offset, const int32_t* rows, const int32_t* nrows, asr_stream s) {
+  if (!h) return ASR_ERR_INVALID_ARG;
+  if ((rows == nullptr) != (nrows == nullptr) || (mul && use_drop) || ((mul || use_drop) && out_dtype != ASR_F32))
+    ASR_FAIL(h, ASR_ERR_INVALID_ARG, "asr_gemm_rows: rows and nrows go together; mul / drop need an fp32 output, one of them");
+  if (rows && dtype == ASR_BF16 && asr_dtype_ok(out_dtype) && (act == 0 || act == 1) && M > 0 && N > 0 && K >= 0 && A && B &&
+      C && lda >= (transA ? M : K) && ldb >= (transB ? K : N) && ldc >= N && (!mul || ldmul >= N) &&
+      (!use_drop || (ldc == N && N % 4 == 0 && keep_prob > 0.f && keep_prob <= 1.f))) {
+    hipStream_t st = (hipStream_t)s;
+    const GemmDrop drop = {use_drop ? keep_prob : 1.f, use_drop ? seed : 0, use_drop ? offset : 0, use_drop ? 1 : 0};
+    const bool took = out_dtype == ASR_F32
+        ? try_gemm_nt_bf16<float>(transA, transB, M, N, K, A, lda, B, ldb, C, ldc, bias, accumulate, st, act, mul, ldmul, drop,
+                                  rows, nrows)
+        : try_gemm_nt_bf16<bf16_t>(transA, transB, M, N, K, A, lda, B, ldb, C, ldc, bias, accumulate, st, act, nullptr, 0,
+                                   drop, rows, nrows);
+    if (took) {
+      ASR_CHECK_LAUNCH(h, "asr_gemm_rows");
+      return ASR_OK;
+    }
+  }
+  if (use_drop)
+    return asr_gemm_drop(h, dtype, transA, transB, M, N, K, A, lda, B, ldb, (float*)C, ldc, bias, accumulate, act, keep_prob,
+                         seed, offset, s);
+  if (mul)
+    return asr_gemm_mul(h, dtype, transA, transB, M, N, K, A, lda, B, ldb, (float*)C, ldc, bias, accumulate, act, mul, ldmul, s);
+  return asr_gemm_act(h, dtype, out_dtype, transA, transB, M, N, K, A, lda, B, ldb, C, ldc, bias, accumulate, act, s);
 }
 
 extern "C" int asr_conv3x3_prep_weights(asr_handle* h, const float* w_hwio, int Cin, int Cout, void* wt_fwd,
diff --git a/tensorflow_end2end_speech_recognition_amd/models/encoders/core/blstm.py b/tensorflow_end2end_speech_recognition_amd/models/encoders/core/blstm.py
--- a/tensorflow_end2end_speech_recognition_amd/models/encoders/core/blstm.py
+++ b/tensorflow_end2end_speech_recognition_amd/models/encoders/core/blstm.py
@@ -59,6 +59,7 @@
         self.halves = ENC_HALVES
         self.layers_b = None
         self._split = 0
+        self._rows = None
 
     def build(self, store, input_dim, rng, scope_prefix=''):
         self.store = store
@@ -122,7 +123,12 @@
             return (rng_state[0], rng_state[1] + li * (1 << 32)) if rng_state is not None else None
 
         preps, ready_w, ready_m = [], [], []
+        self._rows = None
+        ragged = rnn_util.RAGGED_GEMM and inputs.is_cuda and self.dtype != ASR_F32 and \
+            (drop_masks is not None or not self._split_rows(Bp))
         with ops.side_lane(inputs.device):
+            if ragged:
+                self._rows = ops.valid_rows(seq_len, Tt, Bp)
             for li, layer in enumerate(self.layers):
                 preps.append(layer.prepare(inputs.device, self.dtype, Tt, Bp, 1.0, False, None, None,
                                            ldk=ldk0 if li == 0 else None))
@@ -148,7 +154,7 @@
             elif li == 1:
                 ops.wait_event(ready_w[-1])
             x, final = layer.forward(x, seq_len, self.dtype, keep_prob, is_training, prep=preps[li],
-                                     mask_event=ready_m[li])
+                                     mask_event=ready_m[li], **({} if self._rows is None else {'rows': self._rows}))
             finals.append(final)
             if self.num_layers_sub is not None and li + 1 == self.num_layers_sub:
                 self._out_sub_op, self._final_sub_ch = x, final
@@ -285,9 +291,12 @@
             if cb is not None and (cb['gates'].numel() * cb['gates'].element_size() +
                                    cb['cs'].numel() * cb['cs'].element_size()) > (128 << 20):
                 cb = None
+            kw = {}
+            if self._rows is not None and li > 0 and not (d_outputs_sub is not None and li - 1 == self.num_layers_sub - 1):
+                kw['rows'] = self._rows
             dx = self.layers[li].backward(dx.contiguous(), dcf, dhf, need_dx=(li > 0 or need_input_grad),
                                           dout_masked=masked, dx_mask=below, background=(li > 0),
-                                          warm=(cb['gates'], cb['cs']) if cb is not None else None)
+                                          warm=(cb['gates'], cb['cs']) if cb is not None else None, **kw)
             ops.wait_event(getattr(self.layers[li], 'warm_event', None))
             masked = below is not None
             if self.grad_ready_hook is not None:
diff --git a/tensorflow_end2end_speech_recognition_amd/models/encoders/core/rnn_util.py b/tensorflow_end2end_speech_recognition_amd/models/encoders/core/rnn_util.py
--- a/tensorflow_end2end_speech_recognition_amd/models/encoders/core/rnn_util.py
+++ b/tensorflow_end2end_speech_recognition_amd/models/encoders/core/rnn_util.py
@@ -11,6 +11,7 @@
 FORK_ONCE = _os.environ.get('ASR_FORK_ONCE', '1') != '0'
 BG_WGS = int(_os.environ.get('ASR_BG_WGS', '128'))
 DW_AFTER_DX_FLOPS = {'0': float('inf'), '1': 0.0}.get(_os.environ.get('ASR_DW_AFTER_DX', ''), 2e11)
+RAGGED_GEMM = _os.environ.get('ASR_RAGGED_GEMM', '1') != '0'
 
 
 def declare_lstm_vars(store, scope, din, H, ndir, use_peephole, parameter_init, rng, cell_scope=None):
@@ -68,14 +69,14 @@
         return ops.dropout_apply(t, *mask) if isinstance(mask, tuple) else ops.apply_mask(t, mask)
 
     def forward(self, x, seq_len, dtype, keep_prob=1.0, is_training=True, rng_state=None,
-                drop_mask=None, save=True, prep=None, mask_event=None):
+                drop_mask=None, save=True, prep=None, mask_event=None, rows=None):
         T, B, ldk = x.shape
         H, ndir = self.H, self.ndir
         if prep is None:
             prep = self.prepare(x.device, dtype, T, B, keep_prob, is_training, rng_state, drop_mask, ldk=ldk)
         xproj = torch.empty((T, B, ndir * 4 * H), dtype=torch.float32, device=x.device)
         ops.gemm(x.view(T * B, ldk), prep['wxT'], transB=True, bias=prep['bias'],
-                 out=xproj.view(T * B, ndir * 4 * H))
+                 out=xproj.view(T * B, ndir * 4 * H), **({} if rows is None else {'rows': rows}))
         gates, hout, cs, cf, hf = ops.lstm_fwd(xproj, prep['whf'], prep['peep'], seq_len, H, ndir, dtype,
                                                self.forget_bias, self.cell_clip or 0.0)
         out = hout
@@ -90,7 +91,7 @@
         return out, (cf, hf)
 
     def backward(self, dout, d_c_final=None, d_h_final=None, need_dx=True, dout_masked=False, dx_mask=None,
-                 background=False, warm=None, acc=None, finish=True):
+                 background=False, warm=None, acc=None, finish=True, rows=None):
         c = self.ctx
         st = self.store
         dtype = c['dtype']
@@ -114,11 +115,12 @@
         dg2d = dgates.view(T * B, ndir * 4 * H)
         dx = torch.empty((T, B, din), dtype=torch.float32, device=x.device) if need_dx else None
         if need_dx:
+            kw = {} if rows is None else {'rows': rows}
             if isinstance(dx_mask, tuple):
-                ops.gemm(dg2d, c['wx_cat'], transB=True, out=dx.view(T * B, din), drop=dx_mask)
+                ops.gemm(dg2d, c['wx_cat'], transB=True, out=dx.view(T * B, din), drop=dx_mask, **kw)
             else:
                 ops.gemm(dg2d, c['wx_cat'], transB=True, out=dx.view(T * B, din),
-                         mul=dx_mask.view(T * B, din) if dx_mask is not None else None)
+                         mul=dx_mask.view(T * B, din) if dx_mask is not None else None, **kw)
             if FORK_ONCE and background and 2.0 * T * B * din * ndir * 4 * H >= DW_AFTER_DX_FLOPS:
                 fork = ops.stream_event()
         add = acc is not None
diff --git a/tensorflow_end2end_speech_recognition_amd/ops.py b/tensorflow_end2end_speech_recognition_amd/ops.py
--- a/tensorflow_end2end_speech_recognition_amd/ops.py
+++ b/tensorflow_end2end_speech_recognition_amd/ops.py
@@ -344,8 +344,20 @@
     return out
 
 
+def valid_rows(seq_len, T, B):
+    h = _h(seq_len)
+    _chk(seq_len, torch.int32, 'seq_len')
+    if seq_len.numel() != B:
+        raise ValueError('valid_rows: seq_len must hold B = %d lengths' % B)
+    buf = torch.empty((T * B + 4,), dtype=torch.int32, device=seq_len.device)
+    rows, count = buf[4:], buf[:1]
+    h.check(h.lib.asr_valid_rows(h.h, _p(seq_len), int(T), int(B), C.c_void_p(rows.data_ptr()),
+                                 C.c_void_p(count.data_ptr()), _s()), 'asr_valid_rows')
+    return rows, count
+
+
 def gemm(A, B, transA=False, transB=False, bias=None, out=None, out_dtype=None, accumulate=False, relu=False,
-         mul=None, drop=None):
+         mul=None, drop=None, rows=None):
     h = _h(A)
     dt = dtype_id(A.dtype)
     if B.dtype != A.dtype:
@@ -366,6 +378,27 @@
             raise ValueError('gemm: bad out shape %s' % (tuple(out.shape),))
     if bias is not None:
         _chk(bias, torch.float32, 'bias')
+    if rows is not None:
+        rl, cnt = rows
+        _chk(rl, torch.int32, 'rows')
+        _chk(cnt, torch.int32, 'row count')
+        if rl.numel() < M or (mul is not None and drop is not None):
+            raise ValueError('gemm: the row list must have room for M rows; mul and drop exclude each other')
+        if drop is not None and (odt != ASR_F32 or not out.is_contiguous() or N % 4):
+            raise ValueError('gemm: drop needs a contiguous fp32 output with N % 4 == 0')
+        if mul is not None:
+            _chk(mul, torch.float32, 'mul')
+            if odt != ASR_F32 or mul.dim() != 2 or mul.shape != (M, N) or mul.stride(1) != 1:
+                raise ValueError('gemm: mul needs an fp32 output and an fp32 [M,N] multiplier')
+        kp, seed, off = drop if drop is not None else (1.0, 0, 0)
+        h.check(h.lib.asr_gemm_rows(h.h, dt, odt, int(transA), int(transB), M, N, K,
+                                    C.c_void_p(A.data_ptr()), A.stride(0), C.c_void_p(B.data_ptr()), B.stride(0),
+                                    C.c_void_p(out.data_ptr()), out.stride(0), _p(bias), int(accumulate),
+                                    1 if relu else 0, C.c_void_p(mul.data_ptr()) if mul is not None else None,
+                                    mul.stride(0) if mul is not None else 0, 1 if drop is not None else 0, float(kp),
+                                    int(seed), int(off), C.c_void_p(rl.data_ptr()), C.c_void_p(cnt.data_ptr()), _s()),
+                'asr_gemm_rows')
+        return out
     if drop is not None:
         if odt != ASR_F32 or not out.is_contiguous() or N % 4:
             raise ValueError('gemm: drop needs a contiguous fp32 output with N % 4 == 0')
```
